# yex33/ReSpaSol

Hardware: AMD Instinct MI355X
Metric: CSR SpMV GFLOP/s + achieved HBM GB/s (fp64 vs fp32), SuiteSparse set, 1/2/4/8 GPU (higher is better)
Workload: dtype f64; 1 GPU; big-set CSR SpMV fp64, 15 matrices per step; matrices=15, nnz_stored_total=268386865, parallelism=1 GPU, launch=rsp_spmv_batch (1 launch(es) of <= 32 matrices per step part): whole step

## Files before the change

include/rsp.h:

```cpp
#ifndef RSP_H
#define RSP_H

#include <stddef.h>
#include <stdint.h>

#ifdef __cplusplus
extern "C" {
#endif

#define RSP_VERSION_MAJOR 0
#define RSP_VERSION_MINOR 1

typedef enum {
    RSP_STATUS_SUCCESS = 0,
    RSP_STATUS_NOT_INITIALIZED = 1,
    RSP_STATUS_ALLOC_FAILED = 2,
    RSP_STATUS_INVALID_VALUE = 3,
    RSP_STATUS_ARCH_MISMATCH = 4,
    RSP_STATUS_EXECUTION_FAILED = 6,
    RSP_STATUS_INTERNAL_ERROR = 7,
    RSP_STATUS_MATRIX_TYPE_NOT_SUPPORTED = 8,
    RSP_STATUS_ZERO_PIVOT = 9,
    RSP_STATUS_NOT_SUPPORTED = 10
} rsp_status_t;

typedef enum { RSP_R_64F = 0, RSP_R_32F = 1 } rsp_datatype_t;

typedef enum { RSP_OPERATION_NON_TRANSPOSE = 0, RSP_OPERATION_TRANSPOSE = 1 } rsp_operation_t;

typedef struct rsp_context *rsp_handle_t;
typedef struct rsp_spmat *rsp_spmat_t;
typedef struct rsp_ilu0_info *rsp_ilu0_info_t;
typedef struct rsp_spmv_batch *rsp_spmv_batch_t;


rsp_status_t rsp_create(rsp_handle_t *handle);
rsp_status_t rsp_destroy(rsp_handle_t handle);
rsp_status_t rsp_set_stream(rsp_handle_t handle, void *stream);
rsp_status_t rsp_get_stream(rsp_handle_t handle, void **stream);
rsp_status_t rsp_set_ftz(rsp_handle_t handle, int enable);
rsp_status_t rsp_get_ftz(rsp_handle_t handle, int *enable);
const char *rsp_get_error_string(rsp_status_t status);
int rsp_get_version(void);


rsp_status_t rsp_create_csr(rsp_spmat_t *mat, int64_t rows, int64_t cols, int64_t nnz,
                            void *d_row_offsets, void *d_col_ind, void *d_values,
                            rsp_datatype_t value_type);
rsp_status_t rsp_csr_set_values(rsp_spmat_t mat, void *d_values, rsp_datatype_t value_type);
rsp_status_t rsp_destroy_spmat(rsp_spmat_t mat);


rsp_status_t rsp_spmv_buffer_size(rsp_handle_t handle, rsp_operation_t op, const void *alpha,
                                  rsp_spmat_t mat, const void *beta, rsp_datatype_t compute_type,
                                  size_t *buffer_size);
rsp_status_t rsp_spmv_preprocess(rsp_handle_t handle, rsp_operation_t op, const void *alpha,
                                 rsp_spmat_t mat, const void *d_x, const void *beta, void *d_y,
                                 rsp_datatype_t compute_type, void *d_buffer);
rsp_status_t rsp_spmv(rsp_handle_t handle, rsp_operation_t op, const void *alpha, rsp_spmat_t mat,
                      const void *d_x, const void *beta, void *d_y, rsp_datatype_t compute_type,
                      void *d_buffer);


rsp_status_t rsp_create_ilu0_info(rsp_ilu0_info_t *info);
rsp_status_t rsp_destroy_ilu0_info(rsp_ilu0_info_t info);

rsp_status_t rsp_ilu0_buffer_size(rsp_handle_t handle, int n, int nnz, rsp_datatype_t value_type,
                                  rsp_ilu0_info_t info, size_t *buffer_size);

rsp_status_t rsp_ilu0_analysis(rsp_handle_t handle, int n, int nnz, const int *d_row_offsets,
                               const int *d_col_ind, rsp_ilu0_info_t info);

rsp_status_t rsp_trsv_analysis(rsp_handle_t handle, rsp_operation_t op, rsp_ilu0_info_t info);

rsp_status_t rsp_ilu0_zero_pivot(rsp_handle_t handle, rsp_ilu0_info_t info, int *position);

#define RSP_TRSV_L 0
#define RSP_TRSV_LT 1
#define RSP_TRSV_U 2
rsp_status_t rsp_trsv_zero_pivot(rsp_handle_t handle, rsp_ilu0_info_t info, int which, int *position);

rsp_status_t rsp_ilu0_factor(rsp_handle_t handle, rsp_ilu0_info_t info, rsp_datatype_t value_type,
                             void *d_values);

rsp_status_t rsp_trsv_lower_unit(rsp_handle_t handle, rsp_operation_t op, const void *alpha,
                                 rsp_ilu0_info_t info, rsp_datatype_t value_type,
                                 const void *d_values, const void *d_x, void *d_y);

rsp_status_t rsp_trsv_upper(rsp_handle_t handle, const void *alpha, rsp_ilu0_info_t info,
                            rsp_datatype_t value_type, const void *d_values, const void *d_x,
                            void *d_y);


typedef struct rsp_bicgstab *rsp_bicgstab_t;
typedef enum { RSP_SOLVE_CONVERGED = 0, RSP_SOLVE_MAX_ITERS = 1, RSP_SOLVE_BREAKDOWN = 2 } rsp_solve_reason_t;

rsp_status_t rsp_bicgstab_create(rsp_handle_t handle, rsp_spmat_t A, rsp_ilu0_info_t info,
                                 rsp_datatype_t precond_type, const void *d_factor, rsp_bicgstab_t *s);
rsp_status_t rsp_bicgstab_solve(rsp_handle_t handle, rsp_bicgstab_t s, const void *d_b, void *d_x,
                                double rtol, int max_iters, int check_every,
                                int *iters, double *relres, rsp_solve_reason_t *reason);
rsp_status_t rsp_bicgstab_history(rsp_bicgstab_t s, int cap, double *relres, int *count);
rsp_status_t rsp_bicgstab_destroy(rsp_bicgstab_t s);
rsp_status_t rsp_dot(rsp_handle_t handle, rsp_datatype_t value_type, int64_t n, const void *d_x,
                     const void *d_y, double *result);

#define RSP_GMRES_MAX_RESTART 64
typedef struct rsp_gmres *rsp_gmres_t;
rsp_status_t rsp_gmres_create(rsp_handle_t handle, rsp_spmat_t A, rsp_ilu0_info_t info,
                              rsp_datatype_t precond_type, const void *d_factor, int restart,
                              rsp_gmres_t *s);
rsp_status_t rsp_gmres_solve(rsp_handle_t handle, rsp_gmres_t s, const void *d_b, void *d_x, double rtol,
                             int max_iters, int check_every, int *iters, double *relres,
                             rsp_solve_reason_t *reason);
rsp_status_t rsp_gmres_history(rsp_gmres_t s, int cap, double *relres, int *count);
rsp_status_t rsp_gmres_destroy(rsp_gmres_t s);
rsp_status_t rsp_orthogonalize(rsp_handle_t handle, rsp_datatype_t value_type, int64_t n, int k,
                               const void *d_V, int64_t ldv, void *d_w, double *h);
rsp_status_t rsp_gmres_lsq_host(int k, int ldh, const double *H, double beta, double *y, double *est);


rsp_status_t rsp_gather(rsp_handle_t handle, rsp_datatype_t value_type, int64_t n,
                        const int64_t *d_idx, const void *d_src, void *d_dst);
rsp_status_t rsp_scatter(rsp_handle_t handle, rsp_datatype_t value_type, int64_t n,
                         const int64_t *d_idx, const void *d_src, void *d_dst);

rsp_status_t rsp_spmv_plan_info(rsp_spmat_t mat, int64_t *tiles, int64_t *entries_16bit);

rsp_status_t rsp_spmat_set_local_cols(rsp_spmat_t mat, int64_t ncols_local);
rsp_status_t rsp_spmv_part(rsp_handle_t handle, const void *alpha, rsp_spmat_t mat,
                           const void *d_x, const void *beta, void *d_y,
                           rsp_datatype_t compute_type, void *d_buffer, int part);

rsp_status_t rsp_spmv_batch_create(rsp_handle_t handle, int count, const rsp_spmat_t *mats,
                                   const void *const *d_x, void *const *d_y,
                                   void *const *d_buffers, rsp_datatype_t compute_type,
                                   int part, rsp_spmv_batch_t *batch);
rsp_status_t rsp_spmv_batch_run(rsp_handle_t handle, rsp_spmv_batch_t batch, const void *alpha,
                                const void *beta);
rsp_status_t rsp_spmv_batch_destroy(rsp_spmv_batch_t batch);
rsp_status_t rsp_spmv_batch_info(rsp_spmv_batch_t batch, int64_t *tiles, int64_t *entries_16bit);

rsp_status_t rsp_ilu0_levels(rsp_ilu0_info_t info, int *levels_lower, int *levels_upper);
rsp_status_t rsp_ilu0_solve_blocks(rsp_ilu0_info_t info, int *blocks_lower, int *blocks_upper);

rsp_status_t rsp_ilu0_analysis_host(int n, const int *row_offsets, const int *col_ind,
                                    int *levels_lower, int *levels_upper, uint64_t *digest,
                                    double *phase_ms);
rsp_status_t rsp_spmv_plan_host(int m, const int *row_offsets, const int *col_ind, int64_t nnz,
                                rsp_datatype_t compute_type, int64_t *tiles, int64_t *entries_16bit,
                                int64_t *entries_staged);
rsp_status_t rsp_spmv_plan_stats(int m, const int *row_offsets, const int *col_ind, int64_t nnz,
                                 rsp_datatype_t compute_type, int64_t stats[8]);
rsp_status_t rsp_ilu0_plan_digest(rsp_ilu0_info_t info, uint64_t *digest);

#ifdef __cplusplus
}
#endif

#endif
```

respasol_amd/_lib.py:

```python
from __future__ import annotations

import ctypes as C
import os

_HERE = os.path.dirname(os.path.abspath(__file__))
LIB_DIR = os.path.join(_HERE, "lib")
BIN_DIR = os.path.join(_HERE, "bin")


class RspError(RuntimeError):

    def __init__(self, status: int, where: str):
        self.status = int(status)
        super().__init__(f"{where}: {STATUS_NAMES.get(self.status, 'RSP_STATUS_UNKNOWN')} ({self.status})")


STATUS_SUCCESS = 0
STATUS_NOT_INITIALIZED = 1
STATUS_ALLOC_FAILED = 2
STATUS_INVALID_VALUE = 3
STATUS_ARCH_MISMATCH = 4
STATUS_EXECUTION_FAILED = 6
STATUS_INTERNAL_ERROR = 7
STATUS_MATRIX_TYPE_NOT_SUPPORTED = 8
STATUS_ZERO_PIVOT = 9
STATUS_NOT_SUPPORTED = 10
STATUS_NAMES = {
    0: "RSP_STATUS_SUCCESS", 1: "RSP_STATUS_NOT_INITIALIZED", 2: "RSP_STATUS_ALLOC_FAILED",
    3: "RSP_STATUS_INVALID_VALUE", 4: "RSP_STATUS_ARCH_MISMATCH", 6: "RSP_STATUS_EXECUTION_FAILED",
    7: "RSP_STATUS_INTERNAL_ERROR", 8: "RSP_STATUS_MATRIX_TYPE_NOT_SUPPORTED",
    9: "RSP_STATUS_ZERO_PIVOT", 10: "RSP_STATUS_NOT_SUPPORTED",
}

R_64F = 0
R_32F = 1
OP_N = 0
OP_T = 1

SOLVE_CONVERGED = 0
SOLVE_MAX_ITERS = 1
SOLVE_BREAKDOWN = 2
KRY_CHUNK = 2048
KRY_MAX_GRID = 1024
GMRES_MAX_RESTART = 64

MM_FULL_SYMMETRIC = 0x1
MM_QUIET = 0x2
MM_SERIAL = 0x4
SURR_FTZ_STRESS = 0x1


class CSRStruct(C.Structure):

    _fields_ = [("isSymmetric", C.c_int), ("m", C.c_int), ("n", C.c_int), ("nnz", C.c_int),
                ("rowptr", C.POINTER(C.c_int)), ("colidx", C.POINTER(C.c_int)),
                ("values", C.POINTER(C.c_double))]


class COOStruct(C.Structure):

    _fields_ = [("isSymmetric", C.c_int), ("m", C.c_int), ("n", C.c_int), ("nnz", C.c_int),
                ("Colidx", C.POINTER(C.c_int)), ("Rowidx", C.POINTER(C.c_int)),
                ("values", C.POINTER(C.c_double))]


vp = C.c_void_p
ip = C.POINTER(C.c_int)
i64 = C.c_int64
i32 = C.c_int

RSP_PROTOS = {
    "rsp_create": (i32, [C.POINTER(vp)]),
    "rsp_destroy": (i32, [vp]),
    "rsp_set_stream": (i32, [vp, vp]),
    "rsp_get_stream": (i32, [vp, C.POINTER(vp)]),
    "rsp_set_ftz": (i32, [vp, i32]),
    "rsp_get_ftz": (i32, [vp, ip]),
    "rsp_get_error_string": (C.c_char_p, [i32]),
    "rsp_get_version": (i32, []),
    "rsp_create_csr": (i32, [C.POINTER(vp), i64, i64, i64, vp, vp, vp, i32]),
    "rsp_csr_set_values": (i32, [vp, vp, i32]),
    "rsp_destroy_spmat": (i32, [vp]),
    "rsp_spmv_buffer_size": (i32, [vp, i32, vp, vp, vp, i32, C.POINTER(C.c_size_t)]),
    "rsp_spmv_preprocess": (i32, [vp, i32, vp, vp, vp, vp, vp, i32, vp]),
    "rsp_spmv": (i32, [vp, i32, vp, vp, vp, vp, vp, i32, vp]),
    "rsp_create_ilu0_info": (i32, [C.POINTER(vp)]),
    "rsp_destroy_ilu0_info": (i32, [vp]),
    "rsp_ilu0_buffer_size": (i32, [vp, i32, i32, i32, vp, C.POINTER(C.c_size_t)]),
    "rsp_ilu0_analysis": (i32, [vp, i32, i32, vp, vp, vp]),
    "rsp_ilu0_zero_pivot": (i32, [vp, vp, ip]),
    "rsp_trsv_zero_pivot": (i32, [vp, vp, i32, ip]),
    "rsp_ilu0_factor": (i32, [vp, vp, i32, vp]),
    "rsp_trsv_lower_unit": (i32, [vp, i32, vp, vp, i32, vp, vp, vp]),
    "rsp_trsv_upper": (i32, [vp, vp, vp, i32, vp, vp, vp]),
    "rsp_ilu0_levels": (i32, [vp, ip, ip]),
    "rsp_ilu0_solve_blocks": (i32, [vp, ip, ip]),
    "rsp_trsv_analysis": (i32, [vp, i32, vp]),
    "rsp_bicgstab_create": (i32, [vp, vp, vp, i32, vp, C.POINTER(vp)]),
    "rsp_bicgstab_solve": (i32, [vp, vp, vp, vp, C.c_double, i32, i32, ip, C.POINTER(C.c_double), ip]),
    "rsp_bicgstab_history": (i32, [vp, i32, C.POINTER(C.c_double), ip]),
    "rsp_bicgstab_destroy": (i32, [vp]),
    "rsp_dot": (i32, [vp, i32, i64, vp, vp, C.POINTER(C.c_double)]),
    "rsp_gmres_create": (i32, [vp, vp, vp, i32, vp, i32, C.POINTER(vp)]),
    "rsp_gmres_solve": (i32, [vp, vp, vp, vp, C.c_double, i32, i32, ip, C.POINTER(C.c_double), ip]),
    "rsp_gmres_history": (i32, [vp, i32, C.POINTER(C.c_double), ip]),
    "rsp_gmres_destroy": (i32, [vp]),
    "rsp_orthogonalize": (i32, [vp, i32, i64, i32, vp, i64, vp, C.POINTER(C.c_double)]),
    "rsp_gmres_lsq_host": (i32, [i32, i32, C.POINTER(C.c_double), C.c_double, C.POINTER(C.c_double),
                                 C.POINTER(C.c_double)]),
    "rsp_gather": (i32, [vp, i32, i64, vp, vp, vp]),
    "rsp_scatter": (i32, [vp, i32, i64, vp, vp, vp]),
    "rsp_spmat_set_local_cols": (i32, [vp, i64]),
    "rsp_spmv_part": (i32, [vp, vp, vp, vp, vp, vp, i32, vp, i32]),
    "rsp_spmv_batch_create": (i32, [vp, i32, vp, vp, vp, vp, i32, i32, vp]),
    "rsp_spmv_batch_run": (i32, [vp, vp, vp, vp]),
    "rsp_spmv_batch_destroy": (i32, [vp]),
    "rsp_spmv_batch_info": (i32, [vp, vp, vp]),
    "rsp_spmv_plan_info": (i32, [vp, vp, vp]),
    "rsp_ilu0_analysis_host": (i32, [i32, vp, vp, vp, vp, vp, vp]),
    "rsp_spmv_plan_host": (i32, [i32, vp, vp, C.c_int64, i32, vp, vp, vp]),
    "rsp_spmv_plan_stats": (i32, [i32, vp, vp, C.c_int64, i32, vp]),
    "rsp_ilu0_plan_digest": (i32, [vp, vp]),
}

HOST_PROTOS = {
    "loadMatrixMarket": (i32, [C.c_char_p, C.POINTER(CSRStruct), i32, i32]),
    "loadCooMatrix": (i32, [C.c_char_p, C.POINTER(COOStruct), i32, i32]),
    "rsp_mm_load": (i32, [C.c_char_p, C.POINTER(CSRStruct), i32, i32, i32]),
    "rsp_mm_load_buffer": (i32, [C.c_char_p, C.c_size_t, C.POINTER(CSRStruct), i32, i32, i32]),
    "rsp_row_qsort": (None, [ip, C.POINTER(C.c_double), i32, i32]),
    "rsp_csr_free": (None, [C.POINTER(CSRStruct)]),
    "rsp_coo_free": (None, [C.POINTER(COOStruct)]),
    "rsp_csr_save": (i32, [C.c_char_p, C.POINTER(CSRStruct)]),
    "rsp_csr_load": (i32, [C.c_char_p, C.POINTER(CSRStruct)]),
    "rsp_dlarnv": (i32, [i32, ip, i64, C.POINTER(C.c_double)]),
    "rsp_set_cpu_ftz": (None, [i32]),
    "rsp_surrogate_count": (i32, []),
    "rsp_surrogate_name": (C.c_char_p, [i32]),
    "rsp_surrogate_info": (i32, [C.c_char_p, ip, C.POINTER(i64), ip, ip, ip]),
    "rsp_surrogate_rowlens": (i32, [C.c_char_p, C.c_double, i32, i32, i32, ip]),
    "rsp_surrogate_rows": (i32, [C.c_char_p, C.c_double, ip]),
    "rsp_surrogate_fill": (i32, [C.c_char_p, C.c_double, i32, i32, i32, ip, ip, C.POINTER(C.c_double)]),
    "rsp_surrogate_csr": (i32, [C.c_char_p, C.c_double, i32, C.POINTER(CSRStruct)]),
    "rsp_partition_rows": (i32, [ip, i32, i32, ip]),
    "rsp_padded_chunk": (i32, [ip, i32]),
    "rsp_remap_cols_padded": (i32, [i64, ip, ip, i32, i32, ip]),
    "rsp_host_spmv_f64": (None, [i32, ip, ip, vp, vp, vp]),
    "rsp_host_spmv_f32": (None, [i32, ip, ip, vp, vp, vp]),
}


def _load(name: str, protos: dict, path: str | None = None, probe: bool = False) -> C.CDLL:
    path = path or os.path.join(LIB_DIR, name)
    if not os.path.exists(path):
        raise ImportError(
            f"{path} is missing: build the HIP/C libraries first "
            f"(python -c 'import __graft_entry__ as g; g.build()' or make -C respasol_amd/csrc)")
    lib = C.CDLL(path, mode=C.RTLD_GLOBAL)
    for fname, (res, args) in protos.items():
        if probe and not hasattr(lib, fname):
            continue
        fn = getattr(lib, fname)
        fn.restype = res
        fn.argtypes = args
    return lib


host = _load("librsp_host.so", HOST_PROTOS)
_RSP_PATH = os.environ.get("RSP_PROBE_LIB") or os.path.join(LIB_DIR, "librsp.so")
rsp = (None if os.environ.get("RSP_HOST_ONLY") == "1"
       else _load("librsp.so", RSP_PROTOS, _RSP_PATH, probe=bool(os.environ.get("RSP_PROBE_LIB"))))


def check(status: int, where: str) -> None:
    if status != STATUS_SUCCESS:
        raise RspError(status, where)


def loaded_paths() -> list[str]:
    return [os.path.join(LIB_DIR, "librsp_host.so"), _RSP_PATH]
```

respasol_amd/csrc/rsp_api.cpp:

```cpp

#include "rsp_internal.h"

#include <atomic>

using namespace rsp_api;

using rsp::SpmvBlock;
using rsp::SpmvLongRow;
using rsp_plan::PlanOptions;
using rsp_plan::TilePlan;

namespace {
std::atomic<unsigned long long> g_plan_next{1};
unsigned long long plan_new_gen() { return g_plan_next.fetch_add(1); }
}


static int64_t spmv_resident_tiles(rsp_handle_t h, rsp_datatype_t t) {
    return (int64_t)rsp_k::spmv_tiles_per_cu((int)elem_size(t)) * h->num_cus;
}

static PlanOptions handle_plan_options(rsp_handle_t h, rsp_datatype_t t, int64_t local_cols, int64_t spread) {
    const int e = (int)elem_size(t), v = h->spmv_variant;
    PlanOptions o = rsp_plan::plan_options(t);
    o.spread = spread;
    o.local_cols = local_cols;
    o.row_align = (v & 64) ? 128 / e : (v & 128) ? 64 / e : 1;
    o.use_c16 = !(v & 32);
    o.use_stage = !(v & rsp::kSpmvVariantNoStage);
    return o;
}

static rsp_status_t download_pattern(rsp_handle_t h, rsp_spmat_t mat, rsp_an::hvec<int> &rp,
                                     rsp_an::hvec<int> &ci) {
    const int m = (int)mat->rows;
    rp.assign((size_t)m + 1, 0);
    ci.clear();
    if (m > 0) {
        RSP_CHECK_HIP(hipMemcpyAsync(rp.data(), mat->rowptr, ((size_t)m + 1) * sizeof(int),
                                     hipMemcpyDeviceToHost, h->stream));
        RSP_CHECK_HIP(hipStreamSynchronize(h->stream));
    }
    if (m > 0 && rp[0] != 0) return RSP_STATUS_INVALID_VALUE;
    for (int i = 0; i < m; i++)
        if (rp[i + 1] < rp[i]) return RSP_STATUS_INVALID_VALUE;
    if (m > 0 && (int64_t)rp[(size_t)m] > mat->nnz) return RSP_STATUS_INVALID_VALUE;
    if (m > 0 && rp[(size_t)m] > 0) {
        if (!mat->colidx) return RSP_STATUS_INVALID_VALUE;
        ci.resize((size_t)rp[(size_t)m]);
        RSP_CHECK_HIP(hipMemcpyAsync(ci.data(), mat->colidx, ci.size() * sizeof(int),
                                     hipMemcpyDeviceToHost, h->stream));
        RSP_CHECK_HIP(hipStreamSynchronize(h->stream));
        const int ncols = (int)mat->cols;
        for (int c : ci)
            if ((unsigned)c >= (unsigned)ncols) return RSP_STATUS_INVALID_VALUE;
    }
    return RSP_STATUS_SUCCESS;
}

rsp_status_t rsp_api::spmv_plan(rsp_handle_t h, rsp_spmat_t mat, rsp_datatype_t compute_type) {
    const int m = (int)mat->rows;
    rsp_an::hvec<int> rp, ci;
    rsp_status_t st = download_pattern(h, mat, rp, ci);
    if (st != RSP_STATUS_SUCCESS) return st;
    const bool spread = (h->spmv_variant & 512) != 0;
    TilePlan p;
    rsp_plan::make_tile_plan(rp.data(), ci.data(), m, mat->nnz,
                             handle_plan_options(h, compute_type, mat->local_cols,
                                                 spread ? spmv_resident_tiles(h, compute_type) : 0),
                             p);
    const size_t elem = elem_size(compute_type);
    const rsp_plan::SpmvLayout lay = rsp_plan::spmv_layout({p.blocks.size(), p.longrows.size(), (size_t)p.nslots},
                                                           elem, (int64_t)p.c16.size(), p.runs.size());
    mat->planned = 0;
    if (lay.bytes > mat->plan_cap || !mat->d_plan) {
        if (mat->d_plan) {
            int cur = 0;
            (void)hipGetDevice(&cur);
            (void)hipSetDevice(mat->plan_device);
            (void)hipFree(mat->d_plan);
            (void)hipSetDevice(cur);
            mat->d_plan = nullptr;
            mat->plan_cap = 0;
        }
        RSP_CHECK_HIP(hipMalloc(&mat->d_plan, std::max<size_t>(lay.bytes, 256)));
        mat->plan_cap = std::max<size_t>(lay.bytes, 256);
        RSP_CHECK_HIP(hipGetDevice(&mat->plan_device));
    }
    char *buf = (char *)mat->d_plan;
    auto upload = [&](size_t off, const void *src, size_t bytes) {
        return bytes == 0 ? hipSuccess : hipMemcpyAsync(buf + off, src, bytes, hipMemcpyHostToDevice, h->stream);
    };
    RSP_CHECK_HIP(upload(0, p.blocks.data(), p.blocks.size() * sizeof(SpmvBlock)));
    RSP_CHECK_HIP(upload(lay.off_cbase, p.cbase.data(), p.cbase.size() * sizeof(int)));
    RSP_CHECK_HIP(upload(lay.off_poff, p.poff.data(), p.poff.size() * sizeof(int)));
    RSP_CHECK_HIP(upload(lay.off_cidx, p.c16.data(), p.c16.size() * sizeof(uint16_t)));
    RSP_CHECK_HIP(upload(lay.off_runs, p.runs.data(), p.runs.size() * sizeof(int)));
    RSP_CHECK_HIP(upload(lay.off_long, p.longrows.data(), p.longrows.size() * sizeof(SpmvLongRow)));
    if (p.nslots > 0)
        RSP_CHECK_HIP(hipMemsetAsync(buf + lay.off_part, 0, (size_t)p.nslots * 2 * elem, h->stream));
    RSP_CHECK_HIP(hipStreamSynchronize(h->stream));
    mat->planned = 1;
    mat->plan_type = compute_type;
    mat->nblocks = (int)p.blocks.size();
    mat->nint = p.nint;
    mat->plan_gen = plan_new_gen();
    mat->nlong = (int)p.longrows.size();
    mat->nslots = p.nslots;
    mat->nnz_s = m > 0 ? rp[(size_t)m] : 0;
    mat->lay = lay;
    mat->nnz_c16 = p.nnz_c16;
    mat->nnz_staged = p.nnz_staged;
    return RSP_STATUS_SUCCESS;
}

rsp_status_t rsp_api::spmv_run(rsp_handle_t h, rsp_operation_t op, const void *alpha, rsp_spmat_t mat,
                               const void *d_x, const void *beta, void *d_y,
                               rsp_datatype_t compute_type, void *d_buffer, int part) {
    if (!h) return RSP_STATUS_NOT_INITIALIZED;
    if (!mat || !alpha || !beta) return RSP_STATUS_INVALID_VALUE;
    if (op != RSP_OPERATION_NON_TRANSPOSE) return RSP_STATUS_NOT_SUPPORTED;
    if (compute_type != mat->type) return RSP_STATUS_INVALID_VALUE;
    if (mat->rows > 0 && (!d_y || (mat->cols > 0 && !d_x))) return RSP_STATUS_INVALID_VALUE;
    (void)d_buffer;
    if (!mat->planned || mat->plan_type != compute_type) {
        rsp_status_t st = spmv_plan(h, mat, compute_type);
        if (st != RSP_STATUS_SUCCESS) return st;
    }
    char *plan = (char *)mat->d_plan;
    rsp::SpmvArgs a;
    a.m = (int)mat->rows;
    a.rowptr = mat->rowptr;
    a.colidx = mat->colidx;
    a.vals = mat->vals;
    a.x = d_x;
    a.y = d_y;
    a.blocks = (const SpmvBlock *)plan;
    a.nblocks = mat->nblocks;
    a.cbases = (const int *)(plan + mat->lay.off_cbase);
    a.poffs = (const int *)(plan + mat->lay.off_poff);
    a.cidx = (const unsigned short *)(plan + mat->lay.off_cidx);
    a.runs = (const int *)(plan + mat->lay.off_runs);
    a.cmax = mat->cols > 0 ? (int)(mat->cols - 1) : 0;
    a.longrows = (const SpmvLongRow *)(plan + mat->lay.off_long);
    a.nlong = mat->nlong;
    a.partials = plan + mat->lay.off_part;
    if (compute_type == RSP_R_64F) {
        a.alpha = *(const double *)alpha;
        a.beta = *(const double *)beta;
    } else {
        a.alpha = *(const float *)alpha;
        a.beta = *(const float *)beta;
    }
    if (part != 0) {
        if (a.beta != 0.0) return RSP_STATUS_INVALID_VALUE;
        if (part == 1) {
            a.nblocks = mat->nint;
            a.nlong = 0;
        } else {
            a.blocks += mat->nint;
            a.cbases += mat->nint;
            a.poffs += mat->nint;
            a.nblocks = mat->nblocks - mat->nint;
        }
    }
    a.vector_ok = ((((uintptr_t)mat->colidx) | ((uintptr_t)mat->vals)) & 15) == 0;
    a.nnz = mat->nnz_s;
    a.variant = h->spmv_variant;
    hipError_t e;
    if (compute_type == RSP_R_64F)
        e = rsp_k::spmv_f64(a, h->stream);
    else
        e = h->ftz ? rsp_k_ftz::spmv_f32(a, h->stream) : rsp_k::spmv_f32(a, h->stream);
    return e == hipSuccess ? RSP_STATUS_SUCCESS : RSP_STATUS_EXECUTION_FAILED;
}


struct rsp_spmv_batch {
    rsp_datatype_t type;
    int part;
    rsp_an::hvec<rsp_spmat_t> mats;
    rsp_an::hvec<unsigned long long> plan_gen;
    rsp_an::hvec<rsp::SpmvBatchArgs> launches;
    void *d_mem = nullptr;
    int64_t tiles = 0, entries_16bit = 0;
    ~rsp_spmv_batch() {
        if (d_mem) (void)hipFree(d_mem);
    }
};

static rsp_status_t spmv_batch_create(rsp_handle_t h, int count, const rsp_spmat_t *mats,
                                      const void *const *d_x, void *const *d_y,
                                      void *const *d_buffers, rsp_datatype_t compute_type,
                                      int part, rsp_spmv_batch_t *batch) {
    if (!h) return RSP_STATUS_NOT_INITIALIZED;
    (void)d_buffers;
    if (!batch || count < 0 || (count > 0 && (!mats || !d_x || !d_y)))
        return RSP_STATUS_INVALID_VALUE;
    if (part < 0 || part > 2) return RSP_STATUS_INVALID_VALUE;
    if (compute_type != RSP_R_64F && compute_type != RSP_R_32F) return RSP_STATUS_INVALID_VALUE;
    *batch = nullptr;
    for (int j = 0; j < count; j++) {
        rsp_spmat_t A = mats[j];
        if (!A) return RSP_STATUS_INVALID_VALUE;
        if (A->type != compute_type) return RSP_STATUS_INVALID_VALUE;
        if (A->rows > 0 && (!d_y[j] || (A->cols > 0 && !d_x[j]))) return RSP_STATUS_INVALID_VALUE;
        if (!A->planned || A->plan_type != compute_type) {
            rsp_status_t st = spmv_plan(h, A, compute_type);
            if (st != RSP_STATUS_SUCCESS) return st;
        }
    }
    std::unique_ptr<rsp_spmv_batch> b(new rsp_spmv_batch());
    b->type = compute_type;
    b->part = part;
    const int64_t R = spmv_resident_tiles(h, compute_type);
    const bool spread_ok = !(h->spmv_variant & 16);
    rsp_an::hvec<TilePlan> plans((size_t)count);
    struct Region { size_t off, len; };
    struct Span {
        int first, count, nt, nl;
        rsp_an::hvec<Region> reg;
        enum { kEntries, kTiles, kCbases, kPoffs, kLongRows, kC16, kRuns, kPartials };
        const Region &at(int kind, int q) const { return reg[kind < kC16 ? kind : kC16 + (kind - kC16) * count + q]; }
    };
    rsp_an::hvec<Span> spans;
    size_t bytes = 0;
    auto tile_range = [part](const TilePlan &p, int *t0, int *t1) {
        *t0 = part == 2 ? p.nint : 0;
        *t1 = part == 1 ? p.nint : (int)p.blocks.size();
    };
    for (int first = 0; first < count; first += rsp::kSpmvBatchMax) {
        Span sp{first, std::min(rsp::kSpmvBatchMax, count - first), 0, 0, {}};
        rsp_an::hvec<rsp_an::hvec<int>> rps((size_t)sp.count), cis((size_t)sp.count);
        auto plan_members = [&](int64_t spread_all, int64_t nnz_all) {
            sp.nt = 0;
            for (int q = 0; q < sp.count; q++) {
                rsp_spmat_t A = mats[first + q];
                const int64_t nnz_q = A->rows > 0 ? rps[q][(size_t)A->rows] : 0;
                const int64_t share =
                    spread_all > 0 ? std::max<int64_t>(1, spread_all * nnz_q / std::max<int64_t>(1, nnz_all)) : 0;
                TilePlan &p = plans[first + q];
                rsp_plan::make_tile_plan(rps[q].data(), cis[q].data(), (int)A->rows, A->nnz,
                                         handle_plan_options(h, compute_type, A->local_cols, share), p);
                int t0, t1;
                tile_range(p, &t0, &t1);
                sp.nt += t1 - t0;
            }
        };
        int64_t nnz_all = 0;
        for (int q = 0; q < sp.count; q++) {
            rsp_spmat_t A = mats[first + q];
            rsp_status_t st = download_pattern(h, A, rps[q], cis[q]);
            if (st != RSP_STATUS_SUCCESS) return st;
            nnz_all += A->rows > 0 ? rps[q][(size_t)A->rows] : 0;
        }
        plan_members(0, nnz_all);
        if (spread_ok && sp.nt < R) plan_members(R, nnz_all);
        for (int q = 0; q < sp.count; q++) {
            const TilePlan &p = plans[first + q];
            rsp_spmat_t A = mats[first + q];
            if ((int)p.longrows.size() != A->nlong || p.nslots != A->nslots)
                return RSP_STATUS_INTERNAL_ERROR;
            sp.nl += part == 1 ? 0 : (int)p.longrows.size();
        }
        sp.reg = {{0, (size_t)sp.count * sizeof(rsp::SpmvBatchEntry)},
                  {0, (size_t)sp.nt * sizeof(SpmvBlock)},
                  {0, (size_t)sp.nt * sizeof(int)},
                  {0, (size_t)sp.nt * sizeof(int)},
                  {0, (size_t)sp.nl * sizeof(SpmvLongRow)}};
        for (int q = 0; q < sp.count; q++) sp.reg.push_back({0, plans[first + q].c16.size() * sizeof(uint16_t)});
        for (int q = 0; q < sp.count; q++) sp.reg.push_back({0, plans[first + q].runs.size() * sizeof(int)});
        for (int q = 0; q < sp.count; q++)
            sp.reg.push_back({0, (size_t)plans[first + q].nslots * 2 * elem_size(compute_type)});
        for (Region &r : sp.reg) {
            r.off = bytes;
            bytes += (r.len + 15) & ~(size_t)15;
        }
        spans.push_back(sp);
    }
    {
        size_t end = 0;
        for (const Span &sp : spans)
            for (const Region &r : sp.reg) {
                if (r.off < end || r.off + r.len > bytes) return RSP_STATUS_INTERNAL_ERROR;
                end = r.off + r.len;
            }
    }
    if (bytes > 0) RSP_CHECK_HIP(hipMalloc(&b->d_mem, bytes));
    rsp_an::hvec<unsigned char> host(bytes);
    bool fits = true;
    for (const Span &sp : spans) {
        auto dev = [&](int kind, int q = 0) { return (char *)b->d_mem + sp.at(kind, q).off; };
        auto put = [&](int kind, int q, size_t at, const void *src, size_t n) {
            const Region &r = sp.at(kind, q);
            if (at + n > r.len)
                fits = false;
            else if (n > 0)
                memcpy(host.data() + r.off + at, src, n);
        };
        rsp::SpmvBatchArgs a{};
        a.entries = (const rsp::SpmvBatchEntry *)dev(Span::kEntries);
        a.tiles = (const SpmvBlock *)dev(Span::kTiles);
        a.cbases = (const int *)dev(Span::kCbases);
        a.poffs = (const int *)dev(Span::kPoffs);
        a.longrows = (const SpmvLongRow *)dev(Span::kLongRows);
        a.count = sp.count;
        for (int q = 0; q <= rsp::kSpmvBatchMax; q++)
            a.tiles_at.begin[q] = a.longs_at.begin[q] = INT_MAX;
        size_t nt = 0, nl = 0;
        for (int q = 0; q < sp.count; q++) {
            rsp_spmat_t A = mats[sp.first + q];
            const TilePlan &p = plans[sp.first + q];
            int t0, t1;
            tile_range(p, &t0, &t1);
            const size_t ntq = (size_t)(t1 - t0), nlq = part == 1 ? 0 : p.longrows.size();
            rsp::SpmvBatchEntry e{};
            e.rowptr = A->rowptr;
            e.colidx = A->colidx;
            e.vals = A->vals;
            e.x = d_x[sp.first + q];
            e.y = d_y[sp.first + q];
            e.partials = (void *)dev(Span::kPartials, q);
            e.cidx = (const unsigned short *)dev(Span::kC16, q);
            e.runs = (const int *)dev(Span::kRuns, q);
            e.cmax = A->cols > 0 ? (int)(A->cols - 1) : 0;
            e.nnz = A->nnz_s;
            e.vector_ok = ((((uintptr_t)A->colidx) | ((uintptr_t)A->vals)) & 15) == 0;
            put(Span::kEntries, 0, (size_t)q * sizeof(e), &e, sizeof(e));
            a.tiles_at.begin[q] = (int)nt;
            a.longs_at.begin[q] = (int)nl;
            for (int t = t0; t < t1; t++)
                if (p.cbase[(size_t)t] != rsp_plan::kCbaseInt32)
                    b->entries_16bit += p.blocks[(size_t)t].k1 - p.blocks[(size_t)t].k0;
            b->tiles += (int64_t)ntq;
            put(Span::kTiles, 0, nt * sizeof(SpmvBlock), p.blocks.data() + t0, ntq * sizeof(SpmvBlock));
            put(Span::kCbases, 0, nt * sizeof(int), p.cbase.data() + t0, ntq * sizeof(int));
            put(Span::kPoffs, 0, nt * sizeof(int), p.poff.data() + t0, ntq * sizeof(int));
            put(Span::kLongRows, 0, nl * sizeof(SpmvLongRow), p.longrows.data(), nlq * sizeof(SpmvLongRow));
            put(Span::kC16, q, 0, p.c16.data(), p.c16.size() * sizeof(uint16_t));
            put(Span::kRuns, q, 0, p.runs.data(), p.runs.size() * sizeof(int));
            nt += ntq;
            nl += nlq;
        }
        a.tiles_at.begin[sp.count] = (int)nt;
        a.longs_at.begin[sp.count] = (int)nl;
        b->launches.push_back(a);
    }
    if (!fits) return RSP_STATUS_INTERNAL_ERROR;
    if (bytes > 0) {
        RSP_CHECK_HIP(hipMemcpyAsync(b->d_mem, host.data(), bytes, hipMemcpyHostToDevice, h->stream));
        RSP_CHECK_HIP(hipStreamSynchronize(h->stream));
    }
    for (int j = 0; j < count; j++) {
        b->mats.push_back(mats[j]);
        b->plan_gen.push_back(mats[j]->plan_gen);
    }
    *batch = b.release();
    return RSP_STATUS_SUCCESS;
}

extern "C" {

int rsp_get_version(void) { return RSP_VERSION_MAJOR * 1000 + RSP_VERSION_MINOR; }

const char *rsp_get_error_string(rsp_status_t s) {
    switch (s) {
        case RSP_STATUS_SUCCESS: return "RSP_STATUS_SUCCESS";
        case RSP_STATUS_NOT_INITIALIZED: return "RSP_STATUS_NOT_INITIALIZED";
        case RSP_STATUS_ALLOC_FAILED: return "RSP_STATUS_ALLOC_FAILED";
        case RSP_STATUS_INVALID_VALUE: return "RSP_STATUS_INVALID_VALUE";
        case RSP_STATUS_ARCH_MISMATCH: return "RSP_STATUS_ARCH_MISMATCH";
        case RSP_STATUS_EXECUTION_FAILED: return "RSP_STATUS_EXECUTION_FAILED";
        case RSP_STATUS_INTERNAL_ERROR: return "RSP_STATUS_INTERNAL_ERROR";
        case RSP_STATUS_MATRIX_TYPE_NOT_SUPPORTED: return "RSP_STATUS_MATRIX_TYPE_NOT_SUPPORTED";
        case RSP_STATUS_ZERO_PIVOT: return "RSP_STATUS_ZERO_PIVOT";
        case RSP_STATUS_NOT_SUPPORTED: return "RSP_STATUS_NOT_SUPPORTED";
    }
    return "RSP_STATUS_UNKNOWN";
}

rsp_status_t rsp_create(rsp_handle_t *handle) {
    if (!handle) return RSP_STATUS_INVALID_VALUE;
    *handle = nullptr;
    int dev = 0;
    if (hipGetDevice(&dev) != hipSuccess) return RSP_STATUS_NOT_INITIALIZED;
    hipDeviceProp_t prop;
    if (hipGetDeviceProperties(&prop, dev) != hipSuccess) return RSP_STATUS_NOT_INITIALIZED;
    if (strncmp(prop.gcnArchName, "gfx950", 6) != 0) return RSP_STATUS_ARCH_MISMATCH;
    rsp_context *c = new (std::nothrow) rsp_context;
    if (!c) return RSP_STATUS_ALLOC_FAILED;
    c->device = dev;
    c->stream = nullptr;
    c->ftz = 0;
    const char *v = getenv("RSP_SPMV_VARIANT");
    c->spmv_variant = v ? atoi(v) : 0;
    c->num_cus = prop.multiProcessorCount > 0 ? prop.multiProcessorCount : 256;
    rsp_k::warm_spmv();
    rsp_k_ftz::warm_spmv();
    rsp_k::warm_ilu();
    rsp_k_ftz::warm_ilu();
    rsp_k::warm_analysis();
    rsp_k::warm_krylov();
    rsp_k_ftz::warm_krylov();
    c->d_ftrace = nullptr;
    c->d_strace = nullptr;
    c->d_dot = nullptr;
    c->h_dot = nullptr;
    c->d_gm = nullptr;
    c->h_gm = nullptr;
    *handle = c;
    return RSP_STATUS_SUCCESS;
}

rsp_status_t rsp_destroy(rsp_handle_t h) {
    if (!h) return RSP_STATUS_NOT_INITIALIZED;
    if (h->d_ftrace || h->d_strace || h->d_dot || h->h_dot || h->d_gm || h->h_gm) {
        int cur = 0;
        (void)hipGetDevice(&cur);
        (void)hipSetDevice(h->device);
        if (h->d_ftrace) (void)hipFree(h->d_ftrace);
        if (h->d_strace) (void)hipFree(h->d_strace);
        if (h->d_dot) (void)hipFree(h->d_dot);
        if (h->h_dot) (void)hipHostFree(h->h_dot);
        if (h->d_gm) (void)hipFree(h->d_gm);
        if (h->h_gm) (void)hipHostFree(h->h_gm);
        (void)hipSetDevice(cur);
    }
    delete h;
    return RSP_STATUS_SUCCESS;
}

rsp_status_t rsp_set_stream(rsp_handle_t h, void *stream) {
    if (!h) return RSP_STATUS_NOT_INITIALIZED;
    h->stream = (hipStream_t)stream;
    return RSP_STATUS_SUCCESS;
}

rsp_status_t rsp_get_stream(rsp_handle_t h, void **stream) {
    if (!h) return RSP_STATUS_NOT_INITIALIZED;
    if (!stream) return RSP_STATUS_INVALID_VALUE;
    *stream = (void *)h->stream;
    return RSP_STATUS_SUCCESS;
}

rsp_status_t rsp_set_ftz(rsp_handle_t h, int enable) {
    if (!h) return RSP_STATUS_NOT_INITIALIZED;
    h->ftz = enable ? 1 : 0;
    return RSP_STATUS_SUCCESS;
}

rsp_status_t rsp_get_ftz(rsp_handle_t h, int *enable) {
    if (!h) return RSP_STATUS_NOT_INITIALIZED;
    if (!enable) return RSP_STATUS_INVALID_VALUE;
    *enable = h->ftz;
    return RSP_STATUS_SUCCESS;
}


rsp_status_t rsp_create_csr(rsp_spmat_t *mat, int64_t rows, int64_t cols, int64_t nnz,
                            void *d_row_offsets, void *d_col_ind, void *d_values,
                            rsp_datatype_t value_type) {
    if (!mat) return RSP_STATUS_INVALID_VALUE;
    *mat = nullptr;
    if (rows < 0 || cols < 0 || nnz < 0 || rows > INT_MAX - 1 || cols > INT_MAX || nnz > INT_MAX)
        return RSP_STATUS_INVALID_VALUE;
    if (value_type != RSP_R_64F && value_type != RSP_R_32F) return RSP_STATUS_INVALID_VALUE;
    if (!d_row_offsets && rows > 0) return RSP_STATUS_INVALID_VALUE;
    if ((!d_col_ind || !d_values) && nnz > 0) return RSP_STATUS_INVALID_VALUE;
    rsp_spmat *a = new (std::nothrow) rsp_spmat;
    if (!a) return RSP_STATUS_ALLOC_FAILED;
    memset(a, 0, sizeof(*a));
    a->rows = rows;
    a->cols = cols;
    a->nnz = nnz;
    a->rowptr = (int *)d_row_offsets;
    a->colidx = (int *)d_col_ind;
    a->vals = d_values;
    a->type = value_type;
    a->planned = 0;
    a->d_plan = nullptr;
    a->local_cols = -1;
    *mat = a;
    return RSP_STATUS_SUCCESS;
}

rsp_status_t rsp_spmat_set_local_cols(rsp_spmat_t mat, int64_t ncols_local) {
    if (!mat || ncols_local < 0 || ncols_local > mat->cols) return RSP_STATUS_INVALID_VALUE;
    mat->local_cols = ncols_local;
    mat->planned = 0;
    return RSP_STATUS_SUCCESS;
}

rsp_status_t rsp_csr_set_values(rsp_spmat_t mat, void *d_values, rsp_datatype_t value_type) {
    if (!mat) return RSP_STATUS_INVALID_VALUE;
    if (value_type != RSP_R_64F && value_type != RSP_R_32F) return RSP_STATUS_INVALID_VALUE;
    if (d_values != mat->vals) mat->plan_gen = plan_new_gen();
    mat->vals = d_values;
    if (value_type != mat->type) mat->planned = 0;
    mat->type = value_type;
    return RSP_STATUS_SUCCESS;
}

rsp_status_t rsp_destroy_spmat(rsp_spmat_t mat) {
    if (!mat) return RSP_STATUS_INVALID_VALUE;
    if (mat->d_plan) {
        int cur = 0;
        (void)hipGetDevice(&cur);
        (void)hipSetDevice(mat->plan_device);
        (void)hipFree(mat->d_plan);
        (void)hipSetDevice(cur);
    }
    delete mat;
    return RSP_STATUS_SUCCESS;
}


rsp_status_t rsp_spmv_buffer_size(rsp_handle_t h, rsp_operation_t op, const void *alpha,
                                  rsp_spmat_t mat, const void *beta, rsp_datatype_t compute_type,
                                  size_t *buffer_size) {
    (void)alpha;
    (void)beta;
    return guarded([&] {
        if (!h) return RSP_STATUS_NOT_INITIALIZED;
        if (!mat || !buffer_size) return RSP_STATUS_INVALID_VALUE;
        if (op != RSP_OPERATION_NON_TRANSPOSE) return RSP_STATUS_NOT_SUPPORTED;
        if (compute_type != mat->type) return RSP_STATUS_INVALID_VALUE;
        if (!mat->planned || mat->plan_type != compute_type) RSP_TRY(spmv_plan(h, mat, compute_type));
        *buffer_size = 0;
        return RSP_STATUS_SUCCESS;
    });
}

rsp_status_t rsp_spmv_preprocess(rsp_handle_t h, rsp_operation_t op, const void *alpha,
                                 rsp_spmat_t mat, const void *d_x, const void *beta, void *d_y,
                                 rsp_datatype_t compute_type, void *d_buffer) {
    (void)alpha;
    (void)beta;
    (void)d_x;
    (void)d_y;
    (void)d_buffer;
    return guarded([&] {
        if (!h) return RSP_STATUS_NOT_INITIALIZED;
        if (!mat) return RSP_STATUS_INVALID_VALUE;
        if (op != RSP_OPERATION_NON_TRANSPOSE) return RSP_STATUS_NOT_SUPPORTED;
        if (compute_type != mat->type) return RSP_STATUS_INVALID_VALUE;
        return spmv_plan(h, mat, compute_type);
    });
}

rsp_status_t rsp_spmv_plan_info(rsp_spmat_t mat, int64_t *tiles, int64_t *entries_16bit) {
    if (!mat || !tiles || !entries_16bit) return RSP_STATUS_INVALID_VALUE;
    if (!mat->planned) return RSP_STATUS_NOT_INITIALIZED;
    *tiles = mat->nblocks;
    *entries_16bit = mat->nnz_c16;
    return RSP_STATUS_SUCCESS;
}

rsp_status_t rsp_spmv(rsp_handle_t h, rsp_operation_t op, const void *alpha, rsp_spmat_t mat,
                      const void *d_x, const void *beta, void *d_y, rsp_datatype_t compute_type,
                      void *d_buffer) {
    return guarded([&] { return spmv_run(h, op, alpha, mat, d_x, beta, d_y, compute_type, d_buffer, 0); });
}

rsp_status_t rsp_spmv_part(rsp_handle_t h, const void *alpha, rsp_spmat_t mat, const void *d_x,
                           const void *beta, void *d_y, rsp_datatype_t compute_type,
                           void *d_buffer, int part) {
    return guarded([&] {
        if (part < 0 || part > 2) return RSP_STATUS_INVALID_VALUE;
        return spmv_run(h, RSP_OPERATION_NON_TRANSPOSE, alpha, mat, d_x, beta, d_y, compute_type,
                        d_buffer, part);
    });
}


rsp_status_t rsp_spmv_batch_create(rsp_handle_t h, int count, const rsp_spmat_t *mats,
                                   const void *const *d_x, void *const *d_y,
                                   void *const *d_buffers, rsp_datatype_t compute_type,
                                   int part, rsp_spmv_batch_t *batch) {
    return guarded([&] { return spmv_batch_create(h, count, mats, d_x, d_y, d_buffers, compute_type, part, batch); });
}

rsp_status_t rsp_spmv_batch_run(rsp_handle_t h, rsp_spmv_batch_t b, const void *alpha,
                                const void *beta) {
    if (!h) return RSP_STATUS_NOT_INITIALIZED;
    if (!b || !alpha || !beta) return RSP_STATUS_INVALID_VALUE;
    for (size_t j = 0; j < b->mats.size(); j++) {
        const rsp_spmat_t A = b->mats[j];
        if (!A->planned || A->plan_gen != b->plan_gen[j]) return RSP_STATUS_INVALID_VALUE;
    }
    const double av = b->type == RSP_R_64F ? *(const double *)alpha : *(const float *)alpha;
    const double bv = b->type == RSP_R_64F ? *(const double *)beta : *(const float *)beta;
    if (b->part != 0 && bv != 0.0) return RSP_STATUS_INVALID_VALUE;
    for (rsp::SpmvBatchArgs a : b->launches) {
        a.alpha = av;
        a.beta = bv;
        a.variant = h->spmv_variant;
        hipError_t e;
        if (b->type == RSP_R_64F)
            e = rsp_k::spmv_batch_f64(a, h->stream);
        else
            e = h->ftz ? rsp_k_ftz::spmv_batch_f32(a, h->stream) : rsp_k::spmv_batch_f32(a, h->stream);
        if (e != hipSuccess) return RSP_STATUS_EXECUTION_FAILED;
    }
    return RSP_STATUS_SUCCESS;
}

rsp_status_t rsp_spmv_batch_info(rsp_spmv_batch_t b, int64_t *tiles, int64_t *entries_16bit) {
    if (!b || !tiles || !entries_16bit) return RSP_STATUS_INVALID_VALUE;
    *tiles = b->tiles;
    *entries_16bit = b->entries_16bit;
    return RSP_STATUS_SUCCESS;
}

rsp_status_t rsp_spmv_batch_destroy(rsp_spmv_batch_t b) {
    if (!b) return RSP_STATUS_INVALID_VALUE;
    delete b;
    return RSP_STATUS_SUCCESS;
}

rsp_status_t rsp_gather(rsp_handle_t h, rsp_datatype_t value_type, int64_t n, const int64_t *d_idx,
                        const void *d_src, void *d_dst) {
    if (!h) return RSP_STATUS_NOT_INITIALIZED;
    if (value_type != RSP_R_64F && value_type != RSP_R_32F) return RSP_STATUS_INVALID_VALUE;
    if (n < 0 || (n > 0 && (!d_idx || !d_src || !d_dst))) return RSP_STATUS_INVALID_VALUE;
    hipError_t e = rsp_k::gather(value_type == RSP_R_64F ? 8 : 4, n, d_idx, d_src, d_dst, h->stream);
    return e == hipSuccess ? RSP_STATUS_SUCCESS : RSP_STATUS_EXECUTION_FAILED;
}

rsp_status_t rsp_scatter(rsp_handle_t h, rsp_datatype_t value_type, int64_t n, const int64_t *d_idx,
                         const void *d_src, void *d_dst) {
    if (!h) return RSP_STATUS_NOT_INITIALIZED;
    if (value_type != RSP_R_64F && value_type != RSP_R_32F) return RSP_STATUS_INVALID_VALUE;
    if (n < 0 || (n > 0 && (!d_idx || !d_src || !d_dst))) return RSP_STATUS_INVALID_VALUE;
    hipError_t e = rsp_k::scatter(value_type == RSP_R_64F ? 8 : 4, n, d_idx, d_src, d_dst, h->stream);
    return e == hipSuccess ? RSP_STATUS_SUCCESS : RSP_STATUS_EXECUTION_FAILED;
}

rsp_status_t rsp_spmv_plan_host(int m, const int *row_offsets, const int *col_ind, int64_t nnz,
                                rsp_datatype_t compute_type, int64_t *tiles, int64_t *entries_16bit,
                                int64_t *entries_staged) {
    return guarded([&] {
        if (m < 0 || (m > 0 && (!row_offsets || !col_ind)) || !tiles || !entries_16bit || !entries_staged)
            return RSP_STATUS_INVALID_VALUE;
        if (compute_type != RSP_R_64F && compute_type != RSP_R_32F) return RSP_STATUS_NOT_SUPPORTED;
        const PlanOptions o = rsp_plan::plan_options(compute_type);
        TilePlan p;
        rsp_plan::make_tile_plan(row_offsets, col_ind, m, nnz, o, p);
        if (!rsp_plan::plan_verify(row_offsets, col_ind, m, o, p)) return RSP_STATUS_INTERNAL_ERROR;
        *tiles = (int64_t)p.blocks.size();
        *entries_16bit = p.nnz_c16;
        *entries_staged = p.nnz_staged;
        return RSP_STATUS_SUCCESS;
    });
}

rsp_status_t rsp_spmv_plan_stats(int m, const int *row_offsets, const int *col_ind, int64_t nnz,
                                 rsp_datatype_t compute_type, int64_t stats[8]) {
    return guarded([&] {
        if (m < 0 || (m > 0 && (!row_offsets || !col_ind)) || !stats) return RSP_STATUS_INVALID_VALUE;
        if (compute_type != RSP_R_64F && compute_type != RSP_R_32F) return RSP_STATUS_NOT_SUPPORTED;
        TilePlan p;
        rsp_plan::make_tile_plan(row_offsets, col_ind, m, nnz, rsp_plan::plan_options(compute_type), p);
        rsp_plan::plan_stats(p, compute_type, stats);
        return RSP_STATUS_SUCCESS;
    });
}

}
```

respasol_amd/csrc/rsp_kernels.h:

```cpp
#pragma once

#include <hip/hip_runtime.h>
#include <stdint.h>

namespace rsp {

struct alignas(16) SpmvBlock {
    int r0, r1, k0, k1;
};

struct alignas(16) SpmvLongRow {
    int row, first, nchunks, pad;
};

#ifndef RSP_SPMV_THREADS
#define RSP_SPMV_THREADS 256
#endif
constexpr int kSpmvThreads = RSP_SPMV_THREADS;
#ifndef RSP_SPMV_ITER
#define RSP_SPMV_ITER 4
#endif
constexpr int kSpmvIter = RSP_SPMV_ITER;
#ifndef RSP_SPMV_MAXROWS
#define RSP_SPMV_MAXROWS 512
#endif
constexpr int kSpmvMaxRows = RSP_SPMV_MAXROWS;
constexpr int kSpmvLongRow = 256;
constexpr int kSpmvHeavyMax = 128;
constexpr int kSpmvWholeRow = -2147483647 - 1;
template <typename T>
struct SpmvTile {
    static constexpr int kVec = 16 / sizeof(T);
    static constexpr int kSlots = kSpmvThreads * kSpmvIter * kVec;
    static constexpr int kMaxNnz = kSlots - (kVec - 1);
    static constexpr int kChunk = kSpmvThreads * 4 * kVec - (kVec - 1);
    static_assert(kChunk <= kMaxNnz, "a chunk must fit one tile");
    static constexpr int kMaxRows = sizeof(T) == 8 ? kSpmvMaxRows : 2 * kSpmvMaxRows;
    static constexpr int kStageSlots = sizeof(T) == 8 ? 1536 : 2048;
    static constexpr bool kStageList = sizeof(T) == 8;
};
static_assert(SpmvTile<float>::kMaxNnz / 33 < kSpmvHeavyMax && SpmvTile<double>::kMaxNnz / 33 < kSpmvHeavyMax,
              "every > 32-entry row of a tile fits the heavy-row list");
constexpr int kStageRuns = 254;

struct SpmvArgs {
    int m;
    const int *rowptr;
    const int *colidx;
    const void *vals;
    const void *x;
    void *y;
    const SpmvBlock *blocks;
    int nblocks;
    const int *cbases;
    const unsigned short *cidx;
    const int *runs;
    const int *poffs;
    int cmax;
    const SpmvLongRow *longrows;
    int nlong;
    void *partials;
    double alpha, beta;
    int nnz;
    int vector_ok;
    int variant;
};

constexpr int kSpmvBatchMax = 32;
struct alignas(16) SpmvBatchEntry {
    const int *rowptr;
    const int *colidx;
    const void *vals;
    const void *x;
    void *y;
    void *partials;
    const unsigned short *cidx;
    const int *runs;
    int nnz;
    int vector_ok;
    int cmax;
};
struct SpmvBatchTable {
    int begin[kSpmvBatchMax + 1];
};
struct SpmvBatchArgs {
    const SpmvBatchEntry *entries;
    const SpmvBlock *tiles;
    const int *cbases;
    const int *poffs;
    const SpmvLongRow *longrows;
    int count;
    SpmvBatchTable tiles_at, longs_at;
    double alpha, beta;
    int variant;
};
constexpr int kSpmvVariantFixup = 256;
constexpr int kSpmvVariantNoStage = 1024;

struct LevelSeg {
    int lb, le, thin, c0, c1;
    int nth;
};
struct alignas(16) RowTask {
    int i, t0, t1, d;
};
struct alignas(16) LevelChunk {
    int l0, l1;
    int x0, x1;
    int k0, k1;
    int st0, st1;
};
struct alignas(16) FlowItem {
    int x0, n, t0, gate;
};
struct alignas(16) ThinRowPlan {
    int g, out, i, d;
};
struct alignas(8) StagedTerm {
    int slot, j;
};

struct LevelPlan {
    const int *rows;
    const int *ptr_dev;
    const int *ptr_host;
    int nlev;
    const LevelSeg *segs;
    int nseg;
    int batch;
    int group;
    const RowTask *tasks;
    const int *tpos;
    const int *src;
    const LevelChunk *chunks;
    const ThinRowPlan *trow;
    const int *sid;
    const StagedTerm *stg;
    const FlowItem *fitems;
    int has_flow;
    int nterms;
    const int *nshort;
    const int *nshort_host;
    const int *nwave_host;
    const int *sbase_host;
};
constexpr int kLongTerms = 64;
constexpr int kHubTerms = 256;
constexpr int kFatLongTerms = 8;
constexpr int kFatLongDefault = 3;
constexpr int kYWin = 4096;
constexpr int kChunkRows = 1024;
constexpr int kChunkTerms = 4096;
constexpr int kThinThreads = 1024;
constexpr int kGroup = 4;
constexpr int kPadSrc = -(kYWin + 1);
constexpr int kIluWaves = 4;
constexpr int kFacRow = 256;
constexpr int kFacPairs = 1024;
constexpr int kThinSolveRows = 512;
constexpr int kThinSolveTerms = 2048;
constexpr int kThinFactorRows = 1024;
constexpr int kRndItems = 2048;
constexpr int kRndPairs = 4096;
constexpr int kRndStaged = 4096;
constexpr int kRndRounds = 2048;
constexpr int kRndLevelItems = 1 << 15;
constexpr int kRndFlowItems = 1024;
constexpr int kRndItemPairs = 1024;
constexpr int kRndLevelStart = 1 << 15;
struct alignas(16) RndChunk {
    int i0, i1, p0, p1, s0, s1, r0, r1;
};
struct alignas(16) RndItem {
    int pos, u, d, zr;
};

struct alignas(16) FacRow {
    int i, rs, di, re, q0, q1, hasdiag, pad;
};

struct FacSlotLevel {
    long long off;
    int stride, rm, qm, pad;
};
__host__ __device__ constexpr int fac_pairs_at(int rm) { return (8 + 2 * rm + 1) & ~1; }

struct alignas(16) FacFlowItem {
    long long off;
    int rmqm, gate;
};
struct FacFlowRun {
    int lb, le, c0, c1;
};

struct FlowCtl {
    int *status;
    int gen;
    unsigned long long ticks;
    unsigned long long *claim;
    unsigned long long *claim_host;
    int mode;
    unsigned *tickets;
    unsigned long long *tk_seq;
    int *done;
    int grid_x;
    unsigned epoch;
};
constexpr int kFlowClaims = 1;
constexpr int kFlowTickets = 2;
constexpr int kFlowTicketCtrs = 8;
constexpr int kFlowOwnMax = 1024;
constexpr int kFlowStealUs = 50;


struct IluArgs {
    int n;
    const int *rowptr;
    const int *colidx;
    const int *dpos;
    const int *hasdiag;
    void *vals;
    int *zero_pivot;
    const int *upd_ptr;
    const int *upd_l;
    const int *upd_u;
    const int *lord;
    const int *lend;
    const int *udiv;
    const FacRow *frow;
    const int *fslots;
    const FacSlotLevel *fslev;
    int fat_slots;
    int fat_lds;
    LevelPlan plan;
    const RndChunk *rchunks;
    const RndItem *ritems;
    const int *rpairs, *rstaged, *rrounds;
    unsigned long long *trace;
    int trace_cap;
    int defer_rounds;
    int narrow_waves;
    const FacFlowItem *fitems;
    const FacFlowRun *fruns;
    int nfruns;
    const int *lev;
    void *forig;
    int gen;
    int flow, flow_grid, flow_sleep;
    int flow_cus;
    FlowCtl fc;
    int fac_one;
};

constexpr int kBlkRows = 64, kBlkYMax = 32, kBlkNear = 12, kBlkNearWin = 1 << 30, kBlkWin = 16384;
constexpr int kBlkLongCap = 64 * kBlkNear;
constexpr int kBlkPre = 6;
constexpr int kBlkLdsMax = 160 * 1024;
struct alignas(16) BlkDesc {
    int p0, np, kind, kn;
    int eoff, ne, doff, nd;
    int loff, nlev, pad[2];
};
struct alignas(16) BlkRow {
    int off, nx, ny, nfar;
};
struct BlkSeg {
    int b0, b1, p0, p1;
};
struct BlkArgs {
    int n, nb;
    const int *order;
    const BlkDesc *desc;
    const BlkRow *rows;
    const int *ref;
    const int *vpos;
    const unsigned *eord;
    const int *lptr;
    const int *rptr;
    const unsigned *rit;
    const BlkSeg *segs;
    int nseg;
    int lds_elems;
    int lds_words;
    const void *vals, *x;
    void *y;
    double alpha;
    void *ev, *yp;
    void *rc;
};

struct TrsvArgs {
    int n;
    const int *rowptr;
    const int *colidx;
    const int *dpos;
    const int *hasdiag;
    const void *vals;
    const void *x;
    void *y;
    double alpha;
    LevelPlan plan;
    void *sval;
    void *sx;
    void *sdg;
    unsigned long long *trace;
    int trace_cap;
    int trace_clk;
    int wave_lds;
    int narrow_waves;
    int narrow_split;
    int narrow_pairs;
    int loaders;
    int flow;
    int flow_grid;
    int flow_cus;
    FlowCtl fc;
    int flow_sleep;
};


constexpr int kKryThreads = 256;
constexpr int kKryChunk = 2048;
constexpr int kKryMaxGrid = 1024;
struct KryGrid {
    int grid;
    long long chunk;
};
inline KryGrid kry_grid(long long n) {
    KryGrid g;
    const long long span = (long long)kKryChunk * kKryMaxGrid;
    g.chunk = (long long)kKryChunk * (n > span ? (n + span - 1) / span : 1);
    g.grid = n > 0 ? (int)((n + g.chunk - 1) / g.chunk) : 1;
    return g;
}
enum {
    kKryRho0 = 0,
    kKryRho1 = 1,
    kKryAlpha = 2,
    kKryOmega = 3,
    kKryFlag = 4,
    kKryFlagIt = 5,
    kKryScalars = 16
};
enum { kKryPartRR = 0, kKryPartBB, kKryPartRhR, kKryPartRhV, kKryPartTS, kKryPartTT, kKryDots };
enum { kKryBreakRho = 1, kKryBreakOmega = 2, kKryBreakRhV = 3, kKryBreakTT = 4 };
constexpr size_t kKryBlockDoubles = kKryScalars + (size_t)kKryDots * kKryMaxGrid;
enum KryOp {
    kKryInit,
    kKryPUpdate,
    kKryDotRhV,
    kKrySUpdate,
    kKryDotTS,
    kKryXUpdate,
    kKryWiden,
    kKryZero,
    kKryDot
};
enum { kKryF64 = 0, kKryF32 = 1, kKryF64Copy32 = 2 };
struct KryArgs {
    long long n;
    double *blk;
    int it;
    const void *b;
    const void *c;
    void *x, *r, *rhat, *p, *v, *s, *t;
    const void *phat, *shat;
    void *copy32;
};
inline double kry_combine_host(const double *part, int g) {
    double v[kKryThreads];
    for (int t = 0; t < kKryThreads; t++) {
        v[t] = 0.0;
        for (int i = t; i < g; i += kKryThreads) v[t] += part[i];
    }
    double w[kKryThreads / 64];
    for (int k = 0; k < kKryThreads / 64; k++) {
        double *l = v + 64 * k;
        for (int off = 32; off > 0; off >>= 1)
            for (int i = 0; i < off; i++) l[i] += l[i + off];
        w[k] = l[0];
    }
    return ((w[0] + w[1]) + w[2]) + w[3];
}

constexpr int kGmMax = 64;
constexpr int kGmLd = kGmMax + 1;
enum {
    kGmStop = 0,
    kGmDone = 1,
    kGmBeta = 2,
    kGmBn = 3,
    kGmFlag = kKryFlag,
    kGmFlagIt = kKryFlagIt,
    kGmScalars = 16,
    kGmEst = kGmScalars,
    kGmHead = kGmEst + kGmMax,
    kGmR = kGmHead,
    kGmCs = kGmR + kGmLd * kGmMax,
    kGmSn = kGmCs + kGmMax,
    kGmG = kGmSn + kGmMax,
    kGmY = kGmG + kGmLd,
    kGmH1 = kGmY + kGmMax,
    kGmH2 = kGmH1 + kGmLd,
    kGmSmall = (kGmH2 + kGmLd + 15) / 16 * 16
};
enum {
    kGmPartRR = 0,
    kGmPartBB = 1,
    kGmPartNrm = 2,
    kGmPartD1 = 3,
    kGmPartD2 = kGmPartD1 + kGmLd,
    kGmDots = kGmPartD2 + kGmLd
};
enum { kGmBreakH = 1, kGmBreakDiag = 2, kGmBreakNorm = 3, kGmBreakY = 4 };
constexpr size_t kGmBlockDoubles = kGmSmall + (size_t)kGmDots * kKryMaxGrid;
enum GmOp {
    kGmResid,
    kGmNormalise,
    kGmMultiDot,
    kGmUpdate1,
    kGmUpdate2,
    kGmCombine
};
struct GmArgs {
    long long n;
    double *blk;
    int j;
    int first;
    const void *b;
    void *x;
    void *V;
    long long ldv;
    const void *Z;
    long long ldz;
    void *w;
    void *copy32;
};

#if defined(__HIPCC__)
#define RSP_HD __host__ __device__
#else
#define RSP_HD
#endif
RSP_HD inline int gmres_lsq(double *col, int j, double *cs, double *sn, double *g, const double *R, int ldr,
                            int k, double *y) {
    if (col) {
        for (int i = 0; i <= j + 1; i++)
            if (!(col[i] - col[i] == 0.0)) return kGmBreakH;
        for (int i = 0; i < j; i++) {
            const double a = col[i], b = col[i + 1];
            col[i] = cs[i] * a + sn[i] * b;
            col[i + 1] = cs[i] * b - sn[i] * a;
        }
        const double a = col[j], b = col[j + 1];
        const double aa = a < 0.0 ? -a : a, ab = b < 0.0 ? -b : b;
        const double s = aa > ab ? aa : ab;
        if (s == 0.0) return kGmBreakDiag;
        const double as = a / s, bs = b / s;
        const double r = s * sqrt(as * as + bs * bs);
        if (r == 0.0 || !(r - r == 0.0)) return kGmBreakDiag;
        const double c = a / r, t = b / r;
        cs[j] = c;
        sn[j] = t;
        col[j] = r;
        col[j + 1] = 0.0;
        const double gj = g[j];
        g[j] = c * gj;
        g[j + 1] = -(t * gj);
    }
    if (y) {
        for (int i = k - 1; i >= 0; i--) {
            double v = g[i];
            for (int l = i + 1; l < k; l++) v -= R[i + (size_t)l * ldr] * y[l];
            y[i] = v / R[i + (size_t)i * ldr];
        }
    }
    return 0;
}
}

#define RSP_DECLARE_KERNEL_API(NS)                                                              \
    namespace NS {                                                                              \
    hipError_t spmv_f32(const rsp::SpmvArgs &a, hipStream_t s);                                 \
    hipError_t spmv_batch_f32(const rsp::SpmvBatchArgs &a, hipStream_t s);                      \
    hipError_t ilu0_factor_f32(const rsp::IluArgs &a, hipStream_t s);                           \
    hipError_t trsv_lower_n_f32(const rsp::TrsvArgs &a, hipStream_t s);                         \
    hipError_t trsv_lower_t_f32(const rsp::TrsvArgs &a, hipStream_t s);                         \
    hipError_t trsv_upper_f32(const rsp::TrsvArgs &a, hipStream_t s);                           \
    hipError_t trsv_blocks_f32(const rsp::BlkArgs &a, hipStream_t s);                           \
    void warm_spmv();                                                                           \
    void warm_ilu();                                                                            \
    hipError_t krylov(rsp::KryOp op, int type, const rsp::KryArgs &a, hipStream_t s);           \
    hipError_t gmres(rsp::GmOp op, int type, const rsp::GmArgs &a, hipStream_t s);              \
    void warm_krylov();                                                                         \
    }

RSP_DECLARE_KERNEL_API(rsp_k)
RSP_DECLARE_KERNEL_API(rsp_k_ftz)

namespace rsp_k {
hipError_t gather(int elem_bytes, int64_t n, const int64_t *idx, const void *src, void *dst,
                  hipStream_t s);
hipError_t scatter(int elem_bytes, int64_t n, const int64_t *idx, const void *src, void *dst,
                   hipStream_t s);
hipError_t spmv_f64(const rsp::SpmvArgs &a, hipStream_t s);
hipError_t spmv_batch_f64(const rsp::SpmvBatchArgs &a, hipStream_t s);
int spmv_tiles_per_cu(int elem_bytes);
void warm_analysis();
hipError_t ilu0_factor_f64(const rsp::IluArgs &a, hipStream_t s);
hipError_t trsv_lower_n_f64(const rsp::TrsvArgs &a, hipStream_t s);
hipError_t trsv_lower_t_f64(const rsp::TrsvArgs &a, hipStream_t s);
hipError_t trsv_upper_f64(const rsp::TrsvArgs &a, hipStream_t s);
hipError_t trsv_blocks_f64(const rsp::BlkArgs &a, hipStream_t s);
hipError_t ilu0_build_slots(const rsp::IluArgs &a, const int4 *desc, const long long *offs, int nrows,
                            int *slots, hipStream_t s);
hipError_t ilu_an_rows(int n, const int *rp, const int *ci, int *dpos, int *hasdiag, int *flags, hipStream_t s);
hipError_t ilu_an_count(const int *const rows_c[3], const int n_c[3], int cap0, const int *rp, const int *ci,
                        const int *dpos, const int *hasdiag, int *cnt, int *gcur, hipStream_t s);
hipError_t ilu_an_scan(const int *cnt, int *ptr, int count, void *temp, size_t *temp_bytes, hipStream_t s);
hipError_t ilu_an_gather_pairs(const int *rows, int nrows, const int *rp, const int *ptr, const int *cbase,
                               const int *upd_l, const int *upd_u, int *out_l, int *out_u, hipStream_t s);
hipError_t ilu_an_fill(const int *const rows_c[3], const int n_c[3], int cap0, const int *rp, const int *ci,
                       const int *dpos, const int *hasdiag, const int *ptr, int *gcur, int *upd_l, int *upd_u,
                       hipStream_t s);
hipError_t ilu_an_stages(int n, int maxlen, const int *rp, const int *ci, const int *dpos, const int *hasdiag,
                         const int *ptr, const int *upd_l, int *stage, int *lord, int *lend, int *udiv,
                         int *scratch, const int *wrows, int nwrows, hipStream_t s);
struct SolveTermsArgs {
    int kind, n, nx, total, nch, group;
    const rsp::RowTask *tasks;
    const int *ptr;
    const int *rp, *ci, *dpos;
    const int *ltp, *lts, *ltc;
    const int *lpos;
    const int *ne;
    rsp::LevelChunk *chunks;
    const int *cbase;
    int *tpos, *src, *sid;
    rsp::ThinRowPlan *trow;
    rsp::StagedTerm *stg;
    int *slot_of, *nst, *nst_ptr;
    void *scan;
};
hipError_t ilu_an_solve_terms(const SolveTermsArgs &a, hipStream_t s);
}
```

respasol_amd/csrc/spmv.hip:

```cpp

#include <hip/hip_runtime.h>

#include <type_traits>

#include "rsp_kernels.h"
#include "spmv_pack.h"

#ifndef RSP_KNS
#define RSP_KNS rsp_k
#endif

#ifndef RSP_NT_Y
#define RSP_NT_Y -1
#endif

namespace RSP_KNS {

using rsp::kSpmvThreads;
using rsp::kSpmvHeavyMax;
using rsp::SpmvArgs;
using rsp::SpmvBlock;
using rsp::SpmvLongRow;
using rsp::SpmvTile;
using rsp::kSpmvBatchMax;
using rsp::SpmvBatchArgs;
using rsp::SpmvBatchEntry;
using rsp::SpmvBatchTable;

template <typename T, int N>
struct VecT;
template <>
struct VecT<double, 2> {
    typedef double __attribute__((ext_vector_type(2))) V;
    typedef int __attribute__((ext_vector_type(2))) I;
    typedef unsigned short __attribute__((ext_vector_type(2))) H;
};
template <>
struct VecT<float, 4> {
    typedef float __attribute__((ext_vector_type(4))) V;
    typedef int __attribute__((ext_vector_type(4))) I;
    typedef unsigned short __attribute__((ext_vector_type(4))) H;
};

__device__ __forceinline__ int xcd_swizzle(int bid, int nwg) {
    const int q = nwg >> 3, r = nwg & 7;
    const int xcd = bid & 7, idx = bid >> 3;
    const int start = xcd < r ? xcd * (q + 1) : r * (q + 1) + (xcd - r) * q;
    return start + idx;
}

template <bool NT, typename P>
__device__ __forceinline__ P ld(const P *p) {
    if constexpr (NT)
        return __builtin_nontemporal_load(p);
    else
        return *p;
}

template <typename T, bool NT, bool C16 = false, int NTH = kSpmvThreads,
          int IT = SpmvTile<T>::kSlots / (kSpmvThreads * (16 / sizeof(T)))>
__device__ __forceinline__ void stream_products(const int *__restrict__ colidx,
                                                const unsigned short *__restrict__ cidx, int cbase,
                                                int cmax, const T *__restrict__ vals,
                                                const T *__restrict__ x, int kb, int k1,
                                                T *__restrict__ lds) {
    constexpr int VW = 16 / sizeof(T);
    typedef typename VecT<T, VW>::V V;
    typedef typename VecT<T, VW>::I I;
    typedef typename VecT<T, VW>::H H;
    const int tid = threadIdx.x;
    const int last = (k1 - 1) & ~(VW - 1);
    I ci[IT];
    H ch[IT];
#pragma unroll
    for (int it = 0; it < IT; ++it) {
        const int e = min(kb + (it * NTH + tid) * VW, last);
        if constexpr (C16)
            ch[it] = ld<NT>(reinterpret_cast<const H *>(cidx + e));
        else
            ci[it] = ld<NT>(reinterpret_cast<const I *>(colidx + e));
    }
    V vv[IT];
#pragma unroll
    for (int it = 0; it < IT; ++it) {
        const int e = min(kb + (it * NTH + tid) * VW, last);
        vv[it] = ld<NT>(reinterpret_cast<const V *>(vals + e));
    }
    __builtin_amdgcn_sched_barrier(0);
    T xv[IT][VW];
#pragma unroll
    for (int it = 0; it < IT; ++it)
#pragma unroll
        for (int j = 0; j < VW; ++j) {
            int c;
            if constexpr (C16)
                c = min(cbase + (int)ch[it][j], cmax);
            else
                c = ci[it][j];
            xv[it][j] = x[c];
        }
    __builtin_amdgcn_sched_barrier(0);
#pragma unroll
    for (int it = 0; it < IT; ++it) {
        V p;
#pragma unroll
        for (int j = 0; j < VW; ++j) p[j] = vv[it][j] * xv[it][j];
        *reinterpret_cast<V *>(lds + (it * NTH + tid) * VW) = p;
    }
}

__device__ __forceinline__ void lds_barrier() {
    __builtin_amdgcn_fence(__ATOMIC_RELEASE, "workgroup", "local");
    __builtin_amdgcn_s_barrier();
    __builtin_amdgcn_fence(__ATOMIC_ACQUIRE, "workgroup", "local");
}

template <typename T, bool NT, int PKM, int NTH = kSpmvThreads,
          int IT = SpmvTile<T>::kSlots / (kSpmvThreads * (16 / sizeof(T)))>
__device__ __forceinline__ void stream_products_staged(const unsigned short *__restrict__ cidx,
                                                       const unsigned int *__restrict__ pk, int2 rd,
                                                       int nr, const int (&lsl)[SpmvTile<T>::kStageSlots / NTH],
                                                       const T *__restrict__ vals,
                                                       const T *__restrict__ x, int kb, int k1,
                                                       T *__restrict__ lds) {
    constexpr int VW = 16 / sizeof(T);
    constexpr int SMAX = SpmvTile<T>::kStageSlots / NTH;
    typedef typename VecT<T, VW>::V V;
    const int tid = threadIdx.x;
    const int last = (k1 - 1) & ~(VW - 1);
    constexpr int NW = rsp_pack::words_per_thread(IT * VW);
    constexpr int HW = VW / 2;
    static_assert(NW <= IT * HW, "the packed words fit the unpacked ones' registers");
    const bool pkd = PKM == 2 ? pk != nullptr : PKM == 1;
    unsigned int iw[PKM == 1 ? NW : IT * HW];
    V vv[IT];
    if (pkd) {
        const unsigned int *w = pk + tid * NW;
#pragma unroll
        for (int q = 0; q < NW; ++q) iw[q] = ld<NT>(w + q);
    } else {
#pragma unroll
        for (int it = 0; it < IT; ++it) {
            const int e = min(kb + (it * NTH + tid) * VW, last);
            const unsigned int *w = reinterpret_cast<const unsigned int *>(cidx + e);
#pragma unroll
            for (int q = 0; q < HW; ++q) iw[it * HW + q] = ld<NT>(w + q);
        }
    }
#pragma unroll
    for (int it = 0; it < IT; ++it) {
        const int e = min(kb + (it * NTH + tid) * VW, last);
        vv[it] = ld<NT>(reinterpret_cast<const V *>(vals + e));
    }
    __builtin_amdgcn_sched_barrier(0);
    const __amdgpu_buffer_rsrc_t xr =
        __builtin_amdgcn_make_buffer_rsrc((void *)x, (short)0, 0x7ffffffc, 0x00020000);
    auto xload = [&](int col) {
        if constexpr (sizeof(T) == 8)
            return __builtin_bit_cast(T, __builtin_amdgcn_raw_buffer_load_b64(xr, col * 8, 0, 0));
        else
            return __builtin_bit_cast(T, __builtin_amdgcn_raw_buffer_load_b32(xr, col * 4, 0, 0));
    };
    T xs[SMAX];
    int U;
    if (SpmvTile<T>::kStageList && nr == 255) {
        U = rd.y;
#pragma unroll
        for (int k = 0; k < SMAX; ++k)
            if (k * NTH < U) xs[k] = xload(rd.x + lsl[k]);
    } else {
        int2 *tab = reinterpret_cast<int2 *>(lds + SpmvTile<T>::kSlots) - (nr + 1);
        if (tid <= nr) tab[tid] = rd;
        lds_barrier();
        U = tab[nr].y;
        int us[SMAX], lo[SMAX];
#pragma unroll
        for (int k = 0; k < SMAX; ++k) {
            us[k] = min(k * NTH + tid, U - 1);
            lo[k] = 0;
        }
        for (int n = nr; n > 1;) {
            const int h = n >> 1;
#pragma unroll
            for (int k = 0; k < SMAX; ++k)
                if (tab[lo[k] + h].y <= us[k]) lo[k] += h;
            n -= h;
        }
#pragma unroll
        for (int k = 0; k < SMAX; ++k)
            if (k * NTH < U) {
                const int2 r = tab[lo[k]];
                xs[k] = xload(r.x + (us[k] - r.y));
            }
    }
#pragma unroll
    for (int k = 0; k < SMAX; ++k)
        if (k * NTH < U && k * NTH + tid < U) lds[k * NTH + tid] = xs[k];
    lds_barrier();
    T xv[IT][VW];
    if (pkd) {
#pragma unroll
        for (int it = 0; it < IT; ++it)
#pragma unroll
            for (int j = 0; j < VW; ++j) xv[it][j] = lds[min((int)rsp_pack::get_field(iw, it * VW + j), U - 1)];
    } else {
#pragma unroll
        for (int it = 0; it < IT; ++it)
#pragma unroll
            for (int j = 0; j < VW; ++j)
                xv[it][j] = lds[min((int)((iw[(it * VW + j) >> 1] >> (16 * (j & 1))) & 0xffffu), U - 1)];
    }
    lds_barrier();
#pragma unroll
    for (int it = 0; it < IT; ++it) {
        V p;
#pragma unroll
        for (int j = 0; j < VW; ++j) p[j] = vv[it][j] * xv[it][j];
        *reinterpret_cast<V *>(lds + (it * NTH + tid) * VW) = p;
    }
}

template <typename T, int NTH = kSpmvThreads>
__device__ __forceinline__ void stream_products_scalar(const int *__restrict__ colidx,
                                                       const T *__restrict__ vals,
                                                       const T *__restrict__ x, int k0, int kb,
                                                       int k1, T *lds) {
    for (int e = kb + (int)threadIdx.x; e < k1; e += NTH)
        if (e >= k0) lds[e - kb] = vals[e] * x[colidx[e]];
}

template <typename T, int L, int NTH, typename Sink>
__device__ __forceinline__ void reduce_rows(const T *lds, const unsigned short *rp_lds, int nrows, int kb,
                                            int heavy, int *hl, int *hn, Sink sink) {
    constexpr int NA = 8 / L;
    constexpr int NG = NTH / L;
    const int tid = threadIdx.x;
    const int g = tid / L, lane = tid & (L - 1);
    for (int rr = g; rr - g < nrows; rr += NG) {
        bool active = rr < nrows;
        T acc[NA];
#pragma unroll
        for (int t = 0; t < NA; ++t) acc[t] = T(0);
        if (active) {
            const int a0 = rp_lds[rr] - kb, a1 = rp_lds[rr + 1] - kb, last = a1 - 1;
            if (heavy > 0 && a1 - a0 > heavy) {
                active = false;
                if (lane == 0) hl[atomicAdd(hn, 1)] = rr;
            } else {
                for (int base = a0 + lane; base < a1; base += 8) {
                    T v[NA];
#pragma unroll
                    for (int t = 0; t < NA; ++t) v[t] = lds[min(base + t * L, last)];
#pragma unroll
                    for (int t = 0; t < NA; ++t)
                        acc[t] = base + t * L < a1 ? acc[t] + v[t] : acc[t];
                }
            }
        }
#pragma unroll
        for (int h = NA / 2; h >= 1; h >>= 1)
#pragma unroll
            for (int t = 0; t < h; ++t) acc[t] = acc[t] + acc[t + h];
        T s = acc[0];
#pragma unroll
        for (int off = L / 2; off >= 1; off >>= 1) s = s + __shfl_xor(s, off, 64);
        if (active && lane == 0) sink(rr, s);
    }
}

template <typename T, int NTH, typename Sink>
__device__ __forceinline__ void reduce_heavy_rows(const T *lds, const unsigned short *rp_lds, int kb,
                                                  const int *hl, int hn, Sink sink) {
    constexpr int NG = NTH / 8;
    const int tid = threadIdx.x;
    const int g = tid >> 3, lane = tid & 7;
    for (int h = g; h - g < hn; h += NG) {
        const bool active = h < hn;
        T acc = T(0);
        const int rr = active ? hl[h] : 0;
        if (active) {
            const int a1 = rp_lds[rr + 1] - kb, last = a1 - 1;
            for (int base = rp_lds[rr] - kb + lane; base < a1; base += 32) {
                T v[4];
#pragma unroll
                for (int t = 0; t < 4; ++t) v[t] = lds[min(base + 8 * t, last)];
#pragma unroll
                for (int t = 0; t < 4; ++t) acc = base + 8 * t < a1 ? acc + v[t] : acc;
            }
        }
#pragma unroll
        for (int off = 4; off >= 1; off >>= 1) acc = acc + __shfl_xor(acc, off, 64);
        if (active && lane == 0) sink(rr, acc);
    }
}

template <typename T, int NTH = kSpmvThreads, typename Sink>
__device__ __forceinline__ void reduce_tile_rows(const T *lds, const unsigned short *rp_lds, int nrows,
                                                 int nnzt, int kb, int *hl, int *hn, Sink sink) {
    int L = 1;
    while (L < 8 && 2 * L * nrows <= NTH && 8 * L * nrows <= nnzt) L <<= 1;
    switch (L) {
        case 1: reduce_rows<T, 1, NTH>(lds, rp_lds, nrows, kb, 32, hl, hn, sink); break;
        case 2: reduce_rows<T, 2, NTH>(lds, rp_lds, nrows, kb, 64, hl, hn, sink); break;
        case 4: reduce_rows<T, 4, NTH>(lds, rp_lds, nrows, kb, 128, hl, hn, sink); break;
        default: reduce_rows<T, 8, NTH>(lds, rp_lds, nrows, kb, 0, hl, hn, sink); return;
    }
    lds_barrier();
    const int n = *hn;
    if (n > 0) reduce_heavy_rows<T, NTH>(lds, rp_lds, kb, hl, n, sink);
}

template <typename T>
__device__ __forceinline__ T reduce_long(const T *lds, int a, int e, T *wsum) {
    const int tid = threadIdx.x;
    T s = T(0);
    for (int k = a + tid; k < e; k += kSpmvThreads) s += lds[k];
#pragma unroll
    for (int off = 32; off >= 1; off >>= 1) s = s + __shfl_xor(s, off, 64);
    if ((tid & 63) == 0) wsum[tid >> 6] = s;
    lds_barrier();
    return (wsum[0] + wsum[1]) + (wsum[2] + wsum[3]);
}

#ifdef RSP_SPMV_PROBE_LOADS
#include "spmv_probe.h"
#endif

#if defined(__HIP_DEVICE_COMPILE__) && !defined(__gfx950__) && !defined(__gfx942__)
#error "longrow_arrive's relaxed hand-off is only valid on gfx942 / gfx950"
#endif
template <typename T>
__device__ __forceinline__ void longrow_arrive(const SpmvBlock blk, const int *__restrict__ rowptr,
                                               T *partials, T *__restrict__ y, T t, T alpha, T beta,
                                               bool beta_nz) {
    typedef typename std::conditional<sizeof(T) == 8, unsigned long long, unsigned int>::type U;
    constexpr int C = SpmvTile<T>::kChunk;
    const int lane = threadIdx.x & 63;
    const int slot = -(blk.r1 + 1);
    const int rs = rowptr[blk.r0], re = rowptr[blk.r0 + 1];
    const int first = slot - (blk.k0 - rs) / C;
    const int n = (re - rs + C - 1) / C;
    typedef __attribute__((address_space(1))) U GU;
    typedef __attribute__((address_space(1))) unsigned int GI;
    GU *pv = (GU *)reinterpret_cast<U *>(partials);
    GI *ticket = (GI *)reinterpret_cast<unsigned int *>(partials + 2 * first + 1);
    unsigned int arrived = 0;
    if (lane == 0) {
        __hip_atomic_store(pv + 2 * slot, __builtin_bit_cast(U, t), __ATOMIC_RELAXED, __HIP_MEMORY_SCOPE_AGENT);
        asm volatile("s_waitcnt vmcnt(0)" ::: "memory");
        arrived = __hip_atomic_fetch_add(ticket, 1u, __ATOMIC_RELAXED, __HIP_MEMORY_SCOPE_AGENT);
    }
    arrived = (unsigned int)__builtin_amdgcn_readfirstlane((int)arrived);
    if (arrived != (unsigned int)(n - 1)) return;
    T s = T(0);
    for (int c0 = 0; c0 < n; c0 += 64) {
        const T p = c0 + lane < n ? __builtin_bit_cast(T, __hip_atomic_load(pv + 2 * (first + c0 + lane),
                                                                            __ATOMIC_RELAXED, __HIP_MEMORY_SCOPE_AGENT))
                                  : T(0);
        const int cn = min(64, n - c0);
        for (int c = 0; c < cn; ++c) s += __shfl(p, c, 64);
    }
    if (lane == 0) {
        T out = alpha * s;
        if (beta_nz) out += beta * y[blk.r0];
        y[blk.r0] = out;
        __hip_atomic_store(ticket, 0u, __ATOMIC_RELAXED, __HIP_MEMORY_SCOPE_AGENT);
    }
}

template <typename T, bool NT, bool BETA>
__device__ __forceinline__ void spmv_tile(
    const SpmvBlock blk, const int *__restrict__ rowptr, const int *__restrict__ colidx,
    const unsigned short *__restrict__ cidx, const int *__restrict__ runs, int cbase, int poff, int cmax,
    const T *__restrict__ vals, const T *__restrict__ x, T *__restrict__ y,
    T *partials, T alpha, T beta, int beta_nonzero, int nnz, int vector_ok, T *lds,
    T *wsum, unsigned short *rp_lds, int *hl, int fuse) {
    constexpr int VW = 16 / sizeof(T);
    constexpr int RPQ = (SpmvTile<T>::kMaxRows + kSpmvThreads) / kSpmvThreads;
    constexpr int RPW = (SpmvTile<T>::kMaxRows / 2 + kSpmvThreads) / kSpmvThreads;
    static_assert(RPW <= RPQ, "the packed row words fit the row offsets' registers");
    const int tid = threadIdx.x;
    const int k0 = blk.k0, k1 = blk.k1;
    const bool staged = cbase <= -2;
    constexpr int SMAX = SpmvTile<T>::kStageSlots / kSpmvThreads;
    int2 rd = make_int2(0, 0);
    int nr = 0;
    int lsl[SMAX];
    if (staged) {
        const int code = -2 - cbase;
        nr = code & 255;
        if (SpmvTile<T>::kStageList && nr == 255) {
            rd = reinterpret_cast<const int2 *>(runs)[code >> 8];
            const unsigned short *lst = reinterpret_cast<const unsigned short *>(runs + 2 * (code >> 8) + 2);
#pragma unroll
            for (int k = 0; k < SMAX; ++k)
                if (k * kSpmvThreads < rd.y) lsl[k] = lst[min(k * kSpmvThreads + tid, rd.y - 1)];
        } else if (tid <= nr) {
            rd = reinterpret_cast<const int2 *>(runs)[(code >> 8) + tid];
        }
    }
    const int nrows = blk.r1 - blk.r0;
    const int nrows_ld = nrows > 0 ? nrows : 0;
    const bool vec = vector_ok && k1 > k0 && k1 <= (nnz & ~(VW - 1));
    const int kb = vec ? (k0 & ~(VW - 1)) : k0;
    const unsigned int *rec =
        vec && staged && poff >= 0 ? reinterpret_cast<const unsigned int *>(runs) + (poff >> 1) : nullptr;
    const bool prow = rec && (poff & 1);
    const int nrw = (nrows_ld + 2) >> 1;
    const int *rsrc = prow ? reinterpret_cast<const int *>(rec) +
                                 kSpmvThreads * rsp_pack::words_per_thread(SpmvTile<T>::kSlots / kSpmvThreads)
                           : rowptr + blk.r0;
    const int rlim = prow ? nrw - 1 : nrows_ld;
    int rpv[RPQ];
#pragma unroll
    for (int q = 0; q < RPQ; ++q)
        rpv[q] = rsrc[min(tid + q * kSpmvThreads, rlim)];
#ifdef RSP_SPMV_PROBE_LOADS
    if (vec) {
        probe_tile_loads<T, NT>(colidx, vals, y, blk, kb, k1, rpv[0]);
        return;
    }
#endif
    if (vec && cbase >= 0)
        stream_products<T, NT, true>(colidx, cidx, cbase, cmax, vals, x, kb, k1, lds);
    else if (vec && staged && sizeof(T) == 4)
        stream_products_staged<T, NT, 2>(cidx, rec, rd, nr, lsl, vals, x, kb, k1, lds);
    else if (vec && rec)
        stream_products_staged<T, NT, 1>(cidx, rec, rd, nr, lsl, vals, x, kb, k1, lds);
    else if (vec && staged)
        stream_products_staged<T, NT, 0>(cidx, rec, rd, nr, lsl, vals, x, kb, k1, lds);
    else if (vec)
        stream_products<T, NT>(colidx, cidx, 0, 0, vals, x, kb, k1, lds);
    else
        stream_products_scalar<T>(colidx, vals, x, k0, kb, k1, lds);
    if (prow) {
#pragma unroll
        for (int q = 0; q < RPW; ++q) {
            const int i = tid + q * kSpmvThreads;
            if (i < nrw) reinterpret_cast<unsigned int *>(rp_lds)[i] = (unsigned int)rpv[q];
        }
    } else {
#pragma unroll
        for (int q = 0; q < RPQ; ++q) {
            const int i = tid + q * kSpmvThreads;
            if (i <= nrows) rp_lds[i] = (unsigned short)(rpv[q] - kb);
        }
    }
    if (tid == 0) hl[0] = 0;
    lds_barrier();

    if (blk.r1 < 0) {
        const T t = reduce_long(lds, k0 - kb, k1 - kb, wsum);
        if (blk.r1 != rsp::kSpmvWholeRow && fuse) {
            if (tid < 64) longrow_arrive<T>(blk, rowptr, partials, y, t, alpha, beta, BETA);
        } else if (tid == 0) {
            if (blk.r1 == rsp::kSpmvWholeRow) {
                T out = alpha * t;
                if (BETA) out += beta * y[blk.r0];
                y[blk.r0] = out;
            } else {
                partials[2 * -(blk.r1 + 1)] = t;
            }
        }
        return;
    }

    const int r0 = blk.r0;
    reduce_tile_rows<T>(lds, rp_lds, nrows, k1 - k0, 0, hl + 1, hl, [&](int rr, T sum) {
        T out = alpha * sum;
        if (BETA) out += beta * y[r0 + rr];
        constexpr bool kNtY = RSP_NT_Y > 0 || (RSP_NT_Y < 0 && sizeof(T) == 8);
        if constexpr (kNtY)
            __builtin_nontemporal_store(out, y + r0 + rr);
        else
            y[r0 + rr] = out;
    });
}

template <typename T, bool NT, bool BETA>
__global__ __launch_bounds__(kSpmvThreads) void spmv_tiles(
    const int *__restrict__ rowptr, const int *__restrict__ colidx, const T *__restrict__ vals,
    const T *__restrict__ x, T *__restrict__ y, const SpmvBlock *__restrict__ blocks, int nblocks,
    const int *__restrict__ cbases, const int *__restrict__ poffs, const unsigned short *__restrict__ cidx,
    const int *__restrict__ runs, int cmax, T *partials, T alpha, T beta, int beta_nonzero, int nnz,
    int vector_ok, int fuse) {
    __shared__ __attribute__((aligned(16))) T lds[SpmvTile<T>::kSlots];
    __shared__ T wsum[kSpmvThreads / 64];
    __shared__ int hl[1 + kSpmvHeavyMax];
    __shared__ __attribute__((aligned(4))) unsigned short rp_lds[SpmvTile<T>::kMaxRows + 2];
    const int b = xcd_swizzle(blockIdx.x, nblocks);
    spmv_tile<T, NT, BETA>(blocks[b], rowptr, colidx, cidx, runs, cbases[b], poffs[b], cmax, vals, x, y,
                           partials, alpha, beta, beta_nonzero, nnz, vector_ok, lds, wsum, rp_lds, hl,
                           fuse);
}

template <typename T>
__device__ __forceinline__ void fixup_row(const SpmvLongRow r, const T *__restrict__ partials,
                                          T *__restrict__ y, T alpha, T beta, int beta_nonzero) {
    const int lane = threadIdx.x;
    const T yv = (beta_nonzero && lane == 0) ? y[r.row] : T(0);
    T s = T(0);
    for (int c0 = 0; c0 < r.nchunks; c0 += 64) {
        const T p = c0 + lane < r.nchunks ? partials[2 * (r.first + c0 + lane)] : T(0);
        const int cn = min(64, r.nchunks - c0);
        for (int c = 0; c < cn; ++c) s += __shfl(p, c, 64);
    }
    if (lane == 0) {
        T out = alpha * s;
        if (beta_nonzero) out += beta * yv;
        y[r.row] = out;
    }
}

template <typename T>
__global__ __launch_bounds__(64) void spmv_longrow_fixup(const SpmvLongRow *__restrict__ lr,
                                                          int nlong, const T *__restrict__ partials,
                                                          T *__restrict__ y, T alpha, T beta,
                                                          int beta_nonzero) {
    fixup_row<T>(lr[blockIdx.x], partials, y, alpha, beta, beta_nonzero);
}

template <typename T, bool NT, bool BETA, bool SWZ>
__global__ __launch_bounds__(kSpmvThreads) void spmv_tiles_batch(
    const SpmvBatchEntry *__restrict__ entries, const SpmvBlock *__restrict__ tiles,
    const int *__restrict__ cbases, const int *__restrict__ poffs, SpmvBatchTable at, T alpha, T beta,
    int fuse) {
    __shared__ __attribute__((aligned(16))) T lds[SpmvTile<T>::kSlots];
    __shared__ T wsum[kSpmvThreads / 64];
    __shared__ int hl[1 + kSpmvHeavyMax];
    __shared__ __attribute__((aligned(4))) unsigned short rp_lds[SpmvTile<T>::kMaxRows + 2];
    const int b = blockIdx.x;
    int j = 0, lo = 0, hi = at.begin[1];
#pragma unroll
    for (int q = 1; q < kSpmvBatchMax; ++q)
        if (b >= at.begin[q]) {
            j = q;
            lo = at.begin[q];
            hi = at.begin[q + 1];
        }
    const int t = lo + (SWZ ? xcd_swizzle(b - lo, hi - lo) : b - lo);
    const SpmvBatchEntry e = entries[j];
    spmv_tile<T, NT, BETA>(tiles[t], e.rowptr, e.colidx, e.cidx, e.runs, cbases[t], poffs[t], e.cmax,
                           (const T *)e.vals, (const T *)e.x,
                           (T *)e.y, (T *)e.partials, alpha, beta, BETA, e.nnz, e.vector_ok, lds,
                           wsum, rp_lds, hl, fuse);
}

template <typename T>
__global__ __launch_bounds__(64) void spmv_longrow_fixup_batch(
    const SpmvBatchEntry *__restrict__ entries, const SpmvLongRow *__restrict__ lr,
    SpmvBatchTable at, T alpha, T beta, int beta_nonzero) {
    const int i = blockIdx.x;
    int j = 0;
#pragma unroll
    for (int q = 1; q < kSpmvBatchMax; ++q)
        if (i >= at.begin[q]) j = q;
    const SpmvBatchEntry e = entries[j];
    fixup_row<T>(lr[i], (const T *)e.partials, (T *)e.y, alpha, beta, beta_nonzero);
}

template <typename T>
static hipError_t launch_spmv_batch(const SpmvBatchArgs &a, hipStream_t s) {
    const T alpha = (T)a.alpha, beta = (T)a.beta;
    const int bnz = a.beta != 0.0;
    const int ntiles = a.tiles_at.begin[a.count];
    const int fuse = !(a.variant & rsp::kSpmvVariantFixup);
    if (ntiles > 0) {
        const bool nt = !(a.variant & 1), swz = !(a.variant & 8);
        auto kern = bnz ? (nt ? (swz ? spmv_tiles_batch<T, true, true, true>
                                     : spmv_tiles_batch<T, true, true, false>)
                              : (swz ? spmv_tiles_batch<T, false, true, true>
                                     : spmv_tiles_batch<T, false, true, false>))
                        : (nt ? (swz ? spmv_tiles_batch<T, true, false, true>
                                     : spmv_tiles_batch<T, true, false, false>)
                              : (swz ? spmv_tiles_batch<T, false, false, true>
                                     : spmv_tiles_batch<T, false, false, false>));
        hipLaunchKernelGGL(kern, dim3(ntiles), dim3(kSpmvThreads), 0, s, a.entries, a.tiles,
                           a.cbases, a.poffs, a.tiles_at, alpha, beta, fuse);
        const hipError_t e = hipGetLastError();
        if (e != hipSuccess) return e;
    }
    const int nlong = a.longs_at.begin[a.count];
    if (nlong > 0 && !fuse) {
        SpmvBatchTable lt = a.longs_at;
        lt.begin[kSpmvBatchMax] = nlong;
        hipLaunchKernelGGL((spmv_longrow_fixup_batch<T>), dim3(nlong), dim3(64), 0, s,
                           a.entries, a.longrows, lt, alpha, beta, bnz);
        return hipGetLastError();
    }
    return hipSuccess;
}

hipError_t spmv_batch_f32(const SpmvBatchArgs &a, hipStream_t s) {
    return launch_spmv_batch<float>(a, s);
}

template <typename T>
static hipError_t launch_spmv(const SpmvArgs &a, hipStream_t s) {
    if (a.nblocks <= 0) return hipSuccess;
    const T alpha = (T)a.alpha, beta = (T)a.beta;
    const int bnz = a.beta != 0.0;
    const int fuse = !(a.variant & rsp::kSpmvVariantFixup);
    auto kern = (a.variant & 1) ? (bnz ? spmv_tiles<T, false, true> : spmv_tiles<T, false, false>)
                                : (bnz ? spmv_tiles<T, true, true> : spmv_tiles<T, true, false>);
    hipLaunchKernelGGL(kern, dim3(a.nblocks), dim3(kSpmvThreads), 0, s, a.rowptr, a.colidx,
                       (const T *)a.vals, (const T *)a.x, (T *)a.y, a.blocks, a.nblocks, a.cbases,
                       a.poffs, a.cidx, a.runs, a.cmax, (T *)a.partials, alpha, beta, bnz, a.nnz, a.vector_ok, fuse);
    hipError_t e = hipGetLastError();
    if (e != hipSuccess) return e;
    if (a.nlong > 0 && !fuse) {
        hipLaunchKernelGGL((spmv_longrow_fixup<T>), dim3(a.nlong), dim3(64), 0, s,
                           a.longrows, a.nlong, (const T *)a.partials, (T *)a.y, alpha, beta, bnz);
        e = hipGetLastError();
    }
    return e;
}

hipError_t spmv_f32(const SpmvArgs &a, hipStream_t s) { return launch_spmv<float>(a, s); }
void warm_spmv() {
    hipFuncAttributes at;
    (void)hipFuncGetAttributes(&at, reinterpret_cast<const void *>(spmv_tiles<float, true, false>));
    int o = 0;
    (void)hipOccupancyMaxActiveBlocksPerMultiprocessor(&o, spmv_tiles<float, true, false>, kSpmvThreads, 0);
}

#ifndef RSP_FTZ_BUILD
int spmv_tiles_per_cu(int elem_bytes) {
    int o = 0;
    const hipError_t e =
        elem_bytes == 8
            ? hipOccupancyMaxActiveBlocksPerMultiprocessor(&o, spmv_tiles<double, true, false>, kSpmvThreads, 0)
            : hipOccupancyMaxActiveBlocksPerMultiprocessor(&o, spmv_tiles<float, true, false>, kSpmvThreads, 0);
    return (e == hipSuccess && o > 0) ? o : 1;
}

template <typename E>
__global__ __launch_bounds__(256) void gather_kernel(const int64_t *__restrict__ idx,
                                                     const E *__restrict__ src, E *__restrict__ dst,
                                                     int64_t n) {
    const int64_t stride = (int64_t)gridDim.x * 256;
    for (int64_t i = (int64_t)blockIdx.x * 256 + threadIdx.x; i < n; i += stride) dst[i] = src[idx[i]];
}

template <typename E>
__global__ __launch_bounds__(256) void scatter_kernel(const int64_t *__restrict__ idx,
                                                      const E *__restrict__ src, E *__restrict__ dst,
                                                      int64_t n) {
    const int64_t stride = (int64_t)gridDim.x * 256;
    for (int64_t i = (int64_t)blockIdx.x * 256 + threadIdx.x; i < n; i += stride) dst[idx[i]] = src[i];
}

hipError_t scatter(int elem_bytes, int64_t n, const int64_t *idx, const void *src, void *dst,
                   hipStream_t s) {
    if (n <= 0) return hipSuccess;
    const int64_t want = (n + 255) / 256;
    const int grid = (int)(want < 2048 ? want : 2048);
    if (elem_bytes == 8)
        hipLaunchKernelGGL((scatter_kernel<double>), dim3(grid), dim3(256), 0, s, idx,
                           (const double *)src, (double *)dst, n);
    else
        hipLaunchKernelGGL((scatter_kernel<float>), dim3(grid), dim3(256), 0, s, idx,
                           (const float *)src, (float *)dst, n);
    return hipGetLastError();
}

hipError_t gather(int elem_bytes, int64_t n, const int64_t *idx, const void *src, void *dst,
                  hipStream_t s) {
    if (n <= 0) return hipSuccess;
    const int64_t want = (n + 255) / 256;
    const int grid = (int)(want < 2048 ? want : 2048);
    if (elem_bytes == 8)
        hipLaunchKernelGGL((gather_kernel<double>), dim3(grid), dim3(256), 0, s, idx,
                           (const double *)src, (double *)dst, n);
    else
        hipLaunchKernelGGL((gather_kernel<float>), dim3(grid), dim3(256), 0, s, idx,
                           (const float *)src, (float *)dst, n);
    return hipGetLastError();
}

hipError_t spmv_f64(const SpmvArgs &a, hipStream_t s) { return launch_spmv<double>(a, s); }
hipError_t spmv_batch_f64(const SpmvBatchArgs &a, hipStream_t s) {
    return launch_spmv_batch<double>(a, s);
}
#endif

}
```

respasol_amd/csrc/spmv_pack.h:

```cpp
#pragma once

#include <stdint.h>

#if defined(__HIPCC__)
#define RSP_PK_HD __host__ __device__ __forceinline__
#else
#define RSP_PK_HD inline
#endif

namespace rsp_pack {

constexpr int kBits = 12;
constexpr uint32_t kMask = (1u << kBits) - 1;

constexpr int words_per_thread(int fields) { return fields * kBits / 32; }
static_assert(words_per_thread(8) == 3 && words_per_thread(16) == 6, "fp64 / fp32 geometry");

constexpr int index_words(int nth, int fields) { return nth * words_per_thread(fields); }
RSP_PK_HD int row_words(int nrows) { return (nrows + 2) >> 1; }

RSP_PK_HD bool eligible(int nth, int fields, int len) {
    return (long long)index_words(nth, fields) * 4 < 2LL * len;
}

RSP_PK_HD uint32_t get_field(const uint32_t *w, int f) {
    const int b = f * kBits, i = b >> 5, s = b & 31;
    uint32_t v = w[i] >> s;
    if (s > 32 - kBits) v |= w[i + 1] << (32 - s);
    return v & kMask;
}

RSP_PK_HD void put_field(uint32_t *w, int f, uint32_t slot) {
    const int b = f * kBits, i = b >> 5, s = b & 31;
    slot &= kMask;
    w[i] |= slot << s;
    if (s > 32 - kBits) w[i + 1] |= slot >> (32 - s);
}

inline void pack_slots(const uint16_t *c16, int k0, int k1, int vw, int it_n, int nth, uint32_t *out) {
    const int fields = it_n * vw, nw = words_per_thread(fields);
    const int kb = k0 & ~(vw - 1);
    for (int i = 0; i < nth * nw; i++) out[i] = 0;
    for (int tid = 0; tid < nth; tid++)
        for (int it = 0; it < it_n; it++)
            for (int j = 0; j < vw; j++) {
                const long long e = (long long)kb + (long long)(it * nth + tid) * vw + j;
                if (e >= k0 && e < k1) put_field(out + (size_t)tid * nw, it * vw + j, c16[e]);
            }
}

inline uint32_t unpack_slot(const uint32_t *rec, int k0, int e, int vw, int it_n, int nth) {
    const int fields = it_n * vw, nw = words_per_thread(fields);
    const int kb = k0 & ~(vw - 1);
    const int v = (e - kb) / vw, j = (e - kb) % vw;
    const int it = v / nth, tid = v % nth;
    return get_field(rec + (size_t)tid * nw, it * vw + j);
}

inline void pack_rows(const int *rp, int r0, int nrows, int kb, uint32_t *out) {
    const int n = row_words(nrows);
    for (int i = 0; i < n; i++) out[i] = 0;
    for (int i = 0; i <= nrows; i++) out[i >> 1] |= (uint32_t)(uint16_t)(rp[r0 + i] - kb) << (16 * (i & 1));
}

inline int unpack_row(const uint32_t *rows, int i) { return (int)((rows[i >> 1] >> (16 * (i & 1))) & 0xffffu); }

}
```

respasol_amd/csrc/spmv_plan.cpp:

```cpp

#include "spmv_plan.h"
#include "spmv_pack.h"

#include <algorithm>
#include <atomic>
#include <vector>

namespace rsp_plan {

using rsp::SpmvTile;

namespace {

size_t align256(size_t x) { return (x + 255) & ~(size_t)255; }

struct TileGeom {
    int cap, chunk, maxrows;
    int ucap;
    bool list;
    int vw, iw;
    int xelem;
};
template <typename T>
TileGeom geom_of() {
    using S = SpmvTile<T>;
    return {S::kMaxNnz, S::kChunk, S::kMaxRows, S::kStageSlots, S::kStageList, S::kVec,
            rsp_pack::index_words(rsp::kSpmvThreads, rsp::kSpmvIter * S::kVec), (int)sizeof(T)};
}
TileGeom geom(rsp_datatype_t t) { return t == RSP_R_64F ? geom_of<double>() : geom_of<float>(); }

SpmvBounds spmv_bounds(int64_t rows, int64_t nnz, int cap) {
    SpmvBounds b;
    size_t q = (size_t)(nnz / cap) + 1;
    size_t l = (size_t)(nnz / rsp::kSpmvLongRow) + 1;
    b.nlong = q;
    b.nslots = 2 * q + 1;
    b.nblocks = 6 * q + 2 * l + (size_t)(rows / rsp::kSpmvMaxRows) + 8;
    b.nblocks += std::min<size_t>(b.nblocks, 8192);
    return b;
}

}

SpmvLayout spmv_layout(const SpmvBounds &b, size_t elem, int64_t nnz, size_t run_ints) {
    SpmvLayout l;
    l.off_long = align256(b.nblocks * sizeof(SpmvBlock));
    l.off_part = l.off_long + align256(b.nlong * sizeof(SpmvLongRow));
    l.off_cbase = l.off_part + align256(b.nslots * 2 * elem);
    l.off_poff = l.off_cbase + align256(b.nblocks * sizeof(int));
    l.off_cidx = l.off_poff + align256(b.nblocks * sizeof(int));
    l.off_runs = l.off_cidx + align256((size_t)std::max<int64_t>(nnz, 0) * sizeof(uint16_t));
    l.bytes = l.off_runs + align256(run_ints * sizeof(int));
    return l;
}

PlanOptions plan_options(rsp_datatype_t type) {
    using rsp_an::env_int;
    PlanOptions o;
    o.type = type;
    o.stage_list = env_int("RSP_SPMV_STAGE_LIST", 1);
    o.list_cap = env_int("RSP_SPMV_LIST_CAP", o.list_cap);
    o.stage_pct = std::min(std::max(env_int("RSP_SPMV_STAGE_PCT", 80), 0), 100);
    o.pack_mode = std::min(std::max(env_int("RSP_SPMV_PACK", 2), 0), 2);
    return o;
}

RowPlan build_spmv_plan(const int *rp, int m, int cap, int chunk, int maxrows, int row_align) {
    RowPlan out;
    hvec<SpmvBlock> &blocks = out.blocks;
    int slots = 0;
    int r = 0;
    while (r < m) {
        int len = rp[r + 1] - rp[r];
        if (len > rsp::kSpmvLongRow) {
            if (len <= chunk) {
                SpmvBlock b;
                b.r0 = r;
                b.r1 = rsp::kSpmvWholeRow;
                b.k0 = rp[r];
                b.k1 = rp[r + 1];
                blocks.push_back(b);
                r++;
                continue;
            }
            SpmvLongRow lr;
            lr.row = r;
            lr.first = slots;
            lr.nchunks = 0;
            lr.pad = 0;
            for (int k = rp[r]; k < rp[r + 1]; k += chunk) {
                SpmvBlock b;
                b.r0 = r;
                b.r1 = -(slots + 1);
                b.k0 = k;
                b.k1 = std::min(k + chunk, rp[r + 1]);
                blocks.push_back(b);
                slots++;
                lr.nchunks++;
            }
            out.longrows.push_back(lr);
            r++;
            continue;
        }
        int start = r, nnz = 0;
        while (r < m && r - start < maxrows) {
            int l = rp[r + 1] - rp[r];
            if (l > rsp::kSpmvLongRow || (r > start && nnz + l > cap)) break;
            nnz += l;
            r++;
        }
        if (row_align > 1 && r < m && r % row_align != 0) {
            const int ra = r - r % row_align;
            if (ra > start && (int64_t)(rp[ra] - rp[start]) * 4 >= (int64_t)(rp[r] - rp[start]) * 3) r = ra;
        }
        SpmvBlock b;
        b.r0 = start;
        b.r1 = r;
        b.k0 = rp[start];
        b.k1 = rp[r];
        blocks.push_back(b);
    }
    out.nslots = slots;
    return out;
}

namespace {

RowPlan pack_rows(const int *rp, int m, int cap, const TileGeom &g, const PlanOptions &o) {
    return build_spmv_plan(rp, m, cap, g.chunk, g.maxrows, o.row_align);
}

void respread(const int *rp, int m, int64_t nnz_bound, const TileGeom &g, const PlanOptions &o, RowPlan &p) {
    const SpmvBounds bb = spmv_bounds(m, std::max<int64_t>(nnz_bound, 0), g.chunk);
    const int64_t nnz_s = rp[(size_t)m];
    int c = (int)std::max<int64_t>(64, std::min<int64_t>(g.cap, (nnz_s + o.spread - 1) / o.spread));
    for (int tries = 0; tries < 32 && c < g.cap; tries++) {
        RowPlan p2 = pack_rows(rp, m, c, g, o);
        if ((int64_t)p2.blocks.size() <= o.spread && p2.blocks.size() <= bb.nblocks) {
            p = std::move(p2);
            break;
        }
        c += std::max(8, c / 16);
    }
}

int distinct_cols(const int *ci, int k0, int k1, std::vector<int> &cols) {
    cols.assign(ci + k0, ci + k1);
    std::sort(cols.begin(), cols.end());
    cols.erase(std::unique(cols.begin(), cols.end()), cols.end());
    int R = 1;
    for (size_t u = 1; u < cols.size(); u++) R += cols[u] != cols[u - 1] + 1;
    return R;
}

bool list_tiles_ok(const TileGeom &g, const PlanOptions &o) {
    return o.use_stage && o.use_c16 && g.list && o.stage_list != 0;
}

void list_repack(const int *rp, const int *ci, int m, const TileGeom &g, const PlanOptions &o, RowPlan &p) {
    int64_t band = 0, all = 0;
    std::vector<int> cols;
    const size_t step = std::max<size_t>(1, p.blocks.size() / 64);
    for (size_t t = 0; t < p.blocks.size(); t += step) {
        const SpmvBlock &bk = p.blocks[t];
        if (bk.r1 < 0 || bk.k1 <= bk.k0) continue;
        const int R = distinct_cols(ci, bk.k0, bk.k1, cols);
        all += bk.k1 - bk.k0;
        if (cols.back() - cols.front() <= 65535 && R > rsp::kStageRuns && (int)cols.size() > g.ucap)
            band += bk.k1 - bk.k0;
    }
    if (2 * band > all) p = pack_rows(rp, m, std::min(g.cap, std::min(std::max(o.list_cap, 64), g.ucap)), g, o);
}

bool interior_tile(const SpmvBlock &b, const int *ci, int64_t local_cols) {
    if (b.r1 < 0) return false;
    for (int k = b.k0; k < b.k1; k++)
        if (ci[(size_t)k] >= local_cols) return false;
    return true;
}
int partition_interior(const int *ci, int64_t local_cols, hvec<SpmvBlock> &blocks) {
    auto mid = std::stable_partition(blocks.begin(), blocks.end(),
                                     [&](const SpmvBlock &b) { return interior_tile(b, ci, local_cols); });
    return (int)(mid - blocks.begin());
}

enum class TileKind { Int32, Gather16, Runs, List };
TileKind classify_tile(const SpmvBlock &bk, const int *ci, const TileGeom &g, const PlanOptions &o,
                       std::vector<int> &cols, int *lo_out, int *R_out) {
    int lo = ci[(size_t)bk.k0], hi = lo;
    for (int k = bk.k0 + 1; k < bk.k1; k++) {
        lo = std::min(lo, ci[(size_t)k]);
        hi = std::max(hi, ci[(size_t)k]);
    }
    *lo_out = lo;
    if (hi - lo > 65535) return TileKind::Int32;
    const bool x_in_rsrc = ((int64_t)hi + 1) * g.xelem <= (int64_t)0x7ffffffc;
    if (!o.use_stage || bk.r1 < 0 || !x_in_rsrc) return TileKind::Gather16;
    const int len = bk.k1 - bk.k0;
    const int R = *R_out = distinct_cols(ci, bk.k0, bk.k1, cols);
    const int U = (int)cols.size();
    if (U <= g.ucap && R <= rsp::kStageRuns && 100LL * U <= (long long)o.stage_pct * len) return TileKind::Runs;
    if (list_tiles_ok(g, o) && U <= g.ucap && R > rsp::kStageRuns) return TileKind::List;
    return TileKind::Gather16;
}

void encode_columns(const int *ci, int64_t nnz_s, const TileGeom &g, const PlanOptions &o, TilePlan &p) {
    p.c16.assign((size_t)nnz_s, 0);
    const long long nt = (long long)p.blocks.size();
    std::vector<std::vector<int>> truns(o.use_stage ? (size_t)nt : 0);
    std::vector<char> tlist(o.use_stage ? (size_t)nt : 0, 0);
    std::atomic<int64_t> n16{0}, nst{0};
    rsp_an::parallel_for(nt, 64, [&](long long t0, long long t1) {
        std::vector<int> cols;
        int64_t c16n = 0, stn = 0;
        for (long long t = t0; t < t1; t++) {
            const SpmvBlock &bk = p.blocks[(size_t)t];
            if (bk.k1 <= bk.k0) continue;
            int lo = 0, R = 0;
            const TileKind kind = classify_tile(bk, ci, g, o, cols, &lo, &R);
            if (kind == TileKind::Int32) continue;
            const int len = bk.k1 - bk.k0;
            c16n += len;
            if (kind == TileKind::Gather16) {
                p.cbase[(size_t)t] = lo;
                for (int k = bk.k0; k < bk.k1; k++) p.c16[(size_t)k] = (uint16_t)(ci[(size_t)k] - lo);
                continue;
            }
            const int U = (int)cols.size();
            std::vector<int> &r = truns[(size_t)t];
            tlist[(size_t)t] = kind == TileKind::List;
            if (kind == TileKind::Runs) {
                r.reserve(2 * (size_t)(R + 1));
                for (int u = 0; u < U; u++)
                    if (u == 0 || cols[(size_t)u] != cols[(size_t)u - 1] + 1) {
                        r.push_back(cols[(size_t)u]);
                        r.push_back(u);
                    }
                r.push_back(0);
                r.push_back(U);
            } else {
                r.assign(2 + 2 * (size_t)((U + 3) / 4), 0);
                r[0] = cols[0];
                r[1] = U;
                uint16_t *ofs = reinterpret_cast<uint16_t *>(r.data() + 2);
                for (int u = 0; u < U; u++) ofs[u] = (uint16_t)(cols[(size_t)u] - cols[0]);
            }
            for (int k = bk.k0; k < bk.k1; k++)
                p.c16[(size_t)k] =
                    (uint16_t)(std::lower_bound(cols.begin(), cols.end(), ci[(size_t)k]) - cols.begin());
            stn += len;
        }
        n16 += c16n;
        nst += stn;
    });
    p.nnz_c16 = n16;
    p.nnz_staged = nst;
    for (size_t t = 0; t < truns.size(); t++) {
        const std::vector<int> &r = truns[t];
        if (r.empty()) continue;
        const int64_t off = (int64_t)p.runs.size() / 2;
        if (off >= kStageOffLimit) {
            p.nnz_c16 -= p.blocks[t].k1 - p.blocks[t].k0;
            p.nnz_staged -= p.blocks[t].k1 - p.blocks[t].k0;
            continue;
        }
        p.cbase[t] = stage_encode(off, tlist[t] ? kStageListCode : (int)r.size() / 2 - 1);
        p.runs.insert(p.runs.end(), r.begin(), r.end());
    }
}

void pack_staged_tiles(const int *rp, const TileGeom &g, int mode, TilePlan &p) {
    constexpr int IT = rsp::kSpmvIter, NTH = rsp::kSpmvThreads;
    const int VW = g.vw, IW = g.iw;
    if (mode <= 0) return;
    int64_t end = ((int64_t)p.runs.size() + 3) & ~(int64_t)3;
    for (size_t t = 0; t < p.blocks.size(); t++) {
        const SpmvBlock &b = p.blocks[t];
        if (!staged(p.cbase[t]) || b.r1 < 0 || !rsp_pack::eligible(NTH, IT * VW, b.k1 - b.k0)) continue;
        const int64_t words = IW + (mode >= 2 ? rsp_pack::row_words(b.r1 - b.r0) : 0);
        if (end + words >= kPackWordLimit) break;
        p.poff[t] = pack_encode(end, mode >= 2);
        end = (end + words + 3) & ~(int64_t)3;
        p.tiles_packed++;
        p.nnz_packed += b.k1 - b.k0;
    }
    if (p.tiles_packed == 0) return;
    p.runs.resize((size_t)end + 4, 0);
    rsp_an::parallel_for((long long)p.blocks.size(), 64, [&](long long t0, long long t1) {
        for (long long t = t0; t < t1; t++) {
            if (p.poff[(size_t)t] == kNoPack) continue;
            const SpmvBlock &b = p.blocks[(size_t)t];
            const PackCode pc = pack_decode(p.poff[(size_t)t]);
            uint32_t *rec = reinterpret_cast<uint32_t *>(p.runs.data()) + pc.word;
            rsp_pack::pack_slots(p.c16.data(), b.k0, b.k1, VW, IT, NTH, rec);
            if (pc.rows) rsp_pack::pack_rows(rp, b.r0, b.r1 - b.r0, b.k0 & ~(VW - 1), rec + IW);
        }
    });
}

}

void make_tile_plan(const int *rp, const int *ci, int m, int64_t nnz_bound, const PlanOptions &o, TilePlan &p) {
    const TileGeom g = geom(o.type);
    RowPlan &rows = p;
    rows = pack_rows(rp, m, g.cap, g, o);
    const size_t nb = p.blocks.size();
    if (o.spread > 0 && nb > 0 && (int64_t)nb < o.spread) respread(rp, m, nnz_bound, g, o, rows);
    if (list_tiles_ok(g, o) && p.blocks.size() == nb && nb > 0) list_repack(rp, ci, m, g, o, rows);
    p.nint = o.local_cols >= 0 ? partition_interior(ci, o.local_cols, p.blocks) : 0;
    const int64_t nnz_s = m > 0 ? rp[(size_t)m] : 0;
    p.cbase.assign(p.blocks.size(), kCbaseInt32);
    p.c16.clear();
    p.runs.clear();
    p.poff.assign(p.blocks.size(), kNoPack);
    p.tiles_packed = p.nnz_packed = 0;
    p.nnz_c16 = 0;
    p.nnz_staged = 0;
    if (o.use_c16 && nnz_s > 0 && nnz_s <= nnz_bound) {
        encode_columns(ci, nnz_s, g, o, p);
        if (o.use_stage) pack_staged_tiles(rp, g, o.pack_mode, p);
    }
}

void plan_stats(const TilePlan &p, rsp_datatype_t type, int64_t out[8]) {
    const TileGeom g = geom(type);
    int64_t nstaged = 0, idx = 0, desc = 0, rows16 = 0, rowptr = 0;
    for (size_t t = 0; t < p.blocks.size(); t++) {
        const SpmvBlock &b = p.blocks[t];
        const int cb = p.cbase[t], po = p.poff[t];
        const int64_t len = b.k1 - b.k0, nrows = b.r1 > b.r0 ? b.r1 - b.r0 : 0;
        idx += po != kNoPack ? 4LL * g.iw : cb == kCbaseInt32 ? 4 * len : 2 * len;
        if (staged(cb)) {
            const StageCode sc = stage_decode(cb);
            nstaged++;
            desc += sc.list() ? 8 + 2LL * p.runs[2 * (size_t)sc.off + 1] : 8LL * (sc.nr + 1);
        }
        if (po != kNoPack && pack_decode(po).rows)
            rows16 += 4LL * rsp_pack::row_words((int)nrows);
        else
            rowptr += 4 * (nrows + 1);
    }
    out[0] = (int64_t)p.blocks.size();
    out[1] = p.tiles_packed;
    out[2] = p.nnz_packed;
    out[3] = 24 * (int64_t)p.blocks.size() + idx + desc + rows16;
    out[4] = rowptr;
    out[5] = nstaged;
    out[6] = idx;
    out[7] = rows16;
}

namespace {

bool verify_split(const int *ci, const PlanOptions &o, const TilePlan &p) {
    const size_t nt = p.blocks.size(), nint = (size_t)p.nint;
    if (p.nint < 0 || nint > nt || (o.local_cols < 0 && nint != 0)) return false;
    for (size_t t = 0; t < nt; t++) {
        const SpmvBlock &b = p.blocks[t];
        if (o.local_cols >= 0 && t <= nint && interior_tile(b, ci, o.local_cols) != (t < nint)) return false;
        if (t == 0 || t == nint) continue;
        const SpmvBlock &a = p.blocks[t - 1];
        if (a.r0 > b.r0 || (a.r0 == b.r0 && a.k0 >= b.k0)) return false;
    }
    return true;
}

}

bool plan_verify(const int *rp, const int *ci, int m, const PlanOptions &o, const TilePlan &p) {
    const TileGeom g = geom(o.type);
    const int vw = g.vw, iw = g.iw;
    const int nnz_s = m > 0 ? rp[m] : 0;
    if (p.poff.size() != p.blocks.size() || p.cbase.size() != p.blocks.size()) return false;
    if (!p.c16.empty() && p.c16.size() != (size_t)nnz_s) return false;
    int64_t npk = 0, epk = 0;
    for (size_t t = 0; t < p.blocks.size(); t++) {
        const SpmvBlock &b = p.blocks[t];
        const int cb = p.cbase[t], po = p.poff[t];
        if (b.r0 < 0 || b.r0 >= m || (b.r1 >= 0 && (b.r1 < b.r0 || b.r1 > m))) return false;
        if (b.k0 < 0 || b.k1 < b.k0 || b.k1 > nnz_s) return false;
        if (cb != kCbaseInt32 && p.c16.empty() && b.k1 > b.k0) return false;
        if (!o.use_c16 && cb != kCbaseInt32) return false;
        if (!o.use_stage && (staged(cb) || po != kNoPack)) return false;
        const uint32_t *rec = nullptr;
        if (po != kNoPack) {
            const PackCode pc = pack_decode(po);
            const int nrows = b.r1 - b.r0, kb = b.k0 & ~(vw - 1);
            const size_t words = (size_t)iw + (pc.rows ? rsp_pack::row_words(nrows) : 0);
            if (po < 0 || !staged(cb) || b.r1 < 0 || o.pack_mode == 0 || pc.rows != (o.pack_mode >= 2) ||
                !rsp_pack::eligible(rsp::kSpmvThreads, rsp::kSpmvIter * vw, b.k1 - b.k0) || (pc.word & 3) ||
                pc.word + words > p.runs.size())
                return false;
            rec = reinterpret_cast<const uint32_t *>(p.runs.data()) + pc.word;
            const int nwt = iw / rsp::kSpmvThreads;
            for (int tid = 0; tid < rsp::kSpmvThreads; tid++)
                for (int f = 0; f < rsp::kSpmvIter * vw; f++) {
                    const long long e = (long long)kb + (long long)((f / vw) * rsp::kSpmvThreads + tid) * vw + f % vw;
                    if ((e < b.k0 || e >= b.k1) && rsp_pack::get_field(rec + (size_t)tid * nwt, f) != 0) return false;
                }
            if (pc.rows)
                for (int i = 0; i <= nrows; i++)
                    if (rsp_pack::unpack_row(rec + iw, i) + kb != rp[b.r0 + i]) return false;
            npk++;
            epk += b.k1 - b.k0;
        }
        auto slot_of = [&](int k) {
            return rec ? (int)rsp_pack::unpack_slot(rec, b.k0, k, vw, rsp::kSpmvIter, rsp::kSpmvThreads)
                       : (int)p.c16[(size_t)k];
        };
        if (cb == kCbaseInt32 || b.k1 <= b.k0) continue;
        const StageCode sc = staged(cb) ? stage_decode(cb) : StageCode{0, 0};
        const int off = sc.off, nr = sc.nr;
        const int *r = nullptr;
        const uint16_t *ofs = nullptr;
        int U = 0;
        if (staged(cb) && sc.list()) {
            if (o.type != RSP_R_64F) return false;
            if ((size_t)2 * off + 2 > p.runs.size()) return false;
            r = p.runs.data() + 2 * (size_t)off;
            U = r[1];
            if (U < 1 || U > g.ucap || (size_t)2 * off + 2 + 2 * (size_t)((U + 3) / 4) > p.runs.size()) return false;
            ofs = reinterpret_cast<const uint16_t *>(r + 2);
            for (int u = 1; u < U; u++)
                if (ofs[u] <= ofs[u - 1]) return false;
        } else if (staged(cb)) {
            if (nr < 1 || nr > rsp::kStageRuns || (size_t)2 * (off + nr + 1) > p.runs.size()) return false;
            r = p.runs.data() + 2 * (size_t)off;
            U = r[2 * nr + 1];
            if (r[1] != 0 || U > g.ucap) return false;
            for (int j = 1; j <= nr; j++)
                if (r[2 * j + 1] <= r[2 * j - 1] ||
                    (j < nr && r[2 * j] <= r[2 * j - 2] + (r[2 * j + 1] - r[2 * j - 1]) - 1))
                    return false;
        }
        for (int k = b.k0; k < b.k1; k++) {
            int col;
            if (cb >= 0) {
                col = cb + p.c16[(size_t)k];
            } else {
                const int u = slot_of(k);
                if (u >= U) return false;
                int j = 0;
                while (!ofs && j + 1 < nr && r[2 * (j + 1) + 1] <= u) j++;
                col = ofs ? r[0] + ofs[u] : r[2 * j] + (u - r[2 * j + 1]);
            }
            if (col != ci[k]) return false;
        }
    }
    return npk == p.tiles_packed && epk == p.nnz_packed && verify_split(ci, o, p);
}

uint64_t digest(const TilePlan &p) {
    rsp_an::Fnv f;
    f.vec(p.blocks);
    f.vec(p.longrows);
    f.bytes(&p.nslots, sizeof(p.nslots));
    f.bytes(&p.nint, sizeof(p.nint));
    f.vec(p.cbase);
    f.vec(p.c16);
    f.vec(p.runs);
    f.vec(p.poff);
    for (const int64_t c : {p.nnz_c16, p.nnz_staged, p.tiles_packed, p.nnz_packed}) f.bytes(&c, sizeof(c));
    return f.h;
}

}
```

respasol_amd/csrc/spmv_plan.h:

```cpp
#ifndef RSP_SPMV_PLAN_H
#define RSP_SPMV_PLAN_H

#include <stddef.h>
#include <stdint.h>

#include "rsp.h"
#include "host_pool.h"
#include "rsp_kernels.h"

namespace rsp_plan {

using rsp::SpmvBlock;
using rsp::SpmvLongRow;
using rsp_an::hvec;


constexpr int kCbaseInt32 = -1;
constexpr int kStageListCode = 255;
constexpr int64_t kStageOffLimit = 1LL << 22;
struct StageCode {
    int off, nr;
    bool list() const { return nr == kStageListCode; }
};
inline bool staged(int cbase) { return cbase <= -2; }
inline int stage_encode(int64_t off, int nr) { return -2 - (int)((off << 8) | nr); }
inline StageCode stage_decode(int cbase) { return {(-2 - cbase) >> 8, (-2 - cbase) & 255}; }

constexpr int kNoPack = -1;
constexpr int64_t kPackWordLimit = 1LL << 30;
struct PackCode {
    size_t word;
    int rows;
};
inline int pack_encode(int64_t word, int rows) { return (int)(word << 1) | rows; }
inline PackCode pack_decode(int poff) { return {(size_t)(poff >> 1), poff & 1}; }

struct SpmvBounds {
    size_t nblocks, nlong, nslots;
};

struct SpmvLayout {
    size_t off_long, off_part, off_cbase, off_poff, off_cidx, off_runs, bytes;
};
SpmvLayout spmv_layout(const SpmvBounds &b, size_t elem, int64_t nnz, size_t run_ints = 0);

struct PlanOptions {
    rsp_datatype_t type = RSP_R_64F;
    int64_t spread = 0;
    int64_t local_cols = -1;
    int row_align = 1;
    bool use_c16 = true;
    bool use_stage = true;
    int stage_list = 1;
    int list_cap = 1 << 30;
    int stage_pct = 80;
    int pack_mode = 2;
};
PlanOptions plan_options(rsp_datatype_t type);

struct RowPlan {
    hvec<SpmvBlock> blocks;
    hvec<SpmvLongRow> longrows;
    int nslots = 0;
};
RowPlan build_spmv_plan(const int *rp, int m, int cap, int chunk, int maxrows, int row_align);

struct TilePlan : RowPlan {
    int nint = 0;
    hvec<int> cbase;
    hvec<uint16_t> c16;
    hvec<int> runs;
    hvec<int> poff;
    int64_t nnz_c16 = 0;
    int64_t nnz_staged = 0;
    int64_t tiles_packed = 0, nnz_packed = 0;
};

void make_tile_plan(const int *rp, const int *ci, int m, int64_t nnz_bound, const PlanOptions &o, TilePlan &p);

bool plan_verify(const int *rp, const int *ci, int m, const PlanOptions &o, const TilePlan &p);

void plan_stats(const TilePlan &p, rsp_datatype_t type, int64_t out[8]);

uint64_t digest(const TilePlan &p);

}

#endif
```

respasol_amd/drivers/spmv_pack_check.cpp:

```cpp
#include <stdint.h>
#include <stdio.h>

#include <vector>

#include "spmv_pack.h"

namespace {

constexpr int kThreads = 256, kIter = 4;

uint32_t rng_state = 12345u;
uint32_t rnd() {
    rng_state = rng_state * 1664525u + 1013904223u;
    return rng_state >> 8;
}

int check_tile(int vw, int k0, int len, int maxrow, int nslots) {
    const int fields = kIter * vw, k1 = k0 + len, kb = k0 & ~(vw - 1);
    const int total = k1 + 7;
    std::vector<uint16_t> c16((size_t)total);
    for (int e = 0; e < total; e++) c16[(size_t)e] = (uint16_t)(rnd() % (uint32_t)nslots);
    if (kb + kThreads * fields < k1) {
        printf("FAIL: tile of %d entries at %d does not fit %d slots\n", len, k0, kThreads * fields);
        return 1;
    }
    std::vector<int> rp(1, k0);
    for (int l = 1; rp.back() < k1; l = l % maxrow + 1) rp.push_back(rp.back() + l < k1 ? rp.back() + l : k1);
    const int nrows = (int)rp.size() - 1;
    const int iw = rsp_pack::index_words(kThreads, fields);
    std::vector<uint32_t> rec((size_t)iw + (size_t)rsp_pack::row_words(nrows));
    rsp_pack::pack_slots(c16.data(), k0, k1, vw, kIter, kThreads, rec.data());
    rsp_pack::pack_rows(rp.data(), 0, nrows, kb, rec.data() + iw);
    for (int e = k0; e < k1; e++)
        if (rsp_pack::unpack_slot(rec.data(), k0, e, vw, kIter, kThreads) != c16[(size_t)e]) {
            printf("FAIL: vw %d k0 %d len %d: slot of entry %d\n", vw, k0, len, e);
            return 1;
        }
    const int nw = rsp_pack::words_per_thread(fields);
    for (int tid = 0; tid < kThreads; tid++)
        for (int f = 0; f < fields; f++) {
            const int e = kb + ((f / vw) * kThreads + tid) * vw + f % vw;
            const uint32_t got = rsp_pack::get_field(rec.data() + (size_t)tid * nw, f);
            const uint32_t want = e >= k0 && e < k1 ? c16[(size_t)e] : 0u;
            if (got != want) {
                printf("FAIL: vw %d k0 %d len %d: thread %d field %d = %u, want %u\n", vw, k0, len, tid, f, got, want);
                return 1;
            }
        }
    for (int i = 0; i <= nrows; i++)
        if (rsp_pack::unpack_row(rec.data() + iw, i) + kb != rp[(size_t)i]) {
            printf("FAIL: vw %d k0 %d len %d: row offset %d\n", vw, k0, len, i);
            return 1;
        }
    return 0;
}

}

int main() {
    int bad = 0, n = 0;
    bad += rsp_pack::eligible(kThreads, 8, 1536) || !rsp_pack::eligible(kThreads, 8, 1537);
    bad += rsp_pack::eligible(kThreads, 16, 3072) || !rsp_pack::eligible(kThreads, 16, 3073);
    if (bad) printf("FAIL: eligibility edge\n");
    struct Geo { int vw, cap, nslots; } geos[2] = {{2, 2047, 1536}, {4, 4093, 2048}};
    for (const Geo &g : geos) {
        const int lens[] = {1, g.vw, g.cap / 2, g.cap / 2 + 1, 3 * g.cap / 4, 3 * g.cap / 4 + 1, g.cap - 1, g.cap};
        for (int len : lens)
            for (int k0 = 0; k0 < 2 * g.vw; k0++)
                for (int maxrow : {1, 9, 256}) {
                    bad += check_tile(g.vw, k0 + 4096 * (len & 3), len, maxrow, g.nslots);
                    n++;
                }
    }
    bad += check_tile(2, 5, 2047, 9, 4096);
    bad += check_tile(4, 7, 4093, 9, 4096);
    printf("%s: %d tiles\n", bad ? "FAILED" : "ok", n + 2);
    return bad ? 1 : 0;
}
```

respasol_amd/sparse.py:

```python
from __future__ import annotations

import ctypes as C

import numpy as np
import torch

from . import _lib
from ._lib import RspError, check, rsp

_DT = {torch.float64: _lib.R_64F, torch.float32: _lib.R_32F}


def _ptr(t: torch.Tensor | None) -> C.c_void_p:
    return C.c_void_p(t.data_ptr() if t is not None and t.numel() > 0 else 0)


def _scalar(value: float, dtype: torch.dtype):
    return C.c_double(value) if dtype == torch.float64 else C.c_float(value)


class Handle:

    def __init__(self, stream: torch.cuda.Stream | None = None, ftz: bool = False):
        if not torch.cuda.is_available():
            raise RuntimeError("respasol_amd.sparse needs a HIP device (MI355X, gfx950)")
        self._h = C.c_void_p()
        check(rsp.rsp_create(C.byref(self._h)), "rsp_create")
        self.set_stream(stream if stream is not None else torch.cuda.current_stream())
        self.set_ftz(ftz)

    @property
    def ptr(self) -> C.c_void_p:
        return self._h

    def set_stream(self, stream: torch.cuda.Stream) -> None:
        self.stream = stream
        check(rsp.rsp_set_stream(self._h, C.c_void_p(stream.cuda_stream)), "rsp_set_stream")

    def set_ftz(self, on: bool) -> None:
        self.ftz = bool(on)
        check(rsp.rsp_set_ftz(self._h, 1 if on else 0), "rsp_set_ftz")

    def close(self) -> None:
        if self._h:
            rsp.rsp_destroy(self._h)
            self._h = C.c_void_p()

    def __del__(self):
        try:
            self.close()
        except Exception:
            pass


def upload_csr(rowptr: np.ndarray, colidx: np.ndarray, values: np.ndarray,
               dtype: torch.dtype = torch.float64, device: str | torch.device = "cuda"):
    np_dt = np.float64 if dtype == torch.float64 else np.float32
    rp = torch.from_numpy(np.ascontiguousarray(rowptr, np.int32)).to(device)
    ci = torch.from_numpy(np.ascontiguousarray(colidx, np.int32)).to(device)
    va = torch.from_numpy(np.ascontiguousarray(values).astype(np_dt)).to(device)
    return rp, ci, va


class SpMat:

    def __init__(self, handle: Handle, rowptr: torch.Tensor, colidx: torch.Tensor,
                 values: torch.Tensor, n_cols: int, nnz: int | None = None):
        if values.dtype not in _DT:
            raise TypeError("values must be float64 or float32")
        if rowptr.dtype != torch.int32 or colidx.dtype != torch.int32:
            raise TypeError("rowptr/colidx must be int32 (CUSPARSE_INDEX_32I)")
        self.handle = handle
        self.rowptr, self.colidx, self.values = rowptr, colidx, values
        self.m = rowptr.numel() - 1
        self.n = int(n_cols)
        self.dtype = values.dtype
        self.nnz = int(nnz if nnz is not None else colidx.numel())
        self._mat = C.c_void_p()
        check(rsp.rsp_create_csr(C.byref(self._mat), self.m, self.n, self.nnz, _ptr(rowptr),
                                 _ptr(colidx), _ptr(values), _DT[self.dtype]), "rsp_create_csr")
        one, zero = _scalar(1.0, self.dtype), _scalar(0.0, self.dtype)
        size = C.c_size_t()
        check(rsp.rsp_spmv_buffer_size(handle.ptr, _lib.OP_N, C.byref(one), self._mat,
                                       C.byref(zero), _DT[self.dtype], C.byref(size)),
              "rsp_spmv_buffer_size")
        self.buffer = torch.empty(max(int(size.value), 1), dtype=torch.uint8, device=values.device)

    @property
    def nnz_stored(self) -> int:
        return int(self.colidx.numel())

    def spmv(self, x: torch.Tensor, y: torch.Tensor | None = None, alpha: float = 1.0,
             beta: float = 0.0) -> torch.Tensor:
        if x.dtype != self.dtype or x.numel() < self.n:
            raise ValueError("x has the wrong dtype or length")
        if y is None:
            y = torch.empty(self.m, dtype=self.dtype, device=x.device)
        a, b = _scalar(alpha, self.dtype), _scalar(beta, self.dtype)
        check(rsp.rsp_spmv(self.handle.ptr, _lib.OP_N, C.byref(a), self._mat, _ptr(x), C.byref(b),
                           _ptr(y), _DT[self.dtype], _ptr(self.buffer)), "rsp_spmv")
        return y

    def bind(self, x: torch.Tensor, y: torch.Tensor, alpha: float = 1.0, beta: float = 0.0):
        if x.dtype != self.dtype or x.numel() < self.n or y.dtype != self.dtype or y.numel() < self.m:
            raise ValueError("x / y have the wrong dtype or length")
        a, b = _scalar(alpha, self.dtype), _scalar(beta, self.dtype)
        args = (self.handle.ptr, _lib.OP_N, C.byref(a), self._mat, _ptr(x), C.byref(b), _ptr(y),
                _DT[self.dtype], _ptr(self.buffer))
        keep = (a, b, x, y)
        fn = rsp.rsp_spmv

        def call():
            st = fn(*args)
            if st:
                check(st, "rsp_spmv")
        call.keep = keep
        return call

    def set_values(self, values: torch.Tensor) -> None:
        if values.dtype not in _DT:
            raise TypeError("values must be float64 or float32")
        if values.numel() < self.nnz_stored:
            raise ValueError("values is shorter than the pattern")
        check(rsp.rsp_csr_set_values(self._mat, _ptr(values), _DT[values.dtype]), "rsp_csr_set_values")
        self.values = values
        self.dtype = values.dtype

    def set_local_cols(self, ncols_local: int) -> None:
        check(rsp.rsp_spmat_set_local_cols(self._mat, int(ncols_local)), "rsp_spmat_set_local_cols")
        one, zero = _scalar(1.0, self.dtype), _scalar(0.0, self.dtype)
        check(rsp.rsp_spmv_preprocess(self.handle.ptr, _lib.OP_N, C.byref(one), self._mat, None,
                                      C.byref(zero), None, _DT[self.dtype], _ptr(self.buffer)),
              "rsp_spmv_preprocess")

    def plan_info(self) -> dict:
        t, e = C.c_int64(), C.c_int64()
        check(rsp.rsp_spmv_plan_info(self._mat, C.byref(t), C.byref(e)), "rsp_spmv_plan_info")
        return {"tiles": t.value, "entries_16bit": e.value}

    def spmv_part(self, x: torch.Tensor, y: torch.Tensor, part: int, alpha: float = 1.0) -> torch.Tensor:
        if x.dtype != self.dtype or x.numel() < self.n:
            raise ValueError("x has the wrong dtype or length")
        a, b = _scalar(alpha, self.dtype), _scalar(0.0, self.dtype)
        check(rsp.rsp_spmv_part(self.handle.ptr, C.byref(a), self._mat, _ptr(x), C.byref(b), _ptr(y),
                                _DT[self.dtype], _ptr(self.buffer), int(part)), "rsp_spmv_part")
        return y

    def close(self) -> None:
        if self._mat:
            rsp.rsp_destroy_spmat(self._mat)
            self._mat = C.c_void_p()

    def __del__(self):
        try:
            self.close()
        except Exception:
            pass


PLAN_STATS = ("tiles", "packed_tiles", "packed_entries", "schedule_bytes", "rowptr_bytes", "staged_tiles",
              "index_bytes", "packed_rowoff_bytes")


def spmv_plan_stats(rowptr, colidx, fp32: bool = False, nnz: int | None = None) -> dict:
    import numpy as np

    rp = np.ascontiguousarray(rowptr, np.int32)
    ci = np.ascontiguousarray(colidx, np.int32)
    out = (C.c_int64 * len(PLAN_STATS))()
    check(rsp.rsp_spmv_plan_stats(len(rp) - 1, rp.ctypes.data, ci.ctypes.data,
                                  int(nnz if nnz is not None else len(ci)), 1 if fp32 else 0, out),
          "rsp_spmv_plan_stats")
    return dict(zip(PLAN_STATS, (int(v) for v in out)))


class SpmvBatch:

    def __init__(self, handle: Handle, mats: list[SpMat], xs: list[torch.Tensor],
                 ys: list[torch.Tensor], part: int = 0):
        if not (len(mats) == len(xs) == len(ys)):
            raise ValueError("mats, xs and ys must have the same length")
        dt = mats[0].dtype if mats else torch.float64
        for A, x, y in zip(mats, xs, ys):
            if A.dtype != dt or x.dtype != dt or y.dtype != dt:
                raise ValueError("one compute type per batch")
            if x.numel() < A.n or y.numel() < A.m:
                raise ValueError("x or y too short")
        self.handle, self.dtype, self.part = handle, dt, int(part)
        self._keep = (list(mats), list(xs), list(ys))
        n = len(mats)
        arr = C.c_void_p * max(n, 1)
        self._b = C.c_void_p()
        check(rsp.rsp_spmv_batch_create(
            handle.ptr, n, arr(*[A._mat.value for A in mats]), arr(*[x.data_ptr() for x in xs]),
            arr(*[y.data_ptr() for y in ys]), arr(*[A.buffer.data_ptr() for A in mats]),
            _DT[dt], self.part, C.byref(self._b)), "rsp_spmv_batch_create")

    def run(self, alpha: float = 1.0, beta: float = 0.0) -> None:
        a, b = _scalar(alpha, self.dtype), _scalar(beta, self.dtype)
        check(rsp.rsp_spmv_batch_run(self.handle.ptr, self._b, C.byref(a), C.byref(b)),
              "rsp_spmv_batch_run")

    def info(self) -> dict:
        t, e = C.c_int64(), C.c_int64()
        check(rsp.rsp_spmv_batch_info(self._b, C.byref(t), C.byref(e)), "rsp_spmv_batch_info")
        return {"tiles": t.value, "entries_16bit": e.value}

    def close(self) -> None:
        if self._b:
            rsp.rsp_spmv_batch_destroy(self._b)
            self._b = C.c_void_p()

    def __del__(self):
        try:
            self.close()
        except Exception:
            pass


class Ilu0:

    def __init__(self, handle: Handle, rowptr: torch.Tensor, colidx: torch.Tensor,
                 nnz: int | None = None):
        self.handle = handle
        self.rowptr, self.colidx = rowptr, colidx
        self.n = rowptr.numel() - 1
        self.nnz = int(nnz if nnz is not None else colidx.numel())
        self._info = C.c_void_p()
        check(rsp.rsp_create_ilu0_info(C.byref(self._info)), "rsp_create_ilu0_info")

    def analysis(self) -> None:
        check(rsp.rsp_ilu0_analysis(self.handle.ptr, self.n, self.nnz, _ptr(self.rowptr),
                                    _ptr(self.colidx), self._info), "rsp_ilu0_analysis")

    def trsv_analysis(self, transpose: bool = False) -> None:
        op = _lib.OP_T if transpose else _lib.OP_N
        check(rsp.rsp_trsv_analysis(self.handle.ptr, op, self._info), "rsp_trsv_analysis")

    def zero_pivot(self) -> int:
        pos = C.c_int(-1)
        st = rsp.rsp_ilu0_zero_pivot(self.handle.ptr, self._info, C.byref(pos))
        if st == _lib.STATUS_ZERO_PIVOT:
            return pos.value
        check(st, "rsp_ilu0_zero_pivot")
        return -1

    TRSV_L, TRSV_LT, TRSV_U = 0, 1, 2

    def solve_zero_pivot(self, which: int) -> int:
        pos = C.c_int(-1)
        st = rsp.rsp_trsv_zero_pivot(self.handle.ptr, self._info, which, C.byref(pos))
        if st == _lib.STATUS_ZERO_PIVOT:
            return pos.value
        check(st, "rsp_trsv_zero_pivot")
        return -1

    def levels(self) -> tuple[int, int]:
        lo, up = C.c_int(), C.c_int()
        check(rsp.rsp_ilu0_levels(self._info, C.byref(lo), C.byref(up)), "rsp_ilu0_levels")
        return lo.value, up.value

    def solve_blocks(self) -> tuple[int, int]:
        lo, up = C.c_int(), C.c_int()
        check(rsp.rsp_ilu0_solve_blocks(self._info, C.byref(lo), C.byref(up)), "rsp_ilu0_solve_blocks")
        return lo.value, up.value

    def factor(self, values: torch.Tensor) -> None:
        check(rsp.rsp_ilu0_factor(self.handle.ptr, self._info, _DT[values.dtype], _ptr(values)),
              "rsp_ilu0_factor")

    def solve_lower(self, values: torch.Tensor, x: torch.Tensor, y: torch.Tensor | None = None,
                    transpose: bool = False, alpha: float = 1.0) -> torch.Tensor:
        if y is None:
            y = torch.empty_like(x)
        a = _scalar(alpha, values.dtype)
        check(rsp.rsp_trsv_lower_unit(self.handle.ptr, _lib.OP_T if transpose else _lib.OP_N,
                                      C.byref(a), self._info, _DT[values.dtype], _ptr(values),
                                      _ptr(x), _ptr(y)), "rsp_trsv_lower_unit")
        return y

    def solve_upper(self, values: torch.Tensor, x: torch.Tensor, y: torch.Tensor | None = None,
                    alpha: float = 1.0) -> torch.Tensor:
        if y is None:
            y = torch.empty_like(x)
        a = _scalar(alpha, values.dtype)
        check(rsp.rsp_trsv_upper(self.handle.ptr, C.byref(a), self._info, _DT[values.dtype],
                                 _ptr(values), _ptr(x), _ptr(y)), "rsp_trsv_upper")
        return y

    def close(self) -> None:
        if self._info:
            rsp.rsp_destroy_ilu0_info(self._info)
            self._info = C.c_void_p()

    def __del__(self):
        try:
            self.close()
        except Exception:
            pass


class SolveResult:

    __slots__ = ("x", "iters", "relres", "reason", "history")

    def __init__(self, x, iters, relres, reason, history):
        self.x, self.iters, self.relres, self.reason, self.history = x, iters, relres, reason, history

    @property
    def converged(self) -> bool:
        return self.reason == _lib.SOLVE_CONVERGED

    def __repr__(self) -> str:
        return (f"SolveResult(iters={self.iters}, relres={self.relres:.3e}, "
                f"reason={self.reason}, n={self.x.numel()})")


class BiCGStab:

    CONVERGED, MAX_ITERS, BREAKDOWN = _lib.SOLVE_CONVERGED, _lib.SOLVE_MAX_ITERS, _lib.SOLVE_BREAKDOWN

    def __init__(self, handle: Handle, A: SpMat, ilu: Ilu0 | None = None,
                 factor: torch.Tensor | None = None):
        if ilu is not None and factor is None:
            raise ValueError("an ILU(0) preconditioner needs its factored values")
        if factor is not None and factor.dtype not in _DT:
            raise TypeError("factor must be float64 or float32")
        self.handle, self.A, self.ilu, self.factor = handle, A, ilu, factor
        self.dtype = A.dtype
        self._s = C.c_void_p()
        check(rsp.rsp_bicgstab_create(handle.ptr, A._mat, ilu._info if ilu is not None else None,
                                      _DT[factor.dtype] if ilu is not None else _DT[A.dtype],
                                      _ptr(factor) if ilu is not None else None, C.byref(self._s)),
              "rsp_bicgstab_create")

    def solve(self, b: torch.Tensor, x0: torch.Tensor | None = None, rtol: float = 1e-10,
              max_iters: int = 1000, check_every: int = 1) -> SolveResult:
        if b.dtype != self.dtype or b.numel() != self.A.m:
            raise ValueError("b has the wrong dtype or length")
        if x0 is not None and (x0.dtype != self.dtype or x0.numel() != self.A.m):
            raise ValueError("x0 has the wrong dtype or length")
        with torch.cuda.stream(self.handle.stream):
            x = torch.zeros_like(b) if x0 is None else x0.clone()
        iters, reason, rel = C.c_int(), C.c_int(), C.c_double()
        check(rsp.rsp_bicgstab_solve(self.handle.ptr, self._s, _ptr(b), _ptr(x), float(rtol),
                                     int(max_iters), int(check_every), C.byref(iters), C.byref(rel),
                                     C.byref(reason)), "rsp_bicgstab_solve")
        count = C.c_int()
        check(rsp.rsp_bicgstab_history(self._s, 0, None, C.byref(count)), "rsp_bicgstab_history")
        hist = (C.c_double * max(count.value, 1))()
        check(rsp.rsp_bicgstab_history(self._s, count.value, hist, C.byref(count)), "rsp_bicgstab_history")
        return SolveResult(x, iters.value, rel.value, reason.value, list(hist[:count.value]))

    def close(self) -> None:
        if self._s:
            rsp.rsp_bicgstab_destroy(self._s)
            self._s = C.c_void_p()

    def __del__(self):
        try:
            self.close()
        except Exception:
            pass


class GMRES:

    CONVERGED, MAX_ITERS, BREAKDOWN = _lib.SOLVE_CONVERGED, _lib.SOLVE_MAX_ITERS, _lib.SOLVE_BREAKDOWN

    def __init__(self, handle: Handle, A: SpMat, ilu: Ilu0 | None = None,
                 factor: torch.Tensor | None = None, restart: int = 30):
        if ilu is not None and factor is None:
            raise ValueError("an ILU(0) preconditioner needs its factored values")
        if factor is not None and factor.dtype not in _DT:
            raise TypeError("factor must be float64 or float32")
        self.handle, self.A, self.ilu, self.factor = handle, A, ilu, factor
        self.dtype = A.dtype
        self.restart = int(restart)
        self._s = C.c_void_p()
        check(rsp.rsp_gmres_create(handle.ptr, A._mat, ilu._info if ilu is not None else None,
                                   _DT[factor.dtype] if ilu is not None else _DT[A.dtype],
                                   _ptr(factor) if ilu is not None else None, self.restart,
                                   C.byref(self._s)), "rsp_gmres_create")

    def solve(self, b: torch.Tensor, x0: torch.Tensor | None = None, rtol: float = 1e-10,
              max_iters: int = 1000, check_every: int = 1) -> SolveResult:
        if b.dtype != self.dtype or b.numel() != self.A.m:
            raise ValueError("b has the wrong dtype or length")
        if x0 is not None and (x0.dtype != self.dtype or x0.numel() != self.A.m):
            raise ValueError("x0 has the wrong dtype or length")
        with torch.cuda.stream(self.handle.stream):
            x = torch.zeros_like(b) if x0 is None else x0.clone()
        iters, reason, rel = C.c_int(), C.c_int(), C.c_double()
        check(rsp.rsp_gmres_solve(self.handle.ptr, self._s, _ptr(b), _ptr(x), float(rtol), int(max_iters),
                                  int(check_every), C.byref(iters), C.byref(rel), C.byref(reason)),
              "rsp_gmres_solve")
        count = C.c_int()
        check(rsp.rsp_gmres_history(self._s, 0, None, C.byref(count)), "rsp_gmres_history")
        hist = (C.c_double * max(count.value, 1))()
        check(rsp.rsp_gmres_history(self._s, count.value, hist, C.byref(count)), "rsp_gmres_history")
        return SolveResult(x, iters.value, rel.value, reason.value, list(hist[:count.value]))

    def close(self) -> None:
        if self._s:
            rsp.rsp_gmres_destroy(self._s)
            self._s = C.c_void_p()

    def __del__(self):
        try:
            self.close()
        except Exception:
            pass


def dot(handle: Handle, x: torch.Tensor, y: torch.Tensor) -> float:
    if x.dtype != y.dtype or x.dtype not in _DT or x.numel() != y.numel():
        raise ValueError("dot: x and y must share dtype (float64 / float32) and length")
    r = C.c_double()
    check(rsp.rsp_dot(handle.ptr, _DT[x.dtype], x.numel(), C.c_void_p(x.data_ptr()),
                      C.c_void_p(y.data_ptr()), C.byref(r)), "rsp_dot")
    return r.value


def orthogonalize(handle: Handle, V: torch.Tensor, w: torch.Tensor) -> np.ndarray:
    if V.dim() != 2 or w.dim() != 1 or V.dtype != w.dtype or V.dtype not in _DT or V.shape[1] != w.numel():
        raise ValueError("orthogonalize: V must be (k, n) and w (n,), one dtype (float64 / float32)")
    if V.shape[1] > 1 and V.stride(1) != 1:
        raise ValueError("orthogonalize: the rows of V must have unit stride")
    k, n = V.shape
    ldv = V.stride(0) if k > 1 else max(n, 1)
    h = np.zeros(k + 1)
    check(rsp.rsp_orthogonalize(handle.ptr, _DT[V.dtype], n, k, C.c_void_p(V.data_ptr()), ldv,
                                C.c_void_p(w.data_ptr()), h.ctypes.data_as(C.POINTER(C.c_double))),
          "rsp_orthogonalize")
    return h


def gather(handle: Handle, idx: torch.Tensor, src: torch.Tensor, dst: torch.Tensor) -> None:
    if idx.dtype != torch.int64 or src.dtype != dst.dtype or dst.numel() < idx.numel():
        raise ValueError("gather: bad arguments")
    check(rsp.rsp_gather(handle.ptr, _DT[src.dtype], idx.numel(), _ptr(idx), _ptr(src), _ptr(dst)),
          "rsp_gather")


def scatter(handle: Handle, idx: torch.Tensor, src: torch.Tensor, dst: torch.Tensor) -> None:
    if idx.dtype != torch.int64 or src.dtype != dst.dtype or src.numel() < idx.numel():
        raise ValueError("scatter: bad arguments")
    check(rsp.rsp_scatter(handle.ptr, _DT[src.dtype], idx.numel(), _ptr(idx), _ptr(src), _ptr(dst)),
          "rsp_scatter")


__all__ = ["Handle", "SpMat", "Ilu0", "BiCGStab", "GMRES", "SolveResult", "dot", "orthogonalize", "upload_csr",
           "gather", "scatter", "RspError"]
```

Before: 1035 GFLOP/s.

## Merge per-tile block, cbase and poff into one 32-byte head record

Tile metadata is restructured so each tile's block bounds, cbase and poff are stored together in one 32-byte aligned SpmvHead. The kernel now reads its tile header with a single load instead of three separate arrays. A new pack mode 3 also lets a packed record carry its own run descriptors inline with the packed indices, so staged tiles touch fewer cache lines. This mode is only used when RSP_SPMV_PACK=3 is set. Batch regions are aligned to 64 bytes, and a host-side cache-line counting API is added. The costs are larger per-tile metadata and more plan complexity.

```diff
diff --git a/include/rsp.h b/include/rsp.h
--- a/include/rsp.h
+++ b/include/rsp.h
@@ -152,6 +152,8 @@
                                 int64_t *entries_staged);
 rsp_status_t rsp_spmv_plan_stats(int m, const int *row_offsets, const int *col_ind, int64_t nnz,
                                  rsp_datatype_t compute_type, int64_t stats[8]);
+rsp_status_t rsp_spmv_plan_lines(int m, const int *row_offsets, const int *col_ind, int64_t nnz,
+                                 rsp_datatype_t compute_type, int64_t lines[5], uint64_t *digest);
 rsp_status_t rsp_ilu0_plan_digest(rsp_ilu0_info_t info, uint64_t *digest);
 
 #ifdef __cplusplus
diff --git a/respasol_amd/_lib.py b/respasol_amd/_lib.py
--- a/respasol_amd/_lib.py
+++ b/respasol_amd/_lib.py
@@ -120,6 +120,7 @@
     "rsp_ilu0_analysis_host": (i32, [i32, vp, vp, vp, vp, vp, vp]),
     "rsp_spmv_plan_host": (i32, [i32, vp, vp, C.c_int64, i32, vp, vp, vp]),
     "rsp_spmv_plan_stats": (i32, [i32, vp, vp, C.c_int64, i32, vp]),
+    "rsp_spmv_plan_lines": (i32, [i32, vp, vp, C.c_int64, i32, vp, vp]),
     "rsp_ilu0_plan_digest": (i32, [vp, vp]),
 }
 
diff --git a/respasol_amd/csrc/rsp_api.cpp b/respasol_amd/csrc/rsp_api.cpp
--- a/respasol_amd/csrc/rsp_api.cpp
+++ b/respasol_amd/csrc/rsp_api.cpp
@@ -56,6 +56,12 @@
             if ((unsigned)c >= (unsigned)ncols) return RSP_STATUS_INVALID_VALUE;
     }
     return RSP_STATUS_SUCCESS;
+}
+
+static rsp_an::hvec<rsp::SpmvHead> tile_heads(const TilePlan &p, size_t t0, size_t t1) {
+    rsp_an::hvec<rsp::SpmvHead> heads(t1 - t0);
+    for (size_t t = t0; t < t1; t++) heads[t - t0] = {p.blocks[t], p.cbase[t], p.poff[t], {0, 0}};
+    return heads;
 }
 
 rsp_status_t rsp_api::spmv_plan(rsp_handle_t h, rsp_spmat_t mat, rsp_datatype_t compute_type) {
@@ -91,9 +97,8 @@
     auto upload = [&](size_t off, const void *src, size_t bytes) {
         return bytes == 0 ? hipSuccess : hipMemcpyAsync(buf + off, src, bytes, hipMemcpyHostToDevice, h->stream);
     };
-    RSP_CHECK_HIP(upload(0, p.blocks.data(), p.blocks.size() * sizeof(SpmvBlock)));
-    RSP_CHECK_HIP(upload(lay.off_cbase, p.cbase.data(), p.cbase.size() * sizeof(int)));
-    RSP_CHECK_HIP(upload(lay.off_poff, p.poff.data(), p.poff.size() * sizeof(int)));
+    const rsp_an::hvec<rsp::SpmvHead> heads = tile_heads(p, 0, p.blocks.size());
+    RSP_CHECK_HIP(upload(0, heads.data(), heads.size() * sizeof(rsp::SpmvHead)));
     RSP_CHECK_HIP(upload(lay.off_cidx, p.c16.data(), p.c16.size() * sizeof(uint16_t)));
     RSP_CHECK_HIP(upload(lay.off_runs, p.runs.data(), p.runs.size() * sizeof(int)));
     RSP_CHECK_HIP(upload(lay.off_long, p.longrows.data(), p.longrows.size() * sizeof(SpmvLongRow)));
@@ -135,10 +140,8 @@
     a.vals = mat->vals;
     a.x = d_x;
     a.y = d_y;
-    a.blocks = (const SpmvBlock *)plan;
+    a.heads = (const rsp::SpmvHead *)plan;
     a.nblocks = mat->nblocks;
-    a.cbases = (const int *)(plan + mat->lay.off_cbase);
-    a.poffs = (const int *)(plan + mat->lay.off_poff);
     a.cidx = (const unsigned short *)(plan + mat->lay.off_cidx);
     a.runs = (const int *)(plan + mat->lay.off_runs);
     a.cmax = mat->cols > 0 ? (int)(mat->cols - 1) : 0;
@@ -158,9 +161,7 @@
             a.nblocks = mat->nint;
             a.nlong = 0;
         } else {
-            a.blocks += mat->nint;
-            a.cbases += mat->nint;
-            a.poffs += mat->nint;
+            a.heads += mat->nint;
             a.nblocks = mat->nblocks - mat->nint;
         }
     }
@@ -220,7 +221,7 @@
     struct Span {
         int first, count, nt, nl;
         rsp_an::hvec<Region> reg;
-        enum { kEntries, kTiles, kCbases, kPoffs, kLongRows, kC16, kRuns, kPartials };
+        enum { kEntries, kHeads, kLongRows, kC16, kRuns, kPartials };
         const Region &at(int kind, int q) const { return reg[kind < kC16 ? kind : kC16 + (kind - kC16) * count + q]; }
     };
     rsp_an::hvec<Span> spans;
@@ -264,9 +265,7 @@
             sp.nl += part == 1 ? 0 : (int)p.longrows.size();
         }
         sp.reg = {{0, (size_t)sp.count * sizeof(rsp::SpmvBatchEntry)},
-                  {0, (size_t)sp.nt * sizeof(SpmvBlock)},
-                  {0, (size_t)sp.nt * sizeof(int)},
-                  {0, (size_t)sp.nt * sizeof(int)},
+                  {0, (size_t)sp.nt * sizeof(rsp::SpmvHead)},
                   {0, (size_t)sp.nl * sizeof(SpmvLongRow)}};
         for (int q = 0; q < sp.count; q++) sp.reg.push_back({0, plans[first + q].c16.size() * sizeof(uint16_t)});
         for (int q = 0; q < sp.count; q++) sp.reg.push_back({0, plans[first + q].runs.size() * sizeof(int)});
@@ -274,7 +273,7 @@
             sp.reg.push_back({0, (size_t)plans[first + q].nslots * 2 * elem_size(compute_type)});
         for (Region &r : sp.reg) {
             r.off = bytes;
-            bytes += (r.len + 15) & ~(size_t)15;
+            bytes += (r.len + 63) & ~(size_t)63;
         }
         spans.push_back(sp);
     }
@@ -300,9 +299,7 @@
         };
         rsp::SpmvBatchArgs a{};
         a.entries = (const rsp::SpmvBatchEntry *)dev(Span::kEntries);
-        a.tiles = (const SpmvBlock *)dev(Span::kTiles);
-        a.cbases = (const int *)dev(Span::kCbases);
-        a.poffs = (const int *)dev(Span::kPoffs);
+        a.heads = (const rsp::SpmvHead *)dev(Span::kHeads);
         a.longrows = (const SpmvLongRow *)dev(Span::kLongRows);
         a.count = sp.count;
         for (int q = 0; q <= rsp::kSpmvBatchMax; q++)
@@ -333,9 +330,8 @@
                 if (p.cbase[(size_t)t] != rsp_plan::kCbaseInt32)
                     b->entries_16bit += p.blocks[(size_t)t].k1 - p.blocks[(size_t)t].k0;
             b->tiles += (int64_t)ntq;
-            put(Span::kTiles, 0, nt * sizeof(SpmvBlock), p.blocks.data() + t0, ntq * sizeof(SpmvBlock));
-            put(Span::kCbases, 0, nt * sizeof(int), p.cbase.data() + t0, ntq * sizeof(int));
-            put(Span::kPoffs, 0, nt * sizeof(int), p.poff.data() + t0, ntq * sizeof(int));
+            const rsp_an::hvec<rsp::SpmvHead> heads = tile_heads(p, (size_t)t0, (size_t)t1);
+            put(Span::kHeads, 0, nt * sizeof(rsp::SpmvHead), heads.data(), ntq * sizeof(rsp::SpmvHead));
             put(Span::kLongRows, 0, nl * sizeof(SpmvLongRow), p.longrows.data(), nlq * sizeof(SpmvLongRow));
             put(Span::kC16, q, 0, p.c16.data(), p.c16.size() * sizeof(uint16_t));
             put(Span::kRuns, q, 0, p.runs.data(), p.runs.size() * sizeof(int));
@@ -654,6 +650,19 @@
     });
 }
 
+rsp_status_t rsp_spmv_plan_lines(int m, const int *row_offsets, const int *col_ind, int64_t nnz,
+                                 rsp_datatype_t compute_type, int64_t lines[5], uint64_t *digest) {
+    return guarded([&] {
+        if (m < 0 || (m > 0 && (!row_offsets || !col_ind)) || !lines) return RSP_STATUS_INVALID_VALUE;
+        if (compute_type != RSP_R_64F && compute_type != RSP_R_32F) return RSP_STATUS_NOT_SUPPORTED;
+        TilePlan p;
+        rsp_plan::make_tile_plan(row_offsets, col_ind, m, nnz, rsp_plan::plan_options(compute_type), p);
+        rsp_plan::plan_lines(p, compute_type, lines);
+        if (digest) *digest = rsp_plan::digest(p);
+        return RSP_STATUS_SUCCESS;
+    });
+}
+
 rsp_status_t rsp_spmv_plan_stats(int m, const int *row_offsets, const int *col_ind, int64_t nnz,
                                  rsp_datatype_t compute_type, int64_t stats[8]) {
     return guarded([&] {
diff --git a/respasol_amd/csrc/rsp_kernels.h b/respasol_amd/csrc/rsp_kernels.h
--- a/respasol_amd/csrc/rsp_kernels.h
+++ b/respasol_amd/csrc/rsp_kernels.h
@@ -8,6 +8,13 @@
 struct alignas(16) SpmvBlock {
     int r0, r1, k0, k1;
 };
+
+struct alignas(32) SpmvHead {
+    SpmvBlock blk;
+    int cbase, poff;
+    int pad[2];
+};
+static_assert(sizeof(SpmvHead) == 32, "one head is one 32-byte scalar load");
 
 struct alignas(16) SpmvLongRow {
     int row, first, nchunks, pad;
@@ -50,12 +57,10 @@
     const void *vals;
     const void *x;
     void *y;
-    const SpmvBlock *blocks;
+    const SpmvHead *heads;
     int nblocks;
-    const int *cbases;
     const unsigned short *cidx;
     const int *runs;
-    const int *poffs;
     int cmax;
     const SpmvLongRow *longrows;
     int nlong;
@@ -85,9 +90,7 @@
 };
 struct SpmvBatchArgs {
     const SpmvBatchEntry *entries;
-    const SpmvBlock *tiles;
-    const int *cbases;
-    const int *poffs;
+    const SpmvHead *heads;
     const SpmvLongRow *longrows;
     int count;
     SpmvBatchTable tiles_at, longs_at;
diff --git a/respasol_amd/csrc/spmv.hip b/respasol_amd/csrc/spmv.hip
--- a/respasol_amd/csrc/spmv.hip
+++ b/respasol_amd/csrc/spmv.hip
@@ -20,6 +20,7 @@
 using rsp::kSpmvHeavyMax;
 using rsp::SpmvArgs;
 using rsp::SpmvBlock;
+using rsp::SpmvHead;
 using rsp::SpmvLongRow;
 using rsp::SpmvTile;
 using rsp::kSpmvBatchMax;
@@ -382,6 +383,8 @@
     const int tid = threadIdx.x;
     const int k0 = blk.k0, k1 = blk.k1;
     const bool staged = cbase <= -2;
+    const bool own = staged && poff >= 0 && (poff & 2);
+    const int recw = (poff >> 1) & ~3;
     constexpr int SMAX = SpmvTile<T>::kStageSlots / kSpmvThreads;
     int2 rd = make_int2(0, 0);
     int nr = 0;
@@ -396,15 +399,17 @@
             for (int k = 0; k < SMAX; ++k)
                 if (k * kSpmvThreads < rd.y) lsl[k] = lst[min(k * kSpmvThreads + tid, rd.y - 1)];
         } else if (tid <= nr) {
-            rd = reinterpret_cast<const int2 *>(runs)[(code >> 8) + tid];
+            const int *rdp = own ? runs + recw + rsp_pack::kRecHeadWords : runs + 2 * (code >> 8);
+            rd = reinterpret_cast<const int2 *>(rdp)[tid];
         }
     }
     const int nrows = blk.r1 - blk.r0;
     const int nrows_ld = nrows > 0 ? nrows : 0;
     const bool vec = vector_ok && k1 > k0 && k1 <= (nnz & ~(VW - 1));
     const int kb = vec ? (k0 & ~(VW - 1)) : k0;
-    const unsigned int *rec =
-        vec && staged && poff >= 0 ? reinterpret_cast<const unsigned int *>(runs) + (poff >> 1) : nullptr;
+    const unsigned int *rec = vec && staged && poff >= 0 ? reinterpret_cast<const unsigned int *>(runs) + recw +
+                                                               (own ? rsp_pack::rec_slot_word(nr) : 0)
+                                                         : nullptr;
     const bool prow = rec && (poff & 1);
     const int nrw = (nrows_ld + 2) >> 1;
     const int *rsrc = prow ? reinterpret_cast<const int *>(rec) +
@@ -480,16 +485,15 @@
 template <typename T, bool NT, bool BETA>
 __global__ __launch_bounds__(kSpmvThreads) void spmv_tiles(
     const int *__restrict__ rowptr, const int *__restrict__ colidx, const T *__restrict__ vals,
-    const T *__restrict__ x, T *__restrict__ y, const SpmvBlock *__restrict__ blocks, int nblocks,
-    const int *__restrict__ cbases, const int *__restrict__ poffs, const unsigned short *__restrict__ cidx,
-    const int *__restrict__ runs, int cmax, T *partials, T alpha, T beta, int beta_nonzero, int nnz,
-    int vector_ok, int fuse) {
+    const T *__restrict__ x, T *__restrict__ y, const SpmvHead *__restrict__ heads, int nblocks,
+    const unsigned short *__restrict__ cidx, const int *__restrict__ runs, int cmax, T *partials, T alpha,
+    T beta, int beta_nonzero, int nnz, int vector_ok, int fuse) {
     __shared__ __attribute__((aligned(16))) T lds[SpmvTile<T>::kSlots];
     __shared__ T wsum[kSpmvThreads / 64];
     __shared__ int hl[1 + kSpmvHeavyMax];
     __shared__ __attribute__((aligned(4))) unsigned short rp_lds[SpmvTile<T>::kMaxRows + 2];
-    const int b = xcd_swizzle(blockIdx.x, nblocks);
-    spmv_tile<T, NT, BETA>(blocks[b], rowptr, colidx, cidx, runs, cbases[b], poffs[b], cmax, vals, x, y,
+    const SpmvHead hd = heads[xcd_swizzle(blockIdx.x, nblocks)];
+    spmv_tile<T, NT, BETA>(hd.blk, rowptr, colidx, cidx, runs, hd.cbase, hd.poff, cmax, vals, x, y,
                            partials, alpha, beta, beta_nonzero, nnz, vector_ok, lds, wsum, rp_lds, hl,
                            fuse);
 }
@@ -522,9 +526,8 @@
 
 template <typename T, bool NT, bool BETA, bool SWZ>
 __global__ __launch_bounds__(kSpmvThreads) void spmv_tiles_batch(
-    const SpmvBatchEntry *__restrict__ entries, const SpmvBlock *__restrict__ tiles,
-    const int *__restrict__ cbases, const int *__restrict__ poffs, SpmvBatchTable at, T alpha, T beta,
-    int fuse) {
+    const SpmvBatchEntry *__restrict__ entries, const SpmvHead *__restrict__ heads, SpmvBatchTable at,
+    T alpha, T beta, int fuse) {
     __shared__ __attribute__((aligned(16))) T lds[SpmvTile<T>::kSlots];
     __shared__ T wsum[kSpmvThreads / 64];
     __shared__ int hl[1 + kSpmvHeavyMax];
@@ -540,7 +543,8 @@
         }
     const int t = lo + (SWZ ? xcd_swizzle(b - lo, hi - lo) : b - lo);
     const SpmvBatchEntry e = entries[j];
-    spmv_tile<T, NT, BETA>(tiles[t], e.rowptr, e.colidx, e.cidx, e.runs, cbases[t], poffs[t], e.cmax,
+    const SpmvHead hd = heads[t];
+    spmv_tile<T, NT, BETA>(hd.blk, e.rowptr, e.colidx, e.cidx, e.runs, hd.cbase, hd.poff, e.cmax,
                            (const T *)e.vals, (const T *)e.x,
                            (T *)e.y, (T *)e.partials, alpha, beta, BETA, e.nnz, e.vector_ok, lds,
                            wsum, rp_lds, hl, fuse);
@@ -575,8 +579,8 @@
                                      : spmv_tiles_batch<T, true, false, false>)
                               : (swz ? spmv_tiles_batch<T, false, false, true>
                                      : spmv_tiles_batch<T, false, false, false>));
-        hipLaunchKernelGGL(kern, dim3(ntiles), dim3(kSpmvThreads), 0, s, a.entries, a.tiles,
-                           a.cbases, a.poffs, a.tiles_at, alpha, beta, fuse);
+        hipLaunchKernelGGL(kern, dim3(ntiles), dim3(kSpmvThreads), 0, s, a.entries, a.heads,
+                           a.tiles_at, alpha, beta, fuse);
         const hipError_t e = hipGetLastError();
         if (e != hipSuccess) return e;
     }
@@ -604,8 +608,8 @@
     auto kern = (a.variant & 1) ? (bnz ? spmv_tiles<T, false, true> : spmv_tiles<T, false, false>)
                                 : (bnz ? spmv_tiles<T, true, true> : spmv_tiles<T, true, false>);
     hipLaunchKernelGGL(kern, dim3(a.nblocks), dim3(kSpmvThreads), 0, s, a.rowptr, a.colidx,
-                       (const T *)a.vals, (const T *)a.x, (T *)a.y, a.blocks, a.nblocks, a.cbases,
-                       a.poffs, a.cidx, a.runs, a.cmax, (T *)a.partials, alpha, beta, bnz, a.nnz, a.vector_ok, fuse);
+                       (const T *)a.vals, (const T *)a.x, (T *)a.y, a.heads, a.nblocks, a.cidx, a.runs, a.cmax,
+                       (T *)a.partials, alpha, beta, bnz, a.nnz, a.vector_ok, fuse);
     hipError_t e = hipGetLastError();
     if (e != hipSuccess) return e;
     if (a.nlong > 0 && !fuse) {
diff --git a/respasol_amd/csrc/spmv_pack.h b/respasol_amd/csrc/spmv_pack.h
--- a/respasol_amd/csrc/spmv_pack.h
+++ b/respasol_amd/csrc/spmv_pack.h
@@ -18,6 +18,11 @@
 
 constexpr int index_words(int nth, int fields) { return nth * words_per_thread(fields); }
 RSP_PK_HD int row_words(int nrows) { return (nrows + 2) >> 1; }
+
+constexpr int kRecAlignWords = 16;
+constexpr int kRecHeadWords = 2;
+RSP_PK_HD int rec_slot_word(int nr) { return (kRecHeadWords + 2 * (nr + 1) + 3) & ~3; }
+RSP_PK_HD int rec_words(int nr, int iw, int nrows) { return rec_slot_word(nr) + iw + row_words(nrows); }
 
 RSP_PK_HD bool eligible(int nth, int fields, int len) {
     return (long long)index_words(nth, fields) * 4 < 2LL * len;
diff --git a/respasol_amd/csrc/spmv_plan.cpp b/respasol_amd/csrc/spmv_plan.cpp
--- a/respasol_amd/csrc/spmv_plan.cpp
+++ b/respasol_amd/csrc/spmv_plan.cpp
@@ -44,11 +44,9 @@
 
 SpmvLayout spmv_layout(const SpmvBounds &b, size_t elem, int64_t nnz, size_t run_ints) {
     SpmvLayout l;
-    l.off_long = align256(b.nblocks * sizeof(SpmvBlock));
+    l.off_long = align256(b.nblocks * sizeof(rsp::SpmvHead));
     l.off_part = l.off_long + align256(b.nlong * sizeof(SpmvLongRow));
-    l.off_cbase = l.off_part + align256(b.nslots * 2 * elem);
-    l.off_poff = l.off_cbase + align256(b.nblocks * sizeof(int));
-    l.off_cidx = l.off_poff + align256(b.nblocks * sizeof(int));
+    l.off_cidx = l.off_part + align256(b.nslots * 2 * elem);
     l.off_runs = l.off_cidx + align256((size_t)std::max<int64_t>(nnz, 0) * sizeof(uint16_t));
     l.bytes = l.off_runs + align256(run_ints * sizeof(int));
     return l;
@@ -61,7 +59,7 @@
     o.stage_list = env_int("RSP_SPMV_STAGE_LIST", 1);
     o.list_cap = env_int("RSP_SPMV_LIST_CAP", o.list_cap);
     o.stage_pct = std::min(std::max(env_int("RSP_SPMV_STAGE_PCT", 80), 0), 100);
-    o.pack_mode = std::min(std::max(env_int("RSP_SPMV_PACK", 2), 0), 2);
+    o.pack_mode = std::min(std::max(env_int("RSP_SPMV_PACK", 2), 0), 3);
     return o;
 }
 
@@ -204,7 +202,8 @@
     return TileKind::Gather16;
 }
 
-void encode_columns(const int *ci, int64_t nnz_s, const TileGeom &g, const PlanOptions &o, TilePlan &p) {
+void encode_columns(const int *ci, int64_t nnz_s, const TileGeom &g, const PlanOptions &o, int pack_mode,
+                    TilePlan &p, std::vector<std::vector<int>> &own) {
     p.c16.assign((size_t)nnz_s, 0);
     const long long nt = (long long)p.blocks.size();
     std::vector<std::vector<int>> truns(o.use_stage ? (size_t)nt : 0);
@@ -255,9 +254,16 @@
     });
     p.nnz_c16 = n16;
     p.nnz_staged = nst;
+    own.assign(pack_mode >= 3 ? truns.size() : 0, std::vector<int>());
     for (size_t t = 0; t < truns.size(); t++) {
-        const std::vector<int> &r = truns[t];
+        std::vector<int> &r = truns[t];
         if (r.empty()) continue;
+        if (pack_mode >= 3 && !tlist[t] &&
+            rsp_pack::eligible(rsp::kSpmvThreads, rsp::kSpmvIter * g.vw, p.blocks[t].k1 - p.blocks[t].k0)) {
+            p.cbase[t] = stage_encode(0, (int)r.size() / 2 - 1);
+            own[t] = std::move(r);
+            continue;
+        }
         const int64_t off = (int64_t)p.runs.size() / 2;
         if (off >= kStageOffLimit) {
             p.nnz_c16 -= p.blocks[t].k1 - p.blocks[t].k0;
@@ -269,22 +275,31 @@
     }
 }
 
-void pack_staged_tiles(const int *rp, const TileGeom &g, int mode, TilePlan &p) {
+bool pack_staged_tiles(const int *rp, const TileGeom &g, int mode, TilePlan &p,
+                       const std::vector<std::vector<int>> &own) {
     constexpr int IT = rsp::kSpmvIter, NTH = rsp::kSpmvThreads;
     const int VW = g.vw, IW = g.iw;
-    if (mode <= 0) return;
+    if (mode <= 0) return true;
     int64_t end = ((int64_t)p.runs.size() + 3) & ~(int64_t)3;
     for (size_t t = 0; t < p.blocks.size(); t++) {
         const SpmvBlock &b = p.blocks[t];
         if (!staged(p.cbase[t]) || b.r1 < 0 || !rsp_pack::eligible(NTH, IT * VW, b.k1 - b.k0)) continue;
-        const int64_t words = IW + (mode >= 2 ? rsp_pack::row_words(b.r1 - b.r0) : 0);
-        if (end + words >= kPackWordLimit) break;
-        p.poff[t] = pack_encode(end, mode >= 2);
+        const bool ownrec = t < own.size() && !own[t].empty();
+        int64_t words = IW + (mode >= 2 ? rsp_pack::row_words(b.r1 - b.r0) : 0);
+        if (ownrec) {
+            end = (end + rsp_pack::kRecAlignWords - 1) & ~(int64_t)(rsp_pack::kRecAlignWords - 1);
+            words = rsp_pack::rec_words((int)own[t].size() / 2 - 1, IW, b.r1 - b.r0);
+        }
+        if (end + words >= kPackWordLimit) {
+            if (mode >= 3) return false;
+            break;
+        }
+        p.poff[t] = pack_encode(end, mode >= 2, ownrec);
         end = (end + words + 3) & ~(int64_t)3;
         p.tiles_packed++;
         p.nnz_packed += b.k1 - b.k0;
     }
-    if (p.tiles_packed == 0) return;
+    if (p.tiles_packed == 0) return true;
     p.runs.resize((size_t)end + 4, 0);
     rsp_an::parallel_for((long long)p.blocks.size(), 64, [&](long long t0, long long t1) {
         for (long long t = t0; t < t1; t++) {
@@ -292,10 +307,19 @@
             const SpmvBlock &b = p.blocks[(size_t)t];
             const PackCode pc = pack_decode(p.poff[(size_t)t]);
             uint32_t *rec = reinterpret_cast<uint32_t *>(p.runs.data()) + pc.word;
+            if (pc.own) {
+                const std::vector<int> &r = own[(size_t)t];
+                const int nr = (int)r.size() / 2 - 1;
+                rec[0] = (uint32_t)nr;
+                rec[1] = (uint32_t)(b.r1 - b.r0);
+                std::copy(r.begin(), r.end(), reinterpret_cast<int *>(rec) + rsp_pack::kRecHeadWords);
+                rec += rsp_pack::rec_slot_word(nr);
+            }
             rsp_pack::pack_slots(p.c16.data(), b.k0, b.k1, VW, IT, NTH, rec);
             if (pc.rows) rsp_pack::pack_rows(rp, b.r0, b.r1 - b.r0, b.k0 & ~(VW - 1), rec + IW);
         }
     });
+    return true;
 }
 
 }
@@ -309,17 +333,20 @@
     if (list_tiles_ok(g, o) && p.blocks.size() == nb && nb > 0) list_repack(rp, ci, m, g, o, rows);
     p.nint = o.local_cols >= 0 ? partition_interior(ci, o.local_cols, p.blocks) : 0;
     const int64_t nnz_s = m > 0 ? rp[(size_t)m] : 0;
-    p.cbase.assign(p.blocks.size(), kCbaseInt32);
-    p.c16.clear();
-    p.runs.clear();
-    p.poff.assign(p.blocks.size(), kNoPack);
-    p.tiles_packed = p.nnz_packed = 0;
-    p.nnz_c16 = 0;
-    p.nnz_staged = 0;
-    if (o.use_c16 && nnz_s > 0 && nnz_s <= nnz_bound) {
-        encode_columns(ci, nnz_s, g, o, p);
-        if (o.use_stage) pack_staged_tiles(rp, g, o.pack_mode, p);
-    }
+    auto encode = [&](int mode) {
+        p.cbase.assign(p.blocks.size(), kCbaseInt32);
+        p.c16.clear();
+        p.runs.clear();
+        p.poff.assign(p.blocks.size(), kNoPack);
+        p.tiles_packed = p.nnz_packed = 0;
+        p.nnz_c16 = 0;
+        p.nnz_staged = 0;
+        if (!(o.use_c16 && nnz_s > 0 && nnz_s <= nnz_bound)) return true;
+        std::vector<std::vector<int>> own;
+        encode_columns(ci, nnz_s, g, o, o.use_stage ? mode : 0, p, own);
+        return !o.use_stage || pack_staged_tiles(rp, g, mode, p, own);
+    };
+    if (!encode(o.pack_mode)) encode(2);
 }
 
 void plan_stats(const TilePlan &p, rsp_datatype_t type, int64_t out[8]) {
@@ -348,6 +375,40 @@
     out[5] = nstaged;
     out[6] = idx;
     out[7] = rows16;
+}
+
+void plan_lines(const TilePlan &p, rsp_datatype_t type, int64_t out[5]) {
+    const TileGeom g = geom(type);
+    auto open = [](int64_t a, int64_t b, int64_t &last) {
+        if (b <= a) return (int64_t)0;
+        const int64_t l0 = std::max(a >> 7, last + 1), l1 = (b - 1) >> 7;
+        if (l1 < l0) return (int64_t)0;
+        last = l1;
+        return l1 - l0 + 1;
+    };
+    int64_t last[7] = {-1, -1, -1, -1, -1, -1, -1};
+    for (int k = 0; k < 5; k++) out[k] = 0;
+    for (size_t t = 0; t < p.blocks.size(); t++) {
+        const SpmvBlock &b = p.blocks[t];
+        const int cb = p.cbase[t], po = p.poff[t];
+        const int64_t nrows = b.r1 > b.r0 ? b.r1 - b.r0 : 0;
+        out[0] += open(32 * (int64_t)t, 32 * (int64_t)t + 32, last[0]);
+        out[4] += open(16 * (int64_t)t, 16 * (int64_t)t + 16, last[4]) + open(4 * (int64_t)t, 4 * (int64_t)t + 4, last[5]) +
+                  open(4 * (int64_t)t, 4 * (int64_t)t + 4, last[6]);
+        const PackCode pc = po != kNoPack ? pack_decode(po) : PackCode{0, 0, 0};
+        if (staged(cb) && !pc.own) {
+            const StageCode sc = stage_decode(cb);
+            const int64_t a = 8 * (int64_t)sc.off;
+            out[1] += open(a, a + (sc.list() ? 8 + 2LL * p.runs[2 * (size_t)sc.off + 1] : 8LL * (sc.nr + 1)), last[1]);
+        }
+        if (po != kNoPack) {
+            const int64_t a = 4 * (int64_t)pc.word;
+            const int64_t words = pc.own ? rsp_pack::rec_words(stage_decode(cb).nr, g.iw, (int)nrows)
+                                         : g.iw + (pc.rows ? rsp_pack::row_words((int)nrows) : 0);
+            out[2] += open(a, a + 4 * words, last[2]);
+        }
+        if (po == kNoPack || !pc.rows) out[3] += open(4 * (int64_t)b.r0, 4 * ((int64_t)b.r0 + nrows + 1), last[3]);
+    }
 }
 
 namespace {
@@ -383,15 +444,26 @@
         if (!o.use_c16 && cb != kCbaseInt32) return false;
         if (!o.use_stage && (staged(cb) || po != kNoPack)) return false;
         const uint32_t *rec = nullptr;
+        const int *own_desc = nullptr;
         if (po != kNoPack) {
             const PackCode pc = pack_decode(po);
             const int nrows = b.r1 - b.r0, kb = b.k0 & ~(vw - 1);
-            const size_t words = (size_t)iw + (pc.rows ? rsp_pack::row_words(nrows) : 0);
             if (po < 0 || !staged(cb) || b.r1 < 0 || o.pack_mode == 0 || pc.rows != (o.pack_mode >= 2) ||
-                !rsp_pack::eligible(rsp::kSpmvThreads, rsp::kSpmvIter * vw, b.k1 - b.k0) || (pc.word & 3) ||
-                pc.word + words > p.runs.size())
+                !rsp_pack::eligible(rsp::kSpmvThreads, rsp::kSpmvIter * vw, b.k1 - b.k0) || ((po >> 1) & 2))
                 return false;
+            const StageCode scp = stage_decode(cb);
+            if (pc.own != (o.pack_mode >= 3 && !scp.list())) return false;
+            const size_t words = pc.own ? (size_t)rsp_pack::rec_words(scp.nr, iw, nrows)
+                                        : (size_t)iw + (pc.rows ? rsp_pack::row_words(nrows) : 0);
+            if (pc.word + words > p.runs.size()) return false;
             rec = reinterpret_cast<const uint32_t *>(p.runs.data()) + pc.word;
+            if (pc.own) {
+                if ((pc.word & (rsp_pack::kRecAlignWords - 1)) || scp.off != 0 || rec[0] != (uint32_t)scp.nr ||
+                    rec[1] != (uint32_t)nrows)
+                    return false;
+                own_desc = reinterpret_cast<const int *>(rec) + rsp_pack::kRecHeadWords;
+                rec += rsp_pack::rec_slot_word(scp.nr);
+            }
             const int nwt = iw / rsp::kSpmvThreads;
             for (int tid = 0; tid < rsp::kSpmvThreads; tid++)
                 for (int f = 0; f < rsp::kSpmvIter * vw; f++) {
@@ -425,7 +497,7 @@
                 if (ofs[u] <= ofs[u - 1]) return false;
         } else if (staged(cb)) {
             if (nr < 1 || nr > rsp::kStageRuns || (size_t)2 * (off + nr + 1) > p.runs.size()) return false;
-            r = p.runs.data() + 2 * (size_t)off;
+            r = own_desc ? own_desc : p.runs.data() + 2 * (size_t)off;
             U = r[2 * nr + 1];
             if (r[1] != 0 || U > g.ucap) return false;
             for (int j = 1; j <= nr; j++)
diff --git a/respasol_amd/csrc/spmv_plan.h b/respasol_amd/csrc/spmv_plan.h
--- a/respasol_amd/csrc/spmv_plan.h
+++ b/respasol_amd/csrc/spmv_plan.h
@@ -30,17 +30,17 @@
 constexpr int64_t kPackWordLimit = 1LL << 30;
 struct PackCode {
     size_t word;
-    int rows;
+    int rows, own;
 };
-inline int pack_encode(int64_t word, int rows) { return (int)(word << 1) | rows; }
-inline PackCode pack_decode(int poff) { return {(size_t)(poff >> 1), poff & 1}; }
+inline int pack_encode(int64_t word, int rows, int own = 0) { return (int)(word << 1) | (own << 1) | rows; }
+inline PackCode pack_decode(int poff) { return {(size_t)(poff >> 1) & ~(size_t)3, poff & 1, (poff >> 1) & 1}; }
 
 struct SpmvBounds {
     size_t nblocks, nlong, nslots;
 };
 
 struct SpmvLayout {
-    size_t off_long, off_part, off_cbase, off_poff, off_cidx, off_runs, bytes;
+    size_t off_long, off_part, off_cidx, off_runs, bytes;
 };
 SpmvLayout spmv_layout(const SpmvBounds &b, size_t elem, int64_t nnz, size_t run_ints = 0);
 
@@ -82,6 +82,8 @@
 
 void plan_stats(const TilePlan &p, rsp_datatype_t type, int64_t out[8]);
 
+void plan_lines(const TilePlan &p, rsp_datatype_t type, int64_t out[5]);
+
 uint64_t digest(const TilePlan &p);
 
 }
diff --git a/respasol_amd/drivers/spmv_pack_check.cpp b/respasol_amd/drivers/spmv_pack_check.cpp
--- a/respasol_amd/drivers/spmv_pack_check.cpp
+++ b/respasol_amd/drivers/spmv_pack_check.cpp
@@ -55,6 +55,39 @@
     return 0;
 }
 
+int check_record(int vw, int k0, int len, int maxrow, int nslots, int nr) {
+    const int fields = kIter * vw, k1 = k0 + len, kb = k0 & ~(vw - 1);
+    std::vector<uint16_t> c16((size_t)k1 + 7);
+    for (uint16_t &c : c16) c = (uint16_t)(rnd() % (uint32_t)nslots);
+    std::vector<int> rp(1, k0);
+    for (int l = 1; rp.back() < k1; l = l % maxrow + 1) rp.push_back(rp.back() + l < k1 ? rp.back() + l : k1);
+    const int nrows = (int)rp.size() - 1;
+    const int iw = rsp_pack::index_words(kThreads, fields);
+    const int sw = rsp_pack::rec_slot_word(nr);
+    if ((sw & 3) || sw < rsp_pack::kRecHeadWords + 2 * (nr + 1) || sw >= rsp_pack::kRecHeadWords + 2 * (nr + 1) + 4 ||
+        rsp_pack::rec_words(nr, iw, nrows) != sw + iw + rsp_pack::row_words(nrows)) {
+        printf("FAIL: record geometry for %d runs\n", nr);
+        return 1;
+    }
+    std::vector<int> desc;
+    for (int j = 0; j <= nr; j++) {
+        desc.push_back(j < nr ? (int)(rnd() & 0xffff) + 70000 * j : 0);
+        desc.push_back(j < nr ? 6 * j : 6 * nr);
+    }
+    std::vector<uint32_t> rec((size_t)rsp_pack::rec_words(nr, iw, nrows));
+    rec[0] = (uint32_t)nr;
+    rec[1] = (uint32_t)nrows;
+    for (size_t i = 0; i < desc.size(); i++) rec[(size_t)rsp_pack::kRecHeadWords + i] = (uint32_t)desc[i];
+    rsp_pack::pack_slots(c16.data(), k0, k1, vw, kIter, kThreads, rec.data() + sw);
+    rsp_pack::pack_rows(rp.data(), 0, nrows, kb, rec.data() + sw + iw);
+    int bad = rec[0] != (uint32_t)nr || rec[1] != (uint32_t)nrows;
+    for (size_t i = 0; i < desc.size(); i++) bad += (int)rec[(size_t)rsp_pack::kRecHeadWords + i] != desc[i];
+    for (int e = k0; e < k1; e++) bad += rsp_pack::unpack_slot(rec.data() + sw, k0, e, vw, kIter, kThreads) != c16[(size_t)e];
+    for (int i = 0; i <= nrows; i++) bad += rsp_pack::unpack_row(rec.data() + sw + iw, i) + kb != rp[(size_t)i];
+    if (bad) printf("FAIL: vw %d k0 %d len %d runs %d: %d words of the record read back wrong\n", vw, k0, len, nr, bad);
+    return bad != 0;
+}
+
 }
 
 int main() {
@@ -74,6 +107,12 @@
     }
     bad += check_tile(2, 5, 2047, 9, 4096);
     bad += check_tile(4, 7, 4093, 9, 4096);
+    for (const Geo &g : geos)
+        for (int nr : {1, 2, 3, 4, 253, 254})
+            for (int maxrow : {1, 256}) {
+                bad += check_record(g.vw, 4096 + nr % (2 * g.vw), maxrow == 1 ? 511 * g.vw / 2 : g.cap, maxrow, g.nslots, nr);
+                n++;
+            }
     printf("%s: %d tiles\n", bad ? "FAILED" : "ok", n + 2);
     return bad ? 1 : 0;
 }
diff --git a/respasol_amd/sparse.py b/respasol_amd/sparse.py
--- a/respasol_amd/sparse.py
+++ b/respasol_amd/sparse.py
@@ -174,6 +174,22 @@
     return dict(zip(PLAN_STATS, (int(v) for v in out)))
 
 
+PLAN_LINES = ("head_lines", "descriptor_lines", "record_lines", "rowptr_lines", "split_head_lines")
+
+
+def spmv_plan_lines(rowptr, colidx, fp32: bool = False, nnz: int | None = None) -> dict:
+    import numpy as np
+
+    rp = np.ascontiguousarray(rowptr, np.int32)
+    ci = np.ascontiguousarray(colidx, np.int32)
+    out = (C.c_int64 * len(PLAN_LINES))()
+    dig = C.c_uint64()
+    check(rsp.rsp_spmv_plan_lines(len(rp) - 1, rp.ctypes.data, ci.ctypes.data,
+                                  int(nnz if nnz is not None else len(ci)), 1 if fp32 else 0, out, C.byref(dig)),
+          "rsp_spmv_plan_lines")
+    return dict(zip(PLAN_LINES, (int(v) for v in out)), digest=int(dig.value))
+
+
 class SpmvBatch:
 
     def __init__(self, handle: Handle, mats: list[SpMat], xs: list[torch.Tensor],
```

Result: no change. 1027 GFLOP/s (-0.7%).
